# kwea123/nsff_pl

Hardware: AMD Instinct MI355X
Metric: ray-samples/sec (coarse+fine, static+dynamic) (higher is better)
Workload: dtype f16x3 (fp32 operands split into 2 halfs, 3 f16 MFMAs per product, fp32 accumulate; same 1e-4 parity as f32); 1 GPU; C2 (BASELINE.json configs[1]): static+dynamic NSFF, 1024 rays/GPU x (64 coarse + 64 importance -> 192 fine pts), train-mode fwd, fw/bw flow warp t+-1, perturb=1 noise_std=1, 8x256 MLPs, N_tau=48, all 47 outputs on device.  `value` is render_rays' throughput with autograd DISABLED (the train-mode FLAGS, inference launches: nothing kept for a backward pass); what a trainer's forward costs is aux.tra; rays_per_gpu=1024, N_samples=64, N_importance=64, parallelism=single GPU, field_launch=persistent (one workgroup per CU)

## Files before the change

include/nsff_render.h:

```cpp
#ifndef NSFF_RENDER_H
#define NSFF_RENDER_H

#include <stddef.h>
#include <stdint.h>

#ifdef __cplusplus
extern "C" {
#endif

#define NSFF_OK               0
#define NSFF_ERR_INVALID     -1
#define NSFF_ERR_NULL        -2
#define NSFF_ERR_ALIGN       -3
#define NSFF_ERR_HIP         -4

#define NSFF_ABI_VERSION      32
#define NSFF_RAW_STRIDE      16
#define NSFF_MAX_FREQS       24
#define NSFF_MAX_LAYERS       8


typedef struct NsffModelDesc {
    int32_t D;
    int32_t W;
    int32_t skip;
    int32_t in_xyz;
    int32_t in_dir;
    int32_t in_a;
    int32_t in_t;
    int32_t use_viewdir;
    int32_t has_transient;
    int32_t has_flow;
    float   flow_scale;
    int32_t skip_mask;
} NsffModelDesc;

static inline uint32_t nsff_skip_layers(const NsffModelDesc* d) {
    return d->skip_mask ? (uint32_t)d->skip_mask : (d->skip > 0 ? 1u << d->skip : 0u);
}

#define NSFF_PREC_F32        0
#define NSFF_PREC_F16X3      1

int nsff_packed_bytes(const NsffModelDesc* desc, int precision, size_t* bytes);

int nsff_param_count(const NsffModelDesc* desc);

int nsff_pack_weights(const NsffModelDesc* desc, int precision, const float* const* params,
                      void* packed, void* stream);

#define NSFF_PACK_SKIP_FOLD 1
int nsff_pack_weights_ex(const NsffModelDesc* desc, int precision, const float* const* params,
                         void* packed, int32_t flags, void* stream);
int nsff_fold_heads(const NsffModelDesc* desc, int precision, const float* const* params, void* packed, void* stream);

int nsff_posenc(const float* x, int64_t n_rows, const float* freqs_host, int n_freqs,
                float* out, void* stream);

int nsff_time_rows(const float* table, int64_t n_table, int32_t width, const int64_t* ts, int64_t n, int64_t max_t,
                   float* next, float* prev, void* stream);

int nsff_time_rows_backward(const float* g_cur, const float* g_next, const float* g_prev, const int64_t* ts, int64_t n,
                            int64_t max_t, int64_t n_table, int32_t width, float* d_table, void* stream);

typedef struct NsffFieldArgs {
    int64_t n_points;
    int32_t precision;
    int32_t tile_points;
    int32_t pts_per_ray;
    int32_t static_mode;
    int32_t transient_mode;
    int32_t flow_heads;
    const float* xyz;
    int32_t n_freqs;
    float   freqs[NSFF_MAX_FREQS];
    const float* dir_emb;
    const float* a_emb;
    const float* t_emb;
    const float* x_emb;
    int32_t ld_emb;
    int32_t off_xyz, off_dir, off_a, off_t;
    float*  raw;
    void*   save_acts;
    void*   save_xin;
    void*   save_masks;
    void*   save_side;
    const float* t_bias;
    int32_t t_bias_rows;
    int32_t reserved0;
    const float* s_bias;
    int32_t s_bias_rows;
    int32_t launch_form;
    int64_t save_lo_delta[3];
} NsffFieldArgs;

int nsff_field_query(const NsffModelDesc* desc, const void* packed,
                     const NsffFieldArgs* args, void* stream);

#define NSFF_MAX_TIME_BIAS_JOBS 4
typedef struct NsffTimeBiasJob {
    const NsffModelDesc* desc;
    const float* w[NSFF_MAX_LAYERS];
    const float* b[NSFF_MAX_LAYERS];
    const float* t_rows;
    float* out;
    const float* table;
    const int64_t* ts;
    int64_t n_table, max_t;
    int32_t delta, pad_;
    float* rows_out;
} NsffTimeBiasJob;
int nsff_time_bias_rows(const NsffModelDesc* desc);
int nsff_time_bias(const NsffTimeBiasJob* jobs, int32_t n_jobs, int64_t n_rays, void* stream);

#define NSFF_MAX_RNG_JOBS 12
typedef struct NsffRngJob {
    float*   out;
    int64_t  numel;
    uint64_t offset;
    int32_t  kind;
    uint32_t grid;
} NsffRngJob;
int nsff_rng_draws(const NsffRngJob* jobs, int32_t n_jobs, uint64_t seed, void* stream);
typedef struct NsffRngCoarse {
    const float* rays;
    const float* z_lin;
    float*       zs;
    float*       xyz;
    int32_t      n_samples;
    float        perturb;
    int32_t      job;
    int32_t      pad_;
} NsffRngCoarse;
int nsff_rng_draws_coarse(const NsffRngJob* jobs, int32_t n_jobs, uint64_t seed, const NsffRngCoarse* coarse, void* stream);

int nsff_side_bias(const NsffModelDesc* desc, const void* packed_f16x3, const float* w_dir, const float* dir_rows,
                   const float* a_rows, int64_t n_rays, float* out, void* stream);

int nsff_train_dims(const NsffModelDesc* desc, int32_t* xin_rows, int32_t* t_row0, int32_t* side_rows);
int nsff_bwd_packed_bytes(const NsffModelDesc* desc, size_t* bytes);
int nsff_pack_weights_bwd(const NsffModelDesc* desc, const float* const* params, void* packed, void* stream);
int nsff_pack_weights_bwd_ex(const NsffModelDesc* desc, const float* const* params, void* packed, const void* fwd_packed, void* stream);

typedef struct NsffFieldBwdArgs {
    int64_t n_points;
    int32_t static_mode;
    int32_t transient_mode;
    const float* d_raw;
    const float* raw;
    const float* gmax;
    const void*  masks;
    void*  dpre;
    void*  dhead;
    float* d_xin;
    float* d_side;
    int64_t dpre_lo_delta;
} NsffFieldBwdArgs;
int nsff_field_backward(const NsffModelDesc* desc, const void* packed_bwd, const NsffFieldBwdArgs* args, void* stream);
int nsff_last_bwd_kernel(void);
int nsff_last_bwd_grid(void);
int nsff_field_bwd_phase_program(const NsffModelDesc* desc, int32_t dynamic, int32_t want_xin, int64_t n_tiles, uint32_t* out,
                                 int32_t max_phases, uint32_t* seg_offsets, int32_t max_segs);

int nsff_field_input_backward(const float* d_xin, int32_t xin_rows, int32_t t_row0, const float* xyz, int64_t n_rays,
                              int32_t pts_per_ray, const float* freqs_host, int32_t n_freqs, int32_t in_t, float* d_xyz,
                              float* d_t, void* stream);

typedef struct NsffWgradJob {
    const void* a;  const void* b;
    int32_t a_rows, b_rows;
    int64_t out_off;
    int32_t trunk, pad_;
    int64_t a_lo_delta, b_lo_delta;
} NsffWgradJob;
int64_t nsff_weight_grad_scratch(const NsffWgradJob* jobs, int32_t n_jobs, int64_t n_tiles, int32_t n_splits);
int nsff_weight_grad(const NsffWgradJob* jobs, int32_t n_jobs, int64_t n_tiles, int32_t n_splits,
                     float* scratch, float* out, float* bias, const float* gmax, void* stream);

typedef struct NsffGradMapEntry {
    int32_t dst;
    int32_t e_a, e_b;
    int16_t job_a, job_b;
} NsffGradMapEntry;
int nsff_weight_grad_accumulate(const NsffWgradJob* jobs, int32_t n_jobs, int64_t n_tiles, int32_t n_splits, float* scratch,
                                const NsffGradMapEntry* map, int64_t n_map, float* grad_base, const float* gmax, void* stream);

int nsff_weight_grad_accumulate_aux(const NsffWgradJob* jobs, int32_t n_jobs, int64_t n_tiles, int32_t n_splits, float* scratch,
                                    const NsffGradMapEntry* map, int64_t n_map, float* grad_base, float* aux, const float* gmax,
                                    void* stream);

typedef struct NsffFoldGradArgs {
    int32_t n_rows, pad_;
    const float* g; const float* gb;
    const float* w_final; const float* b_final;
    const float* w_head[16];
    float* d_w_head[16]; float* d_b_head[16];
    float* d_w_final; float* d_b_final;
} NsffFoldGradArgs;
int nsff_fold_grads(const NsffFoldGradArgs* args, void* stream);

typedef struct NsffFoldDenseArgs {
    int32_t n_rows, accumulate;
    int32_t ld_head, ld_dhead;
    const float* g; const float* g2; const float* gb; const float* gb2;
    const float* w_head; const float* w_final; const float* b_final;
    float* d_w_head; float* d_b_head; float* d_w_final; float* d_b_final;
} NsffFoldDenseArgs;
int nsff_fold_grads_dense(const NsffFoldDenseArgs* args, void* stream);

int nsff_absmax(const float* x, int64_t n, float* out, void* stream);
int nsff_absmax_raw(const float* d_raw, int64_t n_points, float* out16, void* stream);

int nsff_adam_step(float* param, const float* grad, float* exp_avg, float* exp_avg_sq, int64_t n, float* state,
                   const float* lr, double beta1, double beta2, double eps, double weight_decay, void* stream);

int nsff_adam_step_segments(float* param, const float* grad, float* exp_avg, float* exp_avg_sq, int64_t n, float* state,
                            const float* lr, double beta1, double beta2, double eps, double weight_decay,
                            const int64_t* seg_start, int n_seg, int32_t* seg_used, void* stream);

typedef struct NsffLossArgs {
    int64_t n_rays; int32_t n_samples; int32_t n_keep;
    int32_t n_frames; int32_t max_t;
    double  topk;
    int32_t thickness; int32_t pad_;
    const float* rgb_fine; const float* rgb_coarse;
    const float* depth_fine; const float* depth_coarse;
    const float* t_weights; const float* s_weights;
    const float* xyz_fw; const float* xyz_bw;
    const float* rgb_fw; const float* rgb_bw;
    const float* disocc_fw; const float* disocc_bw;
    const float* disoccs_fw; const float* disoccs_bw;
    const float* xyzs_fw_bw; const float* xyzs_bw_fw;
    const float* xyzs_fine; const float* xyzs_fw; const float* xyzs_bw;
    const float* rgbs; const float* disps;
    const int64_t* ts; const int64_t* cam_ids;
    const float* uv_fw; const float* uv_bw;
    const float* Ks; const float* Ps;
    const float* hyper;
    float* stats;
    float* terms;
    const float* term_w;
    const float* weights;
    float* per_ray;
    float* coef;
    float* g_rgb_fine; float* g_rgb_coarse; float* g_depth_fine; float* g_depth_coarse;
    float* g_t_weights; float* g_s_weights; float* g_xyz_fw; float* g_xyz_bw; float* g_rgb_fw; float* g_rgb_bw;
    float* g_xyzs_fw_bw; float* g_xyzs_bw_fw; float* g_xyzs_fw; float* g_xyzs_bw;
} NsffLossArgs;
int nsff_nerfw_loss(const NsffLossArgs* args, int mode, void* stream);

int nsff_coarse_samples(const float* rays, int64_t n_rays, const float* z_lin, int32_t n_samples,
                        float perturb, const float* perturb_rand,
                        float* zs, float* xyz, void* stream);

int nsff_fine_samples(const float* rays, int64_t n_rays, const float* z_lin, const float* zs_coarse,
                      int32_t n_samples, int32_t n_importance,
                      const float* weights_static, const float* weights_transient,
                      const float* u_static, const float* u_transient, int32_t u_per_ray,
                      float* samples_static, float* samples_transient,
                      float* zs_fine, float* xyz_fine, void* stream);

int nsff_sample_pdf(const float* bins, const float* weights, int64_t n_rays, int32_t n_bins_minus1,
                    const float* u, int32_t n_importance, int32_t u_per_ray, float eps,
                    float* samples, void* stream);

int nsff_warp_points(const float* raw, const float* xyz, const float* zs, int64_t n_points,
                     float z_far, float* xyz_fw, float* xyz_bw, void* stream);

int nsff_frame_rays(const float* K4_host, const float* c2w_host, int32_t H, int32_t W, float near, float shift_near,
                    int64_t first_pixel, int64_t n_pixels, float* rays, void* stream);

typedef struct NsffFrustumArgs {
    const float*   w2c;
    const int64_t* ts;
    float   K4[4];
    int32_t n_cams, n_frames, H, W;
} NsffFrustumArgs;

typedef struct NsffCompositeArgs {
    int64_t n_rays;
    int32_t n_samples;
    int32_t has_transient;
    int32_t has_rgb;
    int32_t flow_mode;
    int32_t want_disocc;
    float   noise_std;
    float   z_far;
    const float* raw;
    const float* raw_fw;
    const float* raw_bw;
    const float* zs;
    const float* xyz;
    const float* xyz_fw;
    const float* xyz_bw;
    const float* noise_static;
    const float* noise_transient;
    const float* noise_fw;
    const float* noise_bw;
    const float* visibility;
    float* static_rgbs;  float* transient_rgbs;
    float* flows_fw;     float* flows_bw;
    float* static_sigmas; float* transient_sigmas;
    float* static_alphas; float* transient_alphas;
    float* static_weights; float* transient_weights; float* weights;
    float* xyzs_fw_bw;   float* xyzs_bw_fw;
    float* disoccs_fw;   float* disoccs_bw;
    float* depth;  float* rgb;  float* transient_alpha;  float* transient_rgb;
    float* static_only_rgb;  float* static_only_depth;
    float* xyz_exp;  float* flow_fw_exp;  float* flow_bw_exp;  float* xyz_fw_exp;  float* xyz_bw_exp;
    float* rgb_fw;   float* rgb_bw;
    float* disocc_fw;  float* disocc_bw;
    NsffFrustumArgs vis;
} NsffCompositeArgs;

int nsff_composite(const NsffCompositeArgs* args, void* stream);

int nsff_frustum_visibility(const NsffFrustumArgs* vis, const float* xyz, int64_t n_points, float* vis_count,
                            void* stream);

typedef struct NsffSplatArgs {
    int32_t H, W, n_planes;
    float   K4[4];
    float   P[12];
    float   scale;
    const float* xyz;
    const float* flow;
    const float* rgb;
    const float* alpha;
    float*       accum;
    void*        work;
    int64_t      work_bytes;
} NsffSplatArgs;
int64_t nsff_splat_work_bytes(int32_t H, int32_t W, int32_t n_planes);
int nsff_splat_planes(const NsffSplatArgs* args, void* stream);

typedef struct NsffMpiArgs {
    int32_t H, W, n_planes;
    float   dt;
    const float* accum_fw;
    const float* accum_bw;
    const float* static_rgb;
    const float* static_alpha;
    const float* zs;
    float* rgb;
    float* depth;
} NsffMpiArgs;
int nsff_mpi_composite(const NsffMpiArgs* args, void* stream);

typedef struct NsffCompositeBwdArgs {
    int64_t n_rays;
    int32_t n_samples, has_transient, flow_mode;
    float   noise_std;
    const float* raw;  const float* raw_fw;  const float* raw_bw;
    const float* zs;   const float* xyz;     const float* f_fw;  const float* f_bw;
    const float* noise_static;  const float* noise_transient;  const float* noise_fw;  const float* noise_bw;
    const float* g_static_sigmas;  const float* g_transient_sigmas;
    const float* g_static_weights; const float* g_transient_weights;  const float* g_weights;
    const float* g_depth;  const float* g_rgb;  const float* g_transient_alpha;  const float* g_transient_rgb;
    const float* g_so_rgb; const float* g_so_depth;
    const float* g_xyz_exp;  const float* g_flow_fw_exp;  const float* g_flow_bw_exp;
    const float* g_rgb_fw;   const float* g_rgb_bw;
    float* scratch;
    float* d_raw;  float* d_raw_fw;  float* d_raw_bw;  float* d_f_fw;  float* d_f_bw;
} NsffCompositeBwdArgs;
int nsff_composite_backward(const NsffCompositeBwdArgs* args, void* stream);

typedef struct {
    int64_t n_points;
    const float* zs;
    float z_far;
    int32_t accumulate;
    int32_t col_a, col_b;
    int32_t pad_;
    const float* g_a[4];
    const float* g_b[4];
    float* out;
} NsffFlowGradArgs;
int nsff_flow_grad(const NsffFlowGradArgs* args, void* stream);

#define NSFF_RAY_RECORD      16

typedef struct NsffSsimArgs {
    int32_t n_frames, H, W, window;
    const float* gt;  const float* pred;  const uint8_t* mask;
    float* map;  float* mean_map;  double* sums;
    void* scratch;  int64_t scratch_bytes;
} NsffSsimArgs;
int64_t nsff_ssim_scratch_bytes(int32_t n_frames, int32_t H, int32_t W);
int nsff_ssim(const NsffSsimArgs* args, void* stream);

int nsff_cdf(const float* weights, int64_t n_frames, int64_t n, double* cdf, void* stream);

typedef struct NsffRayDrawArgs {
    int64_t n_frames, n_pixels, frame, batch;
    const float* records;  const double* cdf;  const float* u;
    float* rays;  float* rgbs;  int64_t* ts;  int64_t* cam_ids;  float* disps;  float* rays_mask;  float* uv_fw;  float* uv_bw;
    int64_t* rand_idx;
} NsffRayDrawArgs;
int nsff_ray_draw(const NsffRayDrawArgs* args, void* stream);

int nsff_prof_enable(int on);
int nsff_prof_collect(int64_t* launches, double* total_ms, double* total_flops, double* executed_flops);
int nsff_prof_collect_clock(int64_t* launches, double* total_ms, double* total_flops, double* executed_flops,
                            double* shader_ticks, double* ticks_ms);

#define NSFF_KERNEL_F32       1
#define NSFF_KERNEL_H3_64     2
#define NSFF_KERNEL_H3_8WAVE  3
#define NSFF_KERNEL_H3A       4
#define NSFF_KERNEL_H3_SAVE   5
#define NSFF_KERNEL_H3A_TBIAS 7
#define NSFF_KERNEL_H3A_SAVE  9
#define NSFF_KERNEL_H3A_SIDE  8
int         nsff_last_field_kernel(void);
int         nsff_last_field_grid(void);
int         nsff_field_phase_program(const NsffModelDesc* desc, int static_mode, int transient_mode, int fold_t, uint32_t* steps,
                             int* n_steps, int* n_static_steps, uint32_t* phases_static, uint32_t* phases_dynamic, int* n_phases);

#define NSFF_RANGE_ACT     0x1u
#define NSFF_RANGE_SAVED   0x2u
#define NSFF_RANGE_PARAMS  0x4u
#define NSFF_RANGE_CODES   0x8u
int         nsff_range_flags(uint32_t* out, int32_t clear, void* stream);

int         nsff_abi_version(void);
const char* nsff_last_hip_error(void);

#ifdef __cplusplus
}
#endif
#endif
```

nsff_pl_amd/_lib.py:

```python
import ctypes as C
import os

import torch

_HERE = os.path.dirname(os.path.abspath(__file__))
LIB_PATH = os.environ.get("NSFF_LIB") or os.path.join(_HERE, "libnsff_hip.so")

RAW_STRIDE = 16
ABI_VERSION = 32
MAX_FREQS = 24

_ERR = {-1: "NSFF_ERR_INVALID (bad shape/flag/unsupported architecture)",
        -2: "NSFF_ERR_NULL (required pointer missing)",
        -3: "NSFF_ERR_ALIGN (pointer not 16-byte aligned)",
        -4: "NSFF_ERR_HIP"}

_fp = C.c_void_p


class ModelDesc(C.Structure):
    _fields_ = [("D", C.c_int32), ("W", C.c_int32), ("skip", C.c_int32),
                ("in_xyz", C.c_int32), ("in_dir", C.c_int32), ("in_a", C.c_int32),
                ("in_t", C.c_int32), ("use_viewdir", C.c_int32),
                ("has_transient", C.c_int32), ("has_flow", C.c_int32),
# ... 4 lines not shown
    _fields_ = [("n_points", C.c_int64), ("precision", C.c_int32), ("tile_points", C.c_int32),
                ("pts_per_ray", C.c_int32),
                ("static_mode", C.c_int32), ("transient_mode", C.c_int32),
                ("flow_heads", C.c_int32),
                ("xyz", _fp), ("n_freqs", C.c_int32), ("freqs", C.c_float * MAX_FREQS),
                ("dir_emb", _fp), ("a_emb", _fp), ("t_emb", _fp),
                ("x_emb", _fp), ("ld_emb", C.c_int32),
                ("off_xyz", C.c_int32), ("off_dir", C.c_int32), ("off_a", C.c_int32),
                ("off_t", C.c_int32), ("raw", _fp), ("save_acts", _fp), ("save_xin", _fp), ("save_masks", _fp),
                ("save_side", _fp), ("t_bias", _fp), ("t_bias_rows", C.c_int32), ("reserved0", C.c_int32),
                ("s_bias", _fp), ("s_bias_rows", C.c_int32), ("launch_form", C.c_int32), ("save_lo_delta", C.c_int64 * 3)]


class TimeBiasJob(C.Structure):
    _fields_ = [("desc", C.POINTER(ModelDesc)), ("w", _fp * 8), ("b", _fp * 8), ("t_rows", _fp), ("out", _fp),
                ("table", _fp), ("ts", _fp), ("n_table", C.c_int64), ("max_t", C.c_int64), ("delta", C.c_int32), ("pad_", C.c_int32),
                ("rows_out", _fp)]


MAX_TIME_BIAS_JOBS = 4


class RngJob(C.Structure):
    _fields_ = [("out", _fp), ("numel", C.c_int64), ("offset", C.c_uint64), ("kind", C.c_int32), ("grid", C.c_uint32)]


MAX_RNG_JOBS = 12


class RngCoarse(C.Structure):
    _fields_ = [("rays", _fp), ("z_lin", _fp), ("zs", _fp), ("xyz", _fp), ("n_samples", C.c_int32), ("perturb", C.c_float),
                ("job", C.c_int32), ("pad_", C.c_int32)]


_COMPOSITE_PTRS_IN = ["raw", "raw_fw", "raw_bw", "zs", "xyz", "xyz_fw", "xyz_bw",
                      "noise_static", "noise_transient", "noise_fw", "noise_bw", "visibility"]
_COMPOSITE_PTRS_OUT = ["static_rgbs", "transient_rgbs", "flows_fw", "flows_bw",
                       "static_sigmas", "transient_sigmas", "static_alphas", "transient_alphas",
                       "static_weights", "transient_weights", "weights",
                       "xyzs_fw_bw", "xyzs_bw_fw", "disoccs_fw", "disoccs_bw",
                       "depth", "rgb", "transient_alpha", "transient_rgb",
                       "static_only_rgb", "static_only_depth",
                       "xyz_exp", "flow_fw_exp", "flow_bw_exp", "xyz_fw_exp", "xyz_bw_exp",
                       "rgb_fw", "rgb_bw", "disocc_fw", "disocc_bw"]


class FrustumArgs(C.Structure):
    _fields_ = [("w2c", _fp), ("ts", _fp), ("K4", C.c_float * 4), ("n_cams", C.c_int32), ("n_frames", C.c_int32),
                ("H", C.c_int32), ("W", C.c_int32)]


class CompositeArgs(C.Structure):
    _fields_ = ([("n_rays", C.c_int64), ("n_samples", C.c_int32), ("has_transient", C.c_int32),
                 ("has_rgb", C.c_int32), ("flow_mode", C.c_int32), ("want_disocc", C.c_int32),
                 ("noise_std", C.c_float), ("z_far", C.c_float)]
                + [(n, _fp) for n in _COMPOSITE_PTRS_IN]
                + [(n, _fp) for n in _COMPOSITE_PTRS_OUT]
                + [("vis", FrustumArgs)])


_CBWD_IN = ["raw", "raw_fw", "raw_bw", "zs", "xyz", "f_fw", "f_bw", "noise_static", "noise_transient", "noise_fw", "noise_bw"]
_CBWD_G = ["g_static_sigmas", "g_transient_sigmas", "g_static_weights", "g_transient_weights", "g_weights", "g_depth",
           "g_rgb", "g_transient_alpha", "g_transient_rgb", "g_so_rgb", "g_so_depth", "g_xyz_exp", "g_flow_fw_exp",
           "g_flow_bw_exp", "g_rgb_fw", "g_rgb_bw"]
_CBWD_OUT = ["scratch", "d_raw", "d_raw_fw", "d_raw_bw", "d_f_fw", "d_f_bw"]


class CompositeBwdArgs(C.Structure):
    _fields_ = ([("n_rays", C.c_int64), ("n_samples", C.c_int32), ("has_transient", C.c_int32), ("flow_mode", C.c_int32),
                 ("noise_std", C.c_float)] + [(n, _fp) for n in _CBWD_IN + _CBWD_G + _CBWD_OUT])


class FieldBwdArgs(C.Structure):
    _fields_ = [("n_points", C.c_int64), ("static_mode", C.c_int32), ("transient_mode", C.c_int32),
                ("d_raw", _fp), ("raw", _fp), ("gmax", _fp), ("masks", _fp), ("dpre", _fp), ("dhead", _fp),
                ("d_xin", _fp), ("d_side", _fp), ("dpre_lo_delta", C.c_int64)]


class WgradJob(C.Structure):
    _fields_ = [("a", _fp), ("b", _fp), ("a_rows", C.c_int32), ("b_rows", C.c_int32), ("out_off", C.c_int64), ("trunk", C.c_int32),
                ("pad_", C.c_int32), ("a_lo_delta", C.c_int64), ("b_lo_delta", C.c_int64)]


class FoldGradArgs(C.Structure):
    _fields_ = [("n_rows", C.c_int32), ("pad_", C.c_int32), ("g", _fp), ("gb", _fp), ("w_final", _fp), ("b_final", _fp),
                ("w_head", _fp * 16), ("d_w_head", _fp * 16), ("d_b_head", _fp * 16), ("d_w_final", _fp), ("d_b_final", _fp)]


class FoldDenseArgs(C.Structure):
    _fields_ = [("n_rows", C.c_int32), ("accumulate", C.c_int32), ("ld_head", C.c_int32), ("ld_dhead", C.c_int32),
                ("g", _fp), ("g2", _fp), ("gb", _fp), ("gb2", _fp), ("w_head", _fp), ("w_final", _fp), ("b_final", _fp),
                ("d_w_head", _fp), ("d_b_head", _fp), ("d_w_final", _fp), ("d_b_final", _fp)]


class SplatArgs(C.Structure):
    _fields_ = [("H", C.c_int32), ("W", C.c_int32), ("n_planes", C.c_int32), ("K4", C.c_float * 4),
                ("P", C.c_float * 12), ("scale", C.c_float),
                ("xyz", _fp), ("flow", _fp), ("rgb", _fp), ("alpha", _fp), ("accum", _fp), ("work", _fp),
                ("work_bytes", C.c_int64)]


class MpiArgs(C.Structure):
    _fields_ = [("H", C.c_int32), ("W", C.c_int32), ("n_planes", C.c_int32), ("dt", C.c_float),
                ("accum_fw", _fp), ("accum_bw", _fp), ("static_rgb", _fp), ("static_alpha", _fp), ("zs", _fp),
                ("rgb", _fp), ("depth", _fp)]


_LOSS_IN = ["rgb_fine", "rgb_coarse", "depth_fine", "depth_coarse", "t_weights", "s_weights", "xyz_fw", "xyz_bw", "rgb_fw",
            "rgb_bw", "disocc_fw", "disocc_bw", "disoccs_fw", "disoccs_bw", "xyzs_fw_bw", "xyzs_bw_fw", "xyzs_fine",
            "xyzs_fw", "xyzs_bw", "rgbs", "disps", "ts", "cam_ids", "uv_fw", "uv_bw", "Ks", "Ps", "hyper", "stats", "terms",
            "term_w"]
LOSS_GRADS = ["g_rgb_fine", "g_rgb_coarse", "g_depth_fine", "g_depth_coarse", "g_t_weights", "g_s_weights", "g_xyz_fw",
              "g_xyz_bw", "g_rgb_fw", "g_rgb_bw", "g_xyzs_fw_bw", "g_xyzs_bw_fw", "g_xyzs_fw", "g_xyzs_bw"]


class LossArgs(C.Structure):
    _fields_ = ([("n_rays", C.c_int64), ("n_samples", C.c_int32), ("n_keep", C.c_int32), ("n_frames", C.c_int32),
                 ("max_t", C.c_int32), ("topk", C.c_double), ("thickness", C.c_int32), ("pad_", C.c_int32)]
                + [(n, _fp) for n in _LOSS_IN] + [("weights", _fp), ("per_ray", _fp), ("coef", _fp)]
                + [(n, _fp) for n in LOSS_GRADS])


class FlowGradArgs(C.Structure):
    _fields_ = [("n_points", C.c_int64), ("zs", _fp), ("z_far", C.c_float), ("accumulate", C.c_int32), ("col_a", C.c_int32),
                ("col_b", C.c_int32), ("pad_", C.c_int32), ("g_a", _fp * 4), ("g_b", _fp * 4), ("out", _fp)]


class SsimArgs(C.Structure):
    _fields_ = [("n_frames", C.c_int32), ("H", C.c_int32), ("W", C.c_int32), ("window", C.c_int32),
                ("gt", _fp), ("pred", _fp), ("mask", _fp), ("map", _fp), ("mean_map", _fp), ("sums", _fp),
                ("scratch", _fp), ("scratch_bytes", C.c_int64)]


RAY_RECORD = 16
_DRAW_OUT = ["rays", "rgbs", "ts", "cam_ids", "disps", "rays_mask", "uv_fw", "uv_bw", "rand_idx"]


class RayDrawArgs(C.Structure):
    _fields_ = ([("n_frames", C.c_int64), ("n_pixels", C.c_int64), ("frame", C.c_int64), ("batch", C.c_int64),
                 ("records", _fp), ("cdf", _fp), ("u", _fp)] + [(n, _fp) for n in _DRAW_OUT])


_SIGNATURES = {
    "nsff_abi_version": (C.c_int, []),
    "nsff_range_flags": (C.c_int, [_fp, C.c_int32, _fp]),
    "nsff_last_field_kernel": (C.c_int, []),
    "nsff_last_field_grid": (C.c_int, []),
    "nsff_field_phase_program": (C.c_int, [C.POINTER(ModelDesc), C.c_int, C.c_int, C.c_int, C.POINTER(C.c_uint32), C.POINTER(C.c_int),
                                   C.POINTER(C.c_int), C.POINTER(C.c_uint32), C.POINTER(C.c_uint32), C.POINTER(C.c_int)]),
    "nsff_time_bias_rows": (C.c_int, [C.POINTER(ModelDesc)]),
    "nsff_time_bias": (C.c_int, [C.POINTER(TimeBiasJob), C.c_int32, C.c_int64, C.c_void_p]),
    "nsff_rng_draws": (C.c_int, [C.POINTER(RngJob), C.c_int32, C.c_uint64, C.c_void_p]),
    "nsff_rng_draws_coarse": (C.c_int, [C.POINTER(RngJob), C.c_int32, C.c_uint64, C.POINTER(RngCoarse), C.c_void_p]),
    "nsff_side_bias": (C.c_int, [C.POINTER(ModelDesc), _fp, _fp, _fp, _fp, C.c_int64, _fp, C.c_void_p]),
    "nsff_last_hip_error": (C.c_char_p, []),
    "nsff_packed_bytes": (C.c_int, [C.POINTER(ModelDesc), C.c_int, C.POINTER(C.c_size_t)]),
    "nsff_param_count": (C.c_int, [C.POINTER(ModelDesc)]),
    "nsff_pack_weights": (C.c_int, [C.POINTER(ModelDesc), C.c_int, C.POINTER(_fp), _fp, _fp]),
    "nsff_pack_weights_ex": (C.c_int, [C.POINTER(ModelDesc), C.c_int, C.POINTER(_fp), _fp, C.c_int32, _fp]),
    "nsff_fold_heads": (C.c_int, [C.POINTER(ModelDesc), C.c_int, C.POINTER(_fp), _fp, _fp]),
    "nsff_posenc": (C.c_int, [_fp, C.c_int64, C.POINTER(C.c_float), C.c_int, _fp, _fp]),
    "nsff_time_rows": (C.c_int, [_fp, C.c_int64, C.c_int32, _fp, C.c_int64, C.c_int64, _fp, _fp, _fp]),
    "nsff_time_rows_backward": (C.c_int, [_fp, _fp, _fp, _fp, C.c_int64, C.c_int64, C.c_int64, C.c_int32, _fp, _fp]),
    "nsff_field_query": (C.c_int, [C.POINTER(ModelDesc), _fp, C.POINTER(FieldArgs), _fp]),
    "nsff_coarse_samples": (C.c_int, [_fp, C.c_int64, _fp, C.c_int32, C.c_float, _fp, _fp, _fp, _fp]),
    "nsff_fine_samples": (C.c_int, [_fp, C.c_int64, _fp, _fp, C.c_int32, C.c_int32, _fp, _fp, _fp, _fp,
                                    C.c_int32, _fp, _fp, _fp, _fp, _fp]),
    "nsff_sample_pdf": (C.c_int, [_fp, _fp, C.c_int64, C.c_int32, _fp, C.c_int32, C.c_int32,
                                  C.c_float, _fp, _fp]),
    "nsff_warp_points": (C.c_int, [_fp, _fp, _fp, C.c_int64, C.c_float, _fp, _fp, _fp]),
    "nsff_composite": (C.c_int, [C.POINTER(CompositeArgs), _fp]),
    "nsff_frustum_visibility": (C.c_int, [C.POINTER(FrustumArgs), _fp, C.c_int64, _fp, _fp]),
    "nsff_frame_rays": (C.c_int, [C.POINTER(C.c_float), C.POINTER(C.c_float), C.c_int32, C.c_int32, C.c_float,
                                  C.c_float, C.c_int64, C.c_int64, _fp, _fp]),
    "nsff_bwd_packed_bytes": (C.c_int, [C.POINTER(ModelDesc), C.POINTER(C.c_size_t)]),
    "nsff_pack_weights_bwd": (C.c_int, [C.POINTER(ModelDesc), C.POINTER(_fp), _fp, _fp]),
    "nsff_field_backward": (C.c_int, [C.POINTER(ModelDesc), _fp, C.POINTER(FieldBwdArgs), _fp]),
    "nsff_field_input_backward": (C.c_int, [_fp, C.c_int32, C.c_int32, _fp, C.c_int64, C.c_int32, C.POINTER(C.c_float), C.c_int32,
                                            C.c_int32, _fp, _fp, _fp]),
    "nsff_train_dims": (C.c_int, [C.POINTER(ModelDesc), C.POINTER(C.c_int32), C.POINTER(C.c_int32), C.POINTER(C.c_int32)]),
    "nsff_weight_grad_scratch": (C.c_int64, [C.POINTER(WgradJob), C.c_int32, C.c_int64, C.c_int32]),
    "nsff_weight_grad": (C.c_int, [C.POINTER(WgradJob), C.c_int32, C.c_int64, C.c_int32, _fp, _fp, _fp, _fp, _fp]),
    "nsff_weight_grad_accumulate": (C.c_int, [C.POINTER(WgradJob), C.c_int32, C.c_int64, C.c_int32, _fp, _fp, C.c_int64,
                                              _fp, _fp, _fp]),
    "nsff_weight_grad_accumulate_aux": (C.c_int, [C.POINTER(WgradJob), C.c_int32, C.c_int64, C.c_int32, _fp, _fp, C.c_int64,
                                                  _fp, _fp, _fp, _fp]),
    "nsff_absmax_raw": (C.c_int, [_fp, C.c_int64, _fp, _fp]),
    "nsff_last_bwd_kernel": (C.c_int, []),
    "nsff_last_bwd_grid": (C.c_int, []),
    "nsff_field_bwd_phase_program": (C.c_int, [C.POINTER(ModelDesc), C.c_int32, C.c_int32, C.c_int64, C.POINTER(C.c_uint32), C.c_int32,
                                                C.POINTER(C.c_uint32), C.c_int32]),
    "nsff_fold_grads": (C.c_int, [C.POINTER(FoldGradArgs), _fp]),
    "nsff_fold_grads_dense": (C.c_int, [C.POINTER(FoldDenseArgs), _fp]),
    "nsff_pack_weights_bwd_ex": (C.c_int, [C.POINTER(ModelDesc), C.POINTER(_fp), _fp, _fp, _fp]),
    "nsff_absmax": (C.c_int, [_fp, C.c_int64, _fp, _fp]),
    "nsff_adam_step": (C.c_int, [_fp, _fp, _fp, _fp, C.c_int64, _fp, _fp, C.c_double, C.c_double, C.c_double, C.c_double, _fp]),
    "nsff_adam_step_segments": (C.c_int, [_fp, _fp, _fp, _fp, C.c_int64, _fp, _fp, C.c_double, C.c_double, C.c_double, C.c_double,
                                          _fp, C.c_int, _fp, _fp]),
    "nsff_composite_backward": (C.c_int, [C.POINTER(CompositeBwdArgs), _fp]),
    "nsff_flow_grad": (C.c_int, [C.POINTER(FlowGradArgs), _fp]),
    "nsff_nerfw_loss": (C.c_int, [C.POINTER(LossArgs), C.c_int, _fp]),
    "nsff_splat_planes": (C.c_int, [C.POINTER(SplatArgs), _fp]),
    "nsff_splat_work_bytes": (C.c_int64, [C.c_int32, C.c_int32, C.c_int32]),
    "nsff_mpi_composite": (C.c_int, [C.POINTER(MpiArgs), _fp]),
    "nsff_ssim_scratch_bytes": (C.c_int64, [C.c_int32, C.c_int32, C.c_int32]),
    "nsff_ssim": (C.c_int, [C.POINTER(SsimArgs), _fp]),
    "nsff_cdf": (C.c_int, [_fp, C.c_int64, C.c_int64, _fp, _fp]),
    "nsff_ray_draw": (C.c_int, [C.POINTER(RayDrawArgs), _fp]),
    "nsff_prof_enable": (C.c_int, [C.c_int]),
    "nsff_prof_collect": (C.c_int, [C.POINTER(C.c_int64), C.POINTER(C.c_double), C.POINTER(C.c_double), C.POINTER(C.c_double)]),
    "nsff_prof_collect_clock": (C.c_int, [C.POINTER(C.c_int64)] + [C.POINTER(C.c_double)] * 5),
}
EXPORTED_SYMBOLS = tuple(_SIGNATURES)

_lib = None


def load():
    global _lib
    if _lib is None:
        if not os.path.exists(LIB_PATH):
            raise RuntimeError(
                f"{LIB_PATH} is missing: build it with `python -c 'import __graft_entry__ as g; g.build()'` "
                "(or `make -C nsff_pl_amd/csrc`).  There is no CPU fallback for the render path.")
        lib = C.CDLL(LIB_PATH)
        for name, (res, args) in _SIGNATURES.items():
            fn = getattr(lib, name)
            fn.restype, fn.argtypes = res, args
        if lib.nsff_abi_version() != ABI_VERSION:
            raise RuntimeError("libnsff_hip.so ABI version mismatch")
        _lib = lib
    return _lib


def _check(rc, what):
    if rc != 0:
        msg = _ERR.get(rc, f"error {rc}")
        if rc == -4:
            msg += ": " + load().nsff_last_hip_error().decode()
        raise RuntimeError(f"{what} failed: {msg}")


def require_gpu_tensor(t, what):
    if not isinstance(t, torch.Tensor) or not t.is_cuda:
        raise RuntimeError(f"{what} must be a GPU tensor: the NSFF render path runs only on the "
                           "HIP kernels of libnsff_hip.so (no CPU fallback)")


def _ptr(t):
    if t is None:
        return None
    assert t.is_cuda and t.dtype == torch.float32 and t.is_contiguous(), "need contiguous fp32 GPU tensor"
    return t.data_ptr()


def _stream():
    return torch.cuda.current_stream().cuda_stream


def model_desc(model):
    if model.W != 256:
        raise RuntimeError(f"unsupported NeRF architecture: W={model.W} (the gfx950 field kernels tile W=256 trunks "
                           "into 4 x 64-neuron wave blocks; other widths are not built)")
    skips = sorted(set(int(s) for s in model.skips))
    if not 2 <= model.D <= 8 or any(not 1 <= s < model.D for s in skips):
        raise RuntimeError(f"unsupported NeRF architecture: D={model.D}, skips={list(model.skips)} (need 2 <= D <= 8 "
                           "and every skip layer in 1..D-1; a skip at layer 0 would concatenate the input with itself)")
    mask = sum(1 << s for s in skips)
    return ModelDesc(D=model.D, W=model.W, skip=skips[0] if len(skips) == 1 else 0, skip_mask=mask if len(skips) != 1 else 0,
                     in_xyz=model.in_channels_xyz,
                     in_dir=model.in_channels_dir,
                     in_a=model.in_channels_a if model.use_viewdir else 0,
                     in_t=model.in_channels_t, use_viewdir=int(model.use_viewdir),
                     has_transient=int(model.encode_transient),
                     has_flow=int(getattr(model, "has_flow_heads", hasattr(model, "transient_flow_fw"))),
                     flow_scale=float(getattr(model, "flow_scale", 0.0)))


def param_list(model):
    def lin(m):
        layer = m[0] if isinstance(m, torch.nn.Sequential) else m
        return [layer.weight, layer.bias]
    out = []
    for i in range(model.D):
        out += lin(getattr(model, f"static_xyz_encoding_{i + 1}"))
    out += lin(model.static_xyz_encoding_final)
    if model.use_viewdir:
        out += lin(model.static_dir_encoding)
    out += lin(model.static_sigma) + lin(model.static_rgb)
    if model.encode_transient:
        for i in range(model.D):
            out += lin(getattr(model, f"transient_xyz_encoding_{i + 1}"))
        out += lin(model.transient_xyz_encoding_final)
        out += lin(model.transient_sigma) + lin(model.transient_rgb)
        if hasattr(model, "transient_flow_fw"):
            out += lin(model.transient_flow_fw) + lin(model.transient_flow_bw)
    return out


def packed_bytes(desc, precision=0):
    n = C.c_size_t(0)
    _check(load().nsff_packed_bytes(C.byref(desc), int(precision), C.byref(n)), "nsff_packed_bytes")
    return n.value


PACK_SKIP_FOLD = 1


def pack_weights(desc, params, packed, precision=0, fold=True):
    lib = load()
    if lib.nsff_param_count(C.byref(desc)) != len(params):
        raise RuntimeError("parameter list does not match the model description")
    keep = [p.detach().contiguous().float() for p in params]
    for p in keep:
        require_gpu_tensor(p, "model parameter")
    arr = (_fp * len(keep))(*[p.data_ptr() for p in keep])
    _check(lib.nsff_pack_weights_ex(C.byref(desc), int(precision), arr, _ptr(packed), 0 if fold else PACK_SKIP_FOLD,
                                    _stream()), "nsff_pack_weights_ex")
    return keep


def fold_heads(desc, params, packed, precision):
    keep = [p.detach().contiguous().float() for p in params]
    arr = (_fp * len(keep))(*[p.data_ptr() for p in keep])
    _check(load().nsff_fold_heads(C.byref(desc), int(precision), arr, _ptr(packed), _stream()), "nsff_fold_heads")
    return keep


def time_rows_backward(g_cur, g_next, g_prev, ts, max_t, n_table):
    gs = [None if g is None else g.contiguous() for g in (g_cur, g_next, g_prev)]
    width = next(g for g in gs if g is not None).shape[1]
    assert ts.dtype == torch.int64 and ts.is_cuda and ts.is_contiguous()
    d = torch.empty(int(n_table), width, device=ts.device)
    _check(load().nsff_time_rows_backward(_ptr(gs[0]), _ptr(gs[1]), _ptr(gs[2]), C.c_void_p(ts.data_ptr()), ts.shape[0],
                                          int(max_t), int(n_table), width, _ptr(d), _stream()), "nsff_time_rows_backward")
    return d


def time_rows(table, ts, max_t, want_next=True, want_prev=True):
    n, width = ts.shape[0], table.shape[1]
    if want_next and want_prev:
        both = torch.empty(2, n, width, device=table.device)
        nxt, prv = both[0], both[1]
    else:
        nxt = torch.empty(n, width, device=table.device) if want_next else None
        prv = torch.empty(n, width, device=table.device) if want_prev else None
    assert ts.dtype == torch.int64 and ts.is_cuda and ts.is_contiguous()
    _check(load().nsff_time_rows(_ptr(table), table.shape[0], width, C.c_void_p(ts.data_ptr()), n, int(max_t),
                                 _ptr(nxt), _ptr(prv), _stream()), "nsff_time_rows")
    return nxt, prv


def posenc(x, freqs, out):
    f = [float(v) for v in freqs]
    arr = (C.c_float * len(f))(*f)
    _check(load().nsff_posenc(_ptr(x), x.shape[0], arr, len(f), _ptr(out), _stream()), "nsff_posenc")


def field_query(model, raw, n_points, pts_per_ray, static_mode, transient_mode, flow_heads=0,
                xyz=None, freqs=None, dir_emb=None, a_emb=None, t_emb=None,
                x_emb=None, emb_offsets=(0, -1, -1, -1), save_acts=None, save_xin=None, save_masks=None, save_side=None,
                precision=None, t_bias=None, s_bias=None, save_lo=False):
    from . import config
    desc = model_desc(model)
    prec = config.precision_code(model) if precision is None else precision
    saves = not (save_acts is None and save_xin is None and save_masks is None and save_side is None)
    packed = model.packed(prec)
    a = FieldArgs()
    a.precision, a.tile_points = prec, config.get_tile_points()
    a.launch_form = 0 if config.get_persistent() else 1
    a.n_points, a.pts_per_ray = int(n_points), int(pts_per_ray)
    a.static_mode, a.transient_mode, a.flow_heads = int(static_mode), int(transient_mode), int(flow_heads)
    a.xyz = _ptr(xyz)
    if freqs is not None:
        f = [float(v) for v in freqs]
        if len(f) > MAX_FREQS:
            raise RuntimeError("too many embedding frequencies")
        a.n_freqs = len(f)
        for i, v in enumerate(f):
            a.freqs[i] = v
    a.dir_emb, a.a_emb, a.t_emb = _ptr(dir_emb), _ptr(a_emb), _ptr(t_emb)
    a.x_emb = _ptr(x_emb)
    a.ld_emb = int(x_emb.shape[1]) if x_emb is not None else 0
    a.off_xyz, a.off_dir, a.off_a, a.off_t = [int(v) for v in emb_offsets]
    a.raw = _ptr(raw)
    a.save_acts = None if save_acts is None else save_acts.data_ptr()
    a.save_xin = None if save_xin is None else save_xin.data_ptr()
    a.save_masks = None if save_masks is None else save_masks.data_ptr()
    a.save_side = None if save_side is None else save_side.data_ptr()
    if save_lo:
        for i, t in enumerate((save_acts, save_xin, save_side)):
            a.save_lo_delta[i] = 0 if t is None else lo_delta(t)
    if t_bias is not None:
        a.t_bias, a.t_bias_rows = _ptr(t_bias), int(t_bias.shape[1])
    if s_bias is not None:
        a.s_bias, a.s_bias_rows = _ptr(s_bias), int(s_bias.shape[1])
    _check(load().nsff_field_query(C.byref(desc), _ptr(packed), C.byref(a), _stream()), "nsff_field_query")


def lo_delta(t):
    n = t.numel()
    if t.untyped_storage().nbytes() < (t.storage_offset() + 2 * n) * t.element_size():
        raise RuntimeError("three-product backward: this buffer has no remainder plane behind it (field_grad.alloc_saves(..., x3=True))")
    return n


def side_bias(model, dir_rows, a_rows=None):
    from . import config
    desc = model_desc(model)
    n_rays = int(dir_rows.shape[0])
    assert dir_rows.shape == (n_rays, desc.in_dir) and (desc.in_a == 0 or (a_rows is not None and a_rows.shape == (n_rays, desc.in_a)))
    packed = model.packed(config.PRECISIONS["f16x3"])
    w = model.static_dir_encoding[0].weight.detach()
    out = torch.empty(n_rays, 1, 256, device=dir_rows.device, dtype=torch.float32)
    _check(load().nsff_side_bias(C.byref(desc), _ptr(packed), _ptr(w), _ptr(dir_rows), _ptr(a_rows) if desc.in_a > 0 else None,
                                 n_rays, _ptr(out), _stream()), "nsff_side_bias")
    return out


_DEVICE_RNG_GEOMETRY = {}


def fused_draws(plan, device, values=True, coarse=None):
    dev = torch.device(device)
    idx = dev.index if dev.index is not None else torch.cuda.current_device()
    if idx not in _DEVICE_RNG_GEOMETRY:
        p = torch.cuda.get_device_properties(idx)
        _DEVICE_RNG_GEOMETRY[idx] = p.multi_processor_count * (p.max_threads_per_multi_processor // 256)
    max_grid = _DEVICE_RNG_GEOMETRY[idx]
    gen = torch.cuda.default_generators[idx]
    seed, offset = gen.initial_seed(), gen.get_offset()
    wanted = values if isinstance(values, (list, tuple)) else [bool(values)] * len(plan)
    sizes = []
    for kind, shape in plan:
        n = 1
        for s in shape:
            n *= int(s)
        sizes.append(n)
    total = sum(n for n, w in zip(sizes, wanted) if w)
    buf = torch.empty(max(total, 1), device=dev, dtype=torch.float32)
    outs, jobs, at = [], [], 0
    for (kind, shape), numel, want in zip(plan, sizes, wanted):
        if numel == 0:
            outs.append(torch.empty(*shape, device=dev, dtype=torch.float32))
            continue
        grid = min(max_grid, (numel + 255) // 256)
        if coarse is not None and not outs and not want:
            jobs.append((None, numel, offset, 0, grid))
            outs.append(None)
        elif want:
            t = buf[at:at + numel].view(*shape)
            at += numel
            jobs.append((t, numel, offset, 1 if kind == "randn" else 0, grid))
            outs.append(t)
        else:
            outs.append(None)
        offset += ((numel - 1) // (1024 * grid) + 1) * 4
    hook = None
    if coarse is not None:
        rays, z_lin, perturb, zs, xyz = coarse
        assert plan and plan[0][0] == "rand" and tuple(plan[0][1]) == (rays.shape[0], z_lin.shape[0]) and perturb > 0
        if sizes[0]:
            hook = RngCoarse(_ptr(rays), _ptr(z_lin), _ptr(zs), _ptr(xyz), int(z_lin.shape[0]), float(perturb), 0, 0)
    for k in range(0, len(jobs), MAX_RNG_JOBS):
        part = jobs[k:k + MAX_RNG_JOBS]
        arr = (RngJob * len(part))()
        for j, (t, numel, off, kind, grid) in enumerate(part):
            arr[j].out, arr[j].numel, arr[j].offset, arr[j].kind, arr[j].grid = (None if t is None else t.data_ptr()), numel, off, kind, grid
        with torch.cuda.device(idx):
            _check(load().nsff_rng_draws_coarse(arr, len(part), seed, C.byref(hook) if (hook is not None and k == 0) else None, _stream()),
                   "nsff_rng_draws")
    gen.set_offset(offset)
    return outs


_FUSED_DRAWS_OK = {}


def fused_draws_match_torch(device):
    dev = torch.device(device)
    idx = dev.index if dev.index is not None else torch.cuda.current_device()
    if idx in _FUSED_DRAWS_OK:
        return _FUSED_DRAWS_OK[idx]
    if torch.cuda.is_current_stream_capturing():
        return False
    gen = torch.cuda.default_generators[idx]
    state = gen.get_state()
    ok = True
    try:
        plan = [("rand", (7, 64)), ("randn", (1031,)), ("rand", (3, 5, 2)), ("randn", (70000,)), ("rand", (300001,))]
        gen.manual_seed(0x5EED1234)
        gen.set_offset(8)
        mine = fused_draws(plan, torch.device("cuda", idx))
        end_mine = gen.get_offset()
        gen.manual_seed(0x5EED1234)
        gen.set_offset(8)
        with torch.cuda.device(idx):
            ref = [(torch.rand if k == "rand" else torch.randn)(*shape, device=torch.device("cuda", idx)) for k, shape in plan]
        end_ref = gen.get_offset()
        ok = end_mine == end_ref and all(torch.equal(a.view(torch.int32), b.view(torch.int32)) for a, b in zip(mine, ref))
    except Exception:
        ok = False
    finally:
        gen.set_state(state)
    if not ok:
        import warnings
        warnings.warn("nsff_pl_amd: the fused generator kernel (nsff_rng_draws) no longer reproduces torch.rand / torch.randn on "
                      f"cuda:{idx} (torch {torch.__version__}); render_rays draws with the torch calls instead (slower by ~1 %, same "
                      "numbers as the reference)")
    _FUSED_DRAWS_OK[idx] = ok
    return ok


def time_bias_rows(model):
    return load().nsff_time_bias_rows(C.byref(model_desc(model)))


def time_bias(jobs, index=None):
    assert 1 <= len(jobs) <= MAX_TIME_BIAS_JOBS
    arr = (TimeBiasJob * len(jobs))()
    keep, outs, per_model, pair = [], [], {}, None
    rows_of = {}
    if index is not None:
        table, ts, max_t = index
        assert ts.dtype == torch.int64 and ts.is_cuda and ts.is_contiguous() and ts.dim() == 1, "ts: one int64 frame index per ray"
        n_rays, width = int(ts.shape[0]), int(table.shape[1])
        deltas = sorted({int(d) for _, d in jobs})
        if 1 in deltas and -1 in deltas:
            both = torch.empty(2, n_rays, width, device=table.device, dtype=torch.float32)
            rows_of[1], rows_of[-1] = both[0], both[1]
        for d in deltas:
            if d not in rows_of:
                rows_of[d] = torch.empty(n_rays, width, device=table.device, dtype=torch.float32)
        written = set()
    else:
        n_rays = int(jobs[0][1].shape[0])
    for j, (model, t_rows) in enumerate(jobs):
        if id(model) not in per_model:
            desc = model_desc(model)
            lins = [getattr(model, f"transient_xyz_encoding_{l + 1}")[0] for l in [0] + sorted(set(int(v) for v in model.skips))]
            wb = [(m.weight.detach(), m.bias.detach()) for m in lins]
            for w, b in wb:
                _ptr(w), _ptr(b)
            per_model[id(model)] = (desc, C.pointer(desc), wb)
        desc, pdesc, wb = per_model[id(model)]
        if index is not None:
            delta, t_rows = int(t_rows), None
            assert width == desc.in_t
        else:
            assert t_rows.shape == (n_rays, desc.in_t)
        dev = wb[0][0].device
        if j + 1 < len(jobs) and jobs[j + 1][0] is model and pair is None:
            pair = torch.empty(2, n_rays, len(wb), 256, device=dev, dtype=torch.float32)
            out = pair[0]
        elif pair is not None:
            out, pair = pair[1], None
        else:
            out = torch.empty(n_rays, len(wb), 256, device=dev, dtype=torch.float32)
        arr[j].desc = pdesc
        for i, (w, b) in enumerate(wb):
            arr[j].w[i], arr[j].b[i] = w.data_ptr(), b.data_ptr()
        arr[j].t_rows, arr[j].out = _ptr(t_rows), _ptr(out)
        if index is not None:
            arr[j].table, arr[j].ts = _ptr(table), ts.data_ptr()
            arr[j].n_table, arr[j].max_t, arr[j].delta = int(table.shape[0]), int(max_t), delta
            if delta not in written:
                arr[j].rows_out = _ptr(rows_of[delta])
                written.add(delta)
        outs.append(out)
    keep.append(per_model)
    _check(load().nsff_time_bias(arr, len(jobs), n_rays, _stream()), "nsff_time_bias")
    return outs if index is None else (outs, rows_of)


def coarse_samples(rays, z_lin, perturb, perturb_rand, zs, xyz):
    _check(load().nsff_coarse_samples(_ptr(rays), rays.shape[0], _ptr(z_lin), z_lin.shape[0],
                                      float(perturb), _ptr(perturb_rand), _ptr(zs), _ptr(xyz), _stream()),
           "nsff_coarse_samples")


def fine_samples(rays, z_lin, zs_coarse, n_importance, w_static, w_transient, u_static, u_transient,
                 u_per_ray, samples_static, samples_transient, zs_fine, xyz_fine):
    _check(load().nsff_fine_samples(_ptr(rays), rays.shape[0], _ptr(z_lin), _ptr(zs_coarse),
                                    z_lin.shape[0], int(n_importance), _ptr(w_static), _ptr(w_transient),
                                    _ptr(u_static), _ptr(u_transient), int(u_per_ray),
                                    _ptr(samples_static), _ptr(samples_transient),
                                    _ptr(zs_fine), _ptr(xyz_fine), _stream()), "nsff_fine_samples")


def sample_pdf(bins, weights, u, u_per_ray, eps, samples):
    _check(load().nsff_sample_pdf(_ptr(bins), _ptr(weights), weights.shape[0], weights.shape[1],
                                  _ptr(u), samples.shape[1], int(u_per_ray), float(eps),
                                  _ptr(samples), _stream()), "nsff_sample_pdf")


def warp_points(raw, xyz, zs, z_far, xyz_fw, xyz_bw):
    _check(load().nsff_warp_points(_ptr(raw), _ptr(xyz), _ptr(zs), zs.numel(), float(z_far),
                                   _ptr(xyz_fw), _ptr(xyz_bw), _stream()), "nsff_warp_points")


def frustum_args(w2c, ts, K4, n_cams, n_frames, H, W):
    assert w2c.is_cuda and w2c.dtype == torch.float32 and w2c.is_contiguous() and w2c.shape == (n_cams * n_frames, 12)
    assert ts.is_cuda and ts.dtype == torch.int64 and ts.is_contiguous() and ts.numel() >= 1
    a = FrustumArgs(w2c=w2c.data_ptr(), ts=ts.data_ptr(), n_cams=int(n_cams), n_frames=int(n_frames), H=int(H), W=int(W))
    a.K4[:] = [float(v) for v in K4]
    a._keep = (w2c, ts)
    return a


def frustum_visibility(vis, xyz, out):
    _check(load().nsff_frustum_visibility(C.byref(vis), _ptr(xyz), xyz.shape[0], _ptr(out), _stream()),
           "nsff_frustum_visibility")


def composite(vis=None, **kw):
    a = CompositeArgs()
    for k, v in kw.items():
        if k in _COMPOSITE_PTRS_IN or k in _COMPOSITE_PTRS_OUT:
            setattr(a, k, _ptr(v))
        else:
            setattr(a, k, v)
    if vis is not None:
        a.vis = vis
    _check(load().nsff_composite(C.byref(a), _stream()), "nsff_composite")


def frame_rays(K4, c2w12, H, W, near, shift_near, first, count, rays):
    k = (C.c_float * 4)(*[float(v) for v in K4])
    m = (C.c_float * 12)(*[float(v) for v in c2w12])
    _check(load().nsff_frame_rays(k, m, int(H), int(W), float(near), float(shift_near), int(first), int(count),
                                  _ptr(rays), _stream()), "nsff_frame_rays")


BWD_PACK = 100


def bwd_packed_bytes(desc):
    n = C.c_size_t(0)
    _check(load().nsff_bwd_packed_bytes(C.byref(desc), C.byref(n)), "nsff_bwd_packed_bytes")
    return n.value


def pack_weights_bwd(desc, params, packed, fwd_packed=None):
    arr = (_fp * len(params))(*[p.data_ptr() for p in params])
    _check(load().nsff_pack_weights_bwd_ex(C.byref(desc), arr, _ptr(packed), _ptr(fwd_packed), _stream()), "nsff_pack_weights_bwd_ex")


def last_bwd_kernel():
    return {0: "c", 1: "h3b", 2: "c+h3b", 3: "x3"}[load().nsff_last_bwd_kernel()]


def last_bwd_grid():
    return load().nsff_last_bwd_grid()


def field_bwd_phase_program(model, dynamic, want_xin, n_tiles, max_phases=32):
    import numpy as np
    desc = model_desc(model)
    out = (C.c_uint32 * (8 * max_phases))()
    segs = (C.c_uint32 * 48)()
    n = load().nsff_field_bwd_phase_program(C.byref(desc), 1 if dynamic else 0, 1 if want_xin else 0, int(n_tiles), out, max_phases, segs, 48)
    if n < 0:
        raise RuntimeError(f"nsff_field_bwd_phase_program failed ({n})")
    offs = np.array(list(segs), np.uint32)
    return (np.array(list(out), np.uint32).reshape(max_phases, 8)[:n] if n > 0 else None), offs


def field_backward(model, n_points, static, transient, d_raw, raw, gmax, masks, dpre, dhead, d_xin, d_side=None, x3=False):
    desc = model_desc(model)
    a = FieldBwdArgs(n_points=int(n_points), static_mode=2 if static else 0, transient_mode=2 if transient else 0,
                     d_raw=_ptr(d_raw), raw=_ptr(raw), gmax=_ptr(gmax), masks=masks.data_ptr(), dpre=dpre.data_ptr(),
                     dhead=dhead.data_ptr(), d_xin=_ptr(d_xin), d_side=_ptr(d_side), dpre_lo_delta=lo_delta(dpre) if x3 else 0)
    _check(load().nsff_field_backward(C.byref(desc), _ptr(model.packed(BWD_PACK)), C.byref(a), _stream()),
           "nsff_field_backward")


def train_dims(model):
    desc = model_desc(model)
    xr, t0, sr = C.c_int32(0), C.c_int32(0), C.c_int32(0)
    _check(load().nsff_train_dims(C.byref(desc), C.byref(xr), C.byref(t0), C.byref(sr)), "nsff_train_dims")
    return xr.value, t0.value, sr.value


def field_input_backward(d_xin, t_row0, xyz, pts_per_ray, freqs, in_t, want_xyz, want_t):
    P, xin_rows = d_xin.shape
    n_rays = P // pts_per_ray
    d_xyz = torch.empty(P, 3, device=d_xin.device) if want_xyz else None
    d_t = torch.empty(n_rays, in_t, device=d_xin.device) if want_t else None
    f = [float(v) for v in freqs]
    arr = (C.c_float * max(len(f), 1))(*f)
    _check(load().nsff_field_input_backward(_ptr(d_xin), int(xin_rows), int(t_row0), _ptr(xyz), n_rays, int(pts_per_ray), arr,
                                            len(f), int(in_t), _ptr(d_xyz), _ptr(d_t), _stream()), "nsff_field_input_backward")
    return d_xyz, d_t


def _wgrad_jobs(jobs, with_off):
    return (WgradJob * len(jobs))(*[WgradJob(a=j[0], b=j[1], a_rows=j[2], b_rows=j[3], out_off=j[4] if with_off else 0, trunk=j[5],
                                             a_lo_delta=j[6] if len(j) > 6 else 0, b_lo_delta=j[7] if len(j) > 7 else 0) for j in jobs])


def weight_grad(jobs, n_tiles, n_splits, out, bias, gmax):
    arr = _wgrad_jobs(jobs, True)
    n = load().nsff_weight_grad_scratch(arr, len(jobs), int(n_tiles), int(n_splits))
    if n < 0:
        raise RuntimeError("nsff_weight_grad_scratch failed")
    scratch = torch.empty(n, device=out.device)
    _check(load().nsff_weight_grad(arr, len(jobs), int(n_tiles), int(n_splits), _ptr(scratch), _ptr(out), _ptr(bias),
                                   _ptr(gmax), _stream()), "nsff_weight_grad")


def weight_grad_accumulate(jobs, n_tiles, n_splits, grad_map, grad_base_ptr, gmax, aux=None):
    arr = _wgrad_jobs(jobs, False)
    n = load().nsff_weight_grad_scratch(arr, len(jobs), int(n_tiles), int(n_splits))
    if n < 0:
        raise RuntimeError("nsff_weight_grad_scratch failed")
    assert grad_map.dtype == torch.int32 and grad_map.is_contiguous() and grad_map.shape[1] == 4
    scratch = torch.empty(n, device=gmax.device)
    _check(load().nsff_weight_grad_accumulate_aux(arr, len(jobs), int(n_tiles), int(n_splits), _ptr(scratch),
                                                  C.c_void_p(grad_map.data_ptr()), grad_map.shape[0], C.c_void_p(grad_base_ptr),
                                                  _ptr(aux), _ptr(gmax), _stream()), "nsff_weight_grad_accumulate_aux")
    return scratch


def fold_grads(g, gb, w_final, b_final, head_rows, d_w_final, d_b_final):
    a = FoldGradArgs(n_rows=len(head_rows), g=_ptr(g), gb=_ptr(gb), w_final=_ptr(w_final), b_final=_ptr(b_final),
                     d_w_final=_ptr(d_w_final), d_b_final=_ptr(d_b_final))
    for r, (w, dw, db) in enumerate(head_rows):
        a.w_head[r], a.d_w_head[r], a.d_b_head[r] = w.data_ptr(), dw.data_ptr(), db.data_ptr()
    _check(load().nsff_fold_grads(C.byref(a), _stream()), "nsff_fold_grads")


def fold_grads_dense(g, gb, w_head, w_final, b_final, d_w_head, d_b_head, d_w_final, d_b_final, accumulate, g2=None, gb2=None):
    R = int(g.shape[0])
    for t in (g, g2, gb, gb2, w_final, b_final, d_w_final, d_b_final, d_b_head):
        assert t is None or (t.is_cuda and t.dtype == torch.float32 and t.is_contiguous())
    for t in (w_head, d_w_head):
        assert t.is_cuda and t.dtype == torch.float32 and t.shape[0] == R and t.shape[1] == 256 and t.stride(1) == 1
    a = FoldDenseArgs(n_rows=R, accumulate=1 if accumulate else 0, ld_head=int(w_head.stride(0)), ld_dhead=int(d_w_head.stride(0)),
                      g=g.data_ptr(), g2=None if g2 is None else g2.data_ptr(), gb=gb.data_ptr(), gb2=None if gb2 is None else gb2.data_ptr(),
                      w_head=w_head.data_ptr(), w_final=w_final.data_ptr(), b_final=b_final.data_ptr(), d_w_head=d_w_head.data_ptr(),
                      d_b_head=d_b_head.data_ptr(), d_w_final=d_w_final.data_ptr(), d_b_final=d_b_final.data_ptr())
    _check(load().nsff_fold_grads_dense(C.byref(a), _stream()), "nsff_fold_grads_dense")


def absmax(x):
    x = x.contiguous()
    if x.dim() == 2 and x.shape[1] == RAW_STRIDE:
        out = torch.empty(RAW_STRIDE, device=x.device, dtype=torch.float32)
        _check(load().nsff_absmax_raw(_ptr(x), x.shape[0], _ptr(out), _stream()), "nsff_absmax_raw")
        return out
    out = torch.empty((), device=x.device, dtype=torch.float32)
    _check(load().nsff_absmax(_ptr(x), x.numel(), _ptr(out), _stream()), "nsff_absmax")
    return out


def adam_step(param, grad, exp_avg, exp_avg_sq, state, lr, beta1, beta2, eps, weight_decay, seg_start=None, seg_used=None):
    if seg_start is None:
        _check(load().nsff_adam_step(_ptr(param), _ptr(grad), _ptr(exp_avg), _ptr(exp_avg_sq), param.numel(), _ptr(state), _ptr(lr),
                                     float(beta1), float(beta2), float(eps), float(weight_decay), _stream()), "nsff_adam_step")
        return
    _check(load().nsff_adam_step_segments(_ptr(param), _ptr(grad), _ptr(exp_avg), _ptr(exp_avg_sq), param.numel(), _ptr(state),
                                          _ptr(lr), float(beta1), float(beta2), float(eps), float(weight_decay),
                                          C.c_void_p(seg_start.data_ptr()), int(seg_used.numel()),
                                          C.c_void_p(seg_used.data_ptr()), _stream()),
           "nsff_adam_step_segments")


def composite_backward(n_rays, n_samples, has_transient, flow_mode, noise_std, **tensors):
    a = CompositeBwdArgs(n_rays=int(n_rays), n_samples=int(n_samples), has_transient=int(has_transient),
                         flow_mode=int(flow_mode), noise_std=float(noise_std))
    for k, v in tensors.items():
        setattr(a, k, _ptr(v))
    _check(load().nsff_composite_backward(C.byref(a), _stream()), "nsff_composite_backward")


def flow_grad(zs, z_far, out, accumulate, col_a=-1, g_a=(), col_b=-1, g_b=()):
    a = FlowGradArgs(n_points=int(out.shape[0]), zs=_ptr(zs), z_far=float(z_far), accumulate=int(bool(accumulate)),
# ... 152 lines not shown
```

nsff_pl_amd/csrc/field_h3.hip:

```cpp
#include <hip/hip_runtime.h>
#include <algorithm>
#include <cstdlib>
#include <vector>
#include "nsff_layout_h3.h"
#include "nsff_common.h"
#include "nsff_internal.h"

typedef float f32x16 __attribute__((ext_vector_type(16)));
typedef _Float16 h8 __attribute__((ext_vector_type(8)));
typedef _Float16 h4 __attribute__((ext_vector_type(4)));
typedef __fp16 h2 __attribute__((ext_vector_type(2)));
typedef _Float16 h2f __attribute__((ext_vector_type(2)));

#ifdef H3_TIMING
__device__ unsigned g_h3_timing[256 * 8 * 32 * 6 + 256 * 4 * 256];
#define H3A_TBASE (256 * 8 * 32 * 6)
__device__ unsigned long long g_h3_span[2] = {~0ull, 0ull};
#define H3_SPAN(k) do { if (lane == 0) { const unsigned long long t_ = __builtin_amdgcn_s_memtime(); \
    if (k) atomicMax(&g_h3_span[1], t_); else atomicMin(&g_h3_span[0], t_); } } while (0)
#define H3_STAMP(k) do { if (lane == 0 && blockIdx.x < 256 && i < 32) \
    g_h3_timing[((blockIdx.x * 8 + wave_id) * 32 + i) * 6 + (k)] = (unsigned)__builtin_amdgcn_s_memtime(); } while (0)
#define H3_HSTAMP(k) do { if (lane == 0 && blockIdx.x < 256) \
    g_h3_timing[((blockIdx.x * 8 + wave) * 32 + 30) * 6 + (k)] = (unsigned)__builtin_amdgcn_s_memtime(); } while (0)
#else
#define H3_STAMP(k) do {} while (0)
#define H3_SPAN(k) do {} while (0)
#define H3_HSTAMP(k) do {} while (0)
#endif

namespace {

#ifndef H3_SAVE_INTERLEAVE
#define H3_SAVE_INTERLEAVE 1
#endif
constexpr int LDH = 264;
__device__ __forceinline__ h8 lds_h8(const _Float16* p) { return *reinterpret_cast<const h8*>(p); }

struct H3Step {
    uint32_t w_off;
    uint32_t bias_off;
    uint16_t nks;
    uint8_t pre;
    uint8_t post;
    uint8_t head;
    uint8_t save;
    uint8_t pad[2];
};
enum { PRE_NONE = 0, PRE_INPUT = 1, PRE_INPUT_T = 2, PRE_SIDE = 3 };
enum { POST_NONE = 0, POST_RELU = 1, POST_LINEAR = 2 };
enum { HEAD_NONE = 0, HEAD_S_SIGMA = 1, HEAD_S_RGB = 2, HEAD_T = 3, HEAD_S_FOLD = 4, HEAD_T_FOLD = 5 };
constexpr int MAX_STEPS = 28;

struct H3KArgs {
    NsffLayoutH3 L;
    H3Step steps[MAX_STEPS];
    int n_steps;
    int n_static_steps;
    int split_trunks;
    long long grid_tiles;
    const uint32_t* packed;
    const float* xyz;
    const float* x_emb;
    const float* dir_emb;
    const float* a_emb;
    const float* t_emb;
    const float* t_bias;
    int tb_rows;
    const float* s_bias;
    int sb_rows;
    float* raw;
    long long lo_delta[3];
    _Float16* save_acts;
    _Float16* save_xin;
    unsigned long long* save_masks;
    _Float16* save_side;
    long long save_stride;
    int xin_rows, side_rows;
    long long n_tiles;
    long long n_points;
    int pts_per_ray;
    int static_mode, transient_mode;
    int D, skip;
    int in_xyz, in_dir, in_a, in_t;
    int use_viewdir;
    float flow_scale;
    int n_freqs;
    int octave_freqs;
    float freqs[NSFF_MAX_FREQS];
    int ld_emb, off_xyz, off_dir, off_a, off_t;
    unsigned long long* span;
    uint32_t* range;
};

struct SpanT { unsigned long long t, r; };
__device__ __forceinline__ SpanT span_begin(const unsigned long long* span) {
    SpanT s{0ull, 0ull};
#ifdef H3_TIMING
    s.t = __builtin_amdgcn_s_memtime();
#endif
    if (span != nullptr && (blockIdx.x & 15) == 0) { s.t = __builtin_amdgcn_s_memtime(); s.r = __builtin_amdgcn_s_memrealtime(); }
    return s;
}
__device__ __forceinline__ void span_end(unsigned long long* span, const SpanT& s0, unsigned tid) {
    if (span == nullptr || (blockIdx.x & 15) != 0 || tid != 0) return;
    const unsigned long long t = __builtin_amdgcn_s_memtime(), r = __builtin_amdgcn_s_memrealtime();
    atomicAdd(span, t - s0.t);
    atomicAdd(span + 1, r - s0.r);
}
__device__ __forceinline__ void span_end(unsigned long long* span, const SpanT& s0) { span_end(span, s0, threadIdx.x); }

#define MFMA_H(a, b, c) __builtin_amdgcn_mfma_f32_32x32x16_f16((a), (b), (c), 0, 0, 0)
#define H3_PIN() __builtin_amdgcn_sched_barrier(0)

__device__ __forceinline__ void split_store(_Float16* xh, _Float16* xl, int idx, float v, float& rm) {
    rm = nsff_absmax3(rm, v, v);
    const _Float16 hi = (_Float16)v;
    xh[idx] = hi;
    xl[idx] = (_Float16)(v - (float)hi);
}

template <int MTW> struct WFrag { h8 wh[MTW], wl[MTW]; };
template <int NT> struct XFrag { h8 xh[NT], xl[NT]; };
template <int MTW> struct WRing { WFrag<MTW> r[4]; };
template <int MTW> struct BiasRegs { float4 b[MTW][4]; };

template <int MTW>
__device__ __forceinline__ void load_w(WFrag<MTW>& f, const uint4* __restrict__& wp) {
    if constexpr (MTW == 2) {
        const uint4 a0 = wp[0], a1 = wp[64], a2 = wp[128], a3 = wp[192];
        wp += 256;
        f.wh[0] = __builtin_bit_cast(h8, a0); f.wl[0] = __builtin_bit_cast(h8, a1);
        f.wh[1] = __builtin_bit_cast(h8, a2); f.wl[1] = __builtin_bit_cast(h8, a3);
    } else {
        const uint4 a0 = wp[0], a1 = wp[64];
        wp += 256;
        f.wh[0] = __builtin_bit_cast(h8, a0); f.wl[0] = __builtin_bit_cast(h8, a1);
    }
}

template <int NT> struct BRows { const _Float16* h[NT]; const _Float16* l[NT]; };
template <int NT>
__device__ __forceinline__ BRows<NT> b_rows(const _Float16* bh, const _Float16* bl, int ld) {
    BRows<NT> b;
#pragma unroll
    for (int nt = 0; nt < NT; ++nt) { b.h[nt] = bh + nt * 32 * ld; b.l[nt] = bl + nt * 32 * ld; }
    return b;
}

template <int NT>
__device__ __forceinline__ void load_x(XFrag<NT>& f, const BRows<NT>& b, int ks) {
#pragma unroll
    for (int nt = 0; nt < NT; ++nt) {
        f.xh[nt] = lds_h8(b.h[nt] + ks * 16);
        f.xl[nt] = lds_h8(b.l[nt] + ks * 16);
    }
}

template <int MTW>
__device__ __forceinline__ const uint4* prefetch_w(WRing<MTW>& ring, const uint4* __restrict__ w) {
// ... 1513 lines not shown
                       hipStream_t st) {
    const NsffModelDesc& d = *desc;
    FoldArgs fs, ft, fd;
    const int pi = fold_args(d, params, fs, ft, fd);
    for (int i = 0; i < pi; ++i) if (!params[i]) return NSFF_ERR_NULL;
    if (!d.use_viewdir) {
        fs.out_w = s_w; fs.out_b = s_b;
        hipLaunchKernelGGL(nsff_fold_kernel_h3, dim3(4), dim3(256), 0, st, fs);
    }
    if (d.has_transient) {
        ft.out_w = t_w; ft.out_b = t_b;
        hipLaunchKernelGGL(nsff_fold_kernel_h3, dim3(d.has_flow ? 10 : 4), dim3(256), 0, st, ft);
    }
    return nsff_launch_status();
}

int nsff_h3_fold_heads(const NsffModelDesc* desc, const float* const* params, void* packed, hipStream_t st) {
    NsffLayoutH3 L;
    const int rc = nsff_make_layout_h3(*desc, L);
    if (rc) return rc;
    const NsffModelDesc& d = *desc;
    FoldArgs fs, ft, fd;
    const int pi = fold_args(d, params, fs, ft, fd);
    for (int i = 0; i < pi; ++i) if (!params[i]) return NSFF_ERR_NULL;
    uint32_t* pw = reinterpret_cast<uint32_t*>(packed);
    PackArgsH3 pf{};
    pf.dst = pw;
    pf.range = nsff_range_word(st);
    int nf = 0;
    auto fold = [&](FoldArgs& f, uint32_t scratch, uint32_t tile, uint32_t bias) {
        f.out_w = reinterpret_cast<float*>(pw + scratch); f.out_b = reinterpret_cast<float*>(pw + bias);
        hipLaunchKernelGGL(nsff_fold_kernel_h3, dim3(32), dim3(256), 0, st, f);
        pf.seg[nf++] = PackSegH3{f.out_w, tile, 2, NSFF_W, NSFF_W, 0, 0, 0, 0, 0, 0, 32};
    };
    if (!d.use_viewdir) fold(fs, L.fold_f32, L.s_fold_w, L.s_fold_b);
    if (d.has_transient) fold(ft, L.fold_f32 + 32 * NSFF_W, L.t_fold_w, L.t_fold_b);
    int max_threads = 8 * NSFF_W;
    if (d.use_viewdir) {
        fd.out_w = reinterpret_cast<float*>(pw + L.dir_fold_f32); fd.out_b = reinterpret_cast<float*>(pw + L.dir_b_fold);
        hipLaunchKernelGGL(nsff_fold_kernel_h3, dim3(NSFF_W), dim3(256), 0, st, fd);
        pf.seg[nf++] = PackSegH3{fd.out_w, L.dir_h_fold, 1, NSFF_W, NSFF_W, NSFF_W, 0, 0, 0, 0, 0, 0};
        max_threads = 64 * NSFF_W;
    }
    if (nf > 0) hipLaunchKernelGGL(nsff_pack_kernel_h3, dim3((max_threads + 255) / 256, nf), dim3(256), 0, st, pf);
    return nsff_launch_status();
}

static int h3_step_program(const NsffModelDesc& d, int static_mode, int transient_mode, bool fold, H3KArgs& k, bool side_fold = false) {
    int n = 0;
    auto push = [&](uint32_t w, uint32_t b, uint32_t kcols, int pre, int post, int head, int slot = -1) {
        H3Step& s = k.steps[n++];
        s.w_off = w; s.bias_off = b; s.nks = (uint16_t)(kcols / 16);
        s.pre = (uint8_t)pre; s.post = (uint8_t)post; s.head = (uint8_t)head;
        s.save = (uint8_t)(slot + 1);
    };
    auto trunk = [&](const NsffTrunkLayoutH3& T, int pre_kind, int last_head, int slot0) {
        for (int l = 0; l < d.D; ++l) {
            const int head = (l == d.D - 1) ? last_head : HEAD_NONE;
            if (l == 0) {
                push(T.seg_x[0], T.bias[0], T.k0, pre_kind, POST_RELU, HEAD_NONE, slot0);
            } else if ((nsff_skip_layers(&d) >> l) & 1u) {
                push(T.seg_h[l], T.bias[l], NSFF_W, PRE_NONE, POST_NONE, HEAD_NONE);
                push(T.seg_x[l], NSFF_NONE, T.k0, pre_kind, POST_RELU, head, slot0 + l);
            } else {
                push(T.seg_h[l], T.bias[l], NSFF_W, PRE_NONE, POST_RELU, head, slot0 + l);
            }
        }
    };
    if (static_mode == 2 && fold && !d.use_viewdir) {
        trunk(k.L.st, PRE_INPUT, HEAD_S_FOLD, 0);
    } else if (static_mode == 2 && fold && side_fold) {
        trunk(k.L.st, PRE_INPUT, HEAD_S_SIGMA, 0);
        push(k.L.dir_h_fold, k.L.dir_b_fold, NSFF_W, PRE_NONE, POST_RELU, HEAD_S_RGB, d.D);
    } else if (static_mode == 2 && fold) {
        trunk(k.L.st, PRE_INPUT, HEAD_S_SIGMA, 0);
        push(k.L.dir_h_fold, k.L.dir_b_fold, NSFF_W, PRE_NONE, POST_NONE, HEAD_NONE);
        push(k.L.dir_x, NSFF_NONE, k.L.side_k, PRE_SIDE, POST_RELU, HEAD_S_RGB, d.D);
    } else if (static_mode) {
        trunk(k.L.st, PRE_INPUT, HEAD_S_SIGMA, 0);
        if (static_mode == 2) {
            push(k.L.st.final_w, k.L.st.final_b, NSFF_W, PRE_NONE, POST_LINEAR, d.use_viewdir ? HEAD_NONE : HEAD_S_RGB, d.D);
            if (d.use_viewdir) {
                push(k.L.dir_h, k.L.dir_b, NSFF_W, PRE_NONE, POST_NONE, HEAD_NONE);
                push(k.L.dir_x, NSFF_NONE, k.L.side_k, PRE_SIDE, POST_RELU, HEAD_S_RGB, d.D);
            }
        }
    }
    k.n_static_steps = n;
    if (transient_mode && fold) {
        trunk(k.L.tr, PRE_INPUT_T, HEAD_T_FOLD, d.D + 1);
    } else if (transient_mode) {
        trunk(k.L.tr, PRE_INPUT_T, HEAD_NONE, d.D + 1);
        push(k.L.tr.final_w, k.L.tr.final_b, NSFF_W, PRE_NONE, POST_LINEAR, HEAD_T, 2 * d.D + 1);
    }
    if (n > MAX_STEPS) return NSFF_ERR_INVALID;
    k.n_steps = n;
    return NSFF_OK;
}

static bool h3a_make_persistent(H3APhase* ph) {
    int at = -1;
    for (int i = 1; i < H3A_MAX_PHASES && !(i > 1 && ph[i].d[0] == H3A_BODY_END); ++i)
        if (ph[i].d[0] == H3A_BODY_B16L) { if (at >= 0) return false; at = i; }
    if (at < 0) return false;
    ph[at].d[0] = H3A_BODY_B16LP;
    for (int j = 3; j < 8; ++j) ph[at].d[j] = ph[0].d[j];
    return true;
}

extern "C" int nsff_field_phase_program(const NsffModelDesc* desc, int static_mode, int transient_mode, int fold_t, uint32_t* steps,
                                int* n_steps, int* n_static_steps, uint32_t* phases_static, uint32_t* phases_dynamic, int* n_phases) {
    if (!desc || !steps || !n_steps || !n_static_steps || !phases_static || !phases_dynamic || !n_phases) return NSFF_ERR_NULL;
    H3KArgs k{};
    int rc = nsff_make_layout_h3(*desc, k.L);
    if (rc) return rc;
    const bool side_fold = (fold_t & 2) != 0 && static_mode == 2 && desc->use_viewdir;
    const bool persist = (fold_t & 4) != 0;
    fold_t &= 1;
    rc = h3_step_program(*desc, static_mode, transient_mode, true, k, side_fold);
    if (rc) return rc;
    for (int i = 0; i < k.n_steps; ++i) {
        const H3Step& st = k.steps[i];
        steps[4 * i + 0] = st.w_off; steps[4 * i + 1] = st.bias_off;
        steps[4 * i + 2] = (uint32_t)st.nks | ((uint32_t)st.pre << 8) | ((uint32_t)st.post << 16) | ((uint32_t)st.head << 24);
        steps[4 * i + 3] = 0;
    }
    *n_steps = k.n_steps; *n_static_steps = k.n_static_steps;
    n_phases[0] = n_phases[1] = 0;
    H3APhase ph[H3A_MAX_PHASES];
    uint32_t boff[H3A_MAX_BIAS];
    int nb = 0, head = 0;
    if (k.n_static_steps > 0 && (side_fold || !(static_mode == 2 && desc->use_viewdir))) {
        for (auto& p : ph) for (auto& x : p.d) x = 0;
        int np = 0;
        k.sb_rows = side_fold ? 1 : 0;
        if (h3a_build_program(k, 0, k.n_static_steps, false, false, ph, boff, nb, head, &np, side_fold) && (!persist || h3a_make_persistent(ph))) {
            n_phases[0] = np;
            for (int i = 0; i < n_phases[0]; ++i) for (int j = 0; j < 8; ++j) phases_static[8 * i + j] = ph[i].d[j];
        }
    }
    if (k.n_steps > k.n_static_steps) {
        for (auto& p : ph) for (auto& x : p.d) x = 0;
        int np = 0;
        k.tb_rows = fold_t ? nsff_time_bias_rows(desc) : 0;
        if (h3a_build_program(k, k.n_static_steps, k.n_steps, true, fold_t != 0, ph, boff, nb, head, &np) && (!persist || h3a_make_persistent(ph))) {
            n_phases[1] = np;
            for (int i = 0; i < n_phases[1]; ++i) for (int j = 0; j < 8; ++j) phases_dynamic[8 * i + j] = ph[i].d[j];
        }
    }
    return NSFF_OK;
}

namespace {
struct TimeBiasJobK { const float* w[NSFF_MAX_LAYERS]; const float* b[NSFF_MAX_LAYERS]; int ld[NSFF_MAX_LAYERS];
                      const float* t_rows; float* out; int rows, in_xyz, in_t;
                      const float* table; const long long* ts; long long n_table, max_t; int delta; float* rows_out; };
struct TimeBiasArgs { TimeBiasJobK job[NSFF_MAX_TIME_BIAS_JOBS]; long long n_rays; };
constexpr int TB_RAYS = 16;
__global__ __launch_bounds__(256) void nsff_time_bias_kernel(const TimeBiasArgs a) {
    const TimeBiasJobK& j = a.job[blockIdx.z];
    const int i = blockIdx.y, n = threadIdx.x;
    if (i >= j.rows) return;
    const long long r0 = (long long)blockIdx.x * TB_RAYS;
    __shared__ __attribute__((aligned(16))) float st[TB_RAYS][64];
    __shared__ float sw[16][NSFF_W + 1];
    const float* __restrict__ wl = j.w[i] + j.in_xyz;
    const int ld = j.ld[i], in_t = j.in_t;
    float tv[TB_RAYS / 4], wv[4][16];
#pragma unroll
    for (int k = 0; k < TB_RAYS / 4; ++k) {
        const int e = threadIdx.x + 256 * k, r = e >> 6, c = e & 63;
        const long long ray = r0 + r < a.n_rays ? r0 + r : a.n_rays - 1;
        const float* row = j.t_rows != nullptr ? j.t_rows + ray * in_t : nullptr;
        if (row == nullptr) {
            long long t = j.ts[ray] + j.delta;
            if (j.delta > 0) t = t < j.max_t ? t : j.max_t;
            if (j.delta < 0) t = t > 0 ? t : 0;
            t = t < 0 ? 0 : (t > j.n_table - 1 ? j.n_table - 1 : t);
            row = j.table + t * in_t;
        }
        tv[k] = c < in_t ? row[c] : 0.f;
        if (j.rows_out != nullptr && i == 0 && c < in_t && r0 + r < a.n_rays) j.rows_out[(r0 + r) * in_t + c] = tv[k];
    }
    const float b = j.b[i][n];
#pragma unroll
    for (int q = 0; q < 4; ++q)
#pragma unroll
        for (int k = 0; k < 16; ++k) {
            const int e = threadIdx.x + 256 * k, row = e >> 4, c = 16 * q + (e & 15);
            wv[q][k] = c < in_t ? wl[row * ld + c] : 0.f;
        }
#pragma unroll
    for (int k = 0; k < TB_RAYS / 4; ++k) { const int e = threadIdx.x + 256 * k; st[e >> 6][e & 63] = tv[k]; }
    float acc[TB_RAYS];
#pragma unroll
    for (int r = 0; r < TB_RAYS; ++r) acc[r] = b;
#pragma unroll
    for (int q = 0; q < 4; ++q) {
        if (16 * q >= in_t) break;
        __syncthreads();
#pragma unroll
        for (int k = 0; k < 16; ++k) { const int e = threadIdx.x + 256 * k; sw[e & 15][e >> 4] = wv[q][k]; }
        __syncthreads();
#pragma unroll
        for (int u = 0; u < 16; u += 4) {
            const float w0 = sw[u][n], w1 = sw[u + 1][n], w2 = sw[u + 2][n], w3 = sw[u + 3][n];
#pragma unroll
            for (int r = 0; r < TB_RAYS; ++r) {
                const float4 t4 = *reinterpret_cast<const float4*>(&st[r][16 * q + u]);
                acc[r] = fmaf(w3, t4.w, fmaf(w2, t4.z, fmaf(w1, t4.y, fmaf(w0, t4.x, acc[r]))));
            }
        }
    }
#pragma unroll
    for (int r = 0; r < TB_RAYS; ++r)
        if (r0 + r < a.n_rays) j.out[((r0 + r) * j.rows + i) * NSFF_W + n] = acc[r];
}
}

extern "C" int nsff_time_bias_rows(const NsffModelDesc* desc) {
    if (!desc || !desc->has_transient || desc->in_t < 1) return 0;
    return 1 + __builtin_popcount(nsff_skip_layers(desc));
}

extern "C" int nsff_time_bias(const NsffTimeBiasJob* jobs, int32_t n_jobs, int64_t n_rays, void* stream) {
    if (!jobs) return NSFF_ERR_NULL;
    if (n_jobs < 1 || n_jobs > NSFF_MAX_TIME_BIAS_JOBS || n_rays < 0) return NSFF_ERR_INVALID;
    if (n_rays == 0) return NSFF_OK;
    TimeBiasArgs a{};
    a.n_rays = n_rays;
    int max_rows = 0;
    for (int q = 0; q < n_jobs; ++q) {
        const NsffTimeBiasJob& jb = jobs[q];
        if (!jb.desc || !jb.out) return NSFF_ERR_NULL;
        if (!jb.t_rows && (!jb.table || !jb.ts || jb.n_table < 1 || jb.delta < -1 || jb.delta > 1)) return NSFF_ERR_NULL;
        const NsffModelDesc& d = *jb.desc;
        NsffLayoutH3 L;
        const int rc = nsff_make_layout_h3(d, L);
        if (rc) return rc;
        TimeBiasJobK& k = a.job[q];
        k.rows = nsff_time_bias_rows(&d);
        if (k.rows < 1) return NSFF_ERR_INVALID;
        if (d.in_t > 64 || (d.in_t & 3) != 0) return NSFF_ERR_INVALID;
        k.in_xyz = d.in_xyz; k.in_t = d.in_t; k.t_rows = jb.t_rows; k.out = jb.out;
        k.table = jb.table; k.ts = reinterpret_cast<const long long*>(jb.ts); k.n_table = jb.n_table; k.max_t = jb.max_t;
        k.delta = jb.delta; k.rows_out = jb.t_rows ? nullptr : jb.rows_out;
        const uint32_t skips = nsff_skip_layers(&d);
        int i = 0;
        for (int l = 0; l < d.D; ++l) {
            if (l != 0 && !((skips >> l) & 1u)) continue;
            k.w[i] = jb.w[i]; k.b[i] = jb.b[i];
            if (!k.w[i] || !k.b[i]) return NSFF_ERR_NULL;
            k.ld[i] = d.in_xyz + d.in_t + (l ? NSFF_W : 0);
            ++i;
        }
        max_rows = std::max(max_rows, k.rows);
    }
    const long long gx = (n_rays + TB_RAYS - 1) / TB_RAYS;
    if (gx > 0x7fffffffLL) return NSFF_ERR_INVALID;
    hipLaunchKernelGGL(nsff_time_bias_kernel, dim3((unsigned)gx, (unsigned)max_rows, (unsigned)n_jobs), dim3(256), 0,
                       reinterpret_cast<hipStream_t>(stream), a);
    return nsff_launch_status();
}

namespace {
struct SideBiasArgs { const float* w; const float* b; const float* dir_rows; const float* a_rows; float* out;
                      int in_dir, in_a, ld; long long n_rays; };
__global__ __launch_bounds__(256) void nsff_side_bias_kernel(const SideBiasArgs a) {
    const int n = threadIdx.x;
    const long long r0 = (long long)blockIdx.x * TB_RAYS;
    const int in = a.in_dir + a.in_a;
    __shared__ __attribute__((aligned(16))) float st[TB_RAYS][NSFF_W];
    __shared__ float sw[16][NSFF_W + 1];
    for (int e = threadIdx.x; e < TB_RAYS * NSFF_W; e += 256) {
        const int r = e >> 8, c = e & 255;
        const long long ray = r0 + r < a.n_rays ? r0 + r : a.n_rays - 1;
        float v = 0.f;
        if (c < a.in_dir) v = a.dir_rows[ray * a.in_dir + c];
        else if (c < in) v = a.a_rows[ray * a.in_a + (c - a.in_dir)];
        st[r][c] = v;
    }
    float acc[TB_RAYS];
    const float b = a.b[n];
#pragma unroll
    for (int r = 0; r < TB_RAYS; ++r) acc[r] = b;
    const float* __restrict__ wl = a.w + NSFF_W;
    for (int c0 = 0; c0 < in; c0 += 16) {
        __syncthreads();
#pragma unroll
        for (int k = 0; k < 16; ++k) {
            const int e = threadIdx.x + 256 * k, row = e >> 4, c = c0 + (e & 15);
            sw[e & 15][row] = c < in ? wl[(long long)row * a.ld + c] : 0.f;
        }
        __syncthreads();
#pragma unroll
        for (int u = 0; u < 16; u += 4) {
            const float w0 = sw[u][n], w1 = sw[u + 1][n], w2 = sw[u + 2][n], w3 = sw[u + 3][n];
#pragma unroll
            for (int r = 0; r < TB_RAYS; ++r) {
                const float4 t4 = *reinterpret_cast<const float4*>(&st[r][c0 + u]);
                acc[r] = fmaf(w3, t4.w, fmaf(w2, t4.z, fmaf(w1, t4.y, fmaf(w0, t4.x, acc[r]))));
            }
        }
    }
#pragma unroll
    for (int r = 0; r < TB_RAYS; ++r)
        if (r0 + r < a.n_rays) a.out[(r0 + r) * NSFF_W + n] = acc[r];
}
}

extern "C" int nsff_side_bias(const NsffModelDesc* desc, const void* packed_f16x3, const float* w_dir, const float* dir_rows,
                              const float* a_rows, int64_t n_rays, float* out, void* stream) {
    if (!desc || !packed_f16x3 || !w_dir || !dir_rows || !out) return NSFF_ERR_NULL;
    const NsffModelDesc& d = *desc;
    NsffLayoutH3 L;
    const int rc = nsff_make_layout_h3(d, L);
    if (rc) return rc;
    if (!d.use_viewdir || d.in_dir < 1 || n_rays < 0) return NSFF_ERR_INVALID;
    if (d.in_a > 0 && !a_rows) return NSFF_ERR_NULL;
    if (n_rays == 0) return NSFF_OK;
    SideBiasArgs a{};
    a.w = w_dir; a.b = reinterpret_cast<const float*>(packed_f16x3) + L.dir_b_fold;
    a.dir_rows = dir_rows; a.a_rows = a_rows; a.out = out;
    a.in_dir = d.in_dir; a.in_a = d.in_a; a.ld = NSFF_W + d.in_dir + d.in_a; a.n_rays = n_rays;
    const long long gx = (n_rays + TB_RAYS - 1) / TB_RAYS;
    if (gx > 0x7fffffffLL) return NSFF_ERR_INVALID;
    hipLaunchKernelGGL(nsff_side_bias_kernel, dim3((unsigned)gx), dim3(256), 0, reinterpret_cast<hipStream_t>(stream), a);
    return nsff_launch_status();
}

int g_nsff_last_h3_kernel = 0;
static int h3a_device_cus() {
    static int cus[64];
    int dev = 0;
    if (hipGetDevice(&dev) != hipSuccess || dev < 0 || dev >= 64) return 0;
    if (cus[dev] == 0) {
        int n = 0;
        cus[dev] = (hipDeviceGetAttribute(&n, hipDeviceAttributeMultiprocessorCount, dev) == hipSuccess && n > 0) ? n : -1;
    }
    return cus[dev] > 0 ? cus[dev] : 0;
}

int g_nsff_last_h3_grid = 0;

namespace {
struct SideTileArgs { const float* dir_emb; const float* a_emb; _Float16* out; long long n_points; int pts_per_ray, in_dir, in_a, side_rows;
                     uint32_t* range; };
__global__ __launch_bounds__(256) void nsff_side_tile_kernel(const SideTileArgs a) {
    const long long tile = blockIdx.x, p0 = tile * 64;
    const int lane = threadIdx.x & 63, rblocks = a.side_rows >> 5;
    _Float16* dst = a.out + tile * (64LL * a.side_rows);
    float rm = 0.f;
    for (int blk = threadIdx.x >> 6; blk < 4 * rblocks; blk += 4) {
        const int ks = blk / rblocks, rb = blk % rblocks;
        const int row = 32 * rb + (lane & 31), pt0 = 16 * ks + 8 * (lane >> 5);
        h8 out;
#pragma unroll
        for (int t = 0; t < 8; ++t) {
            const long long p = p0 + pt0 + t;
            float v = 0.f;
            if (p < a.n_points) {
                const long long ray = p / a.pts_per_ray;
                if (row < a.in_dir) v = a.dir_emb[ray * a.in_dir + row];
                else if (row < a.in_dir + a.in_a) v = a.a_emb[ray * a.in_a + (row - a.in_dir)];
            }
            rm = nsff_absmax3(rm, v, v);
            out[t] = (_Float16)v;
        }
        *reinterpret_cast<h8*>(dst + (((long long)ks * rblocks + rb) * 64 + lane) * 8) = out;
    }
    nsff_range_flag(a.range, rm, NSFF_RANGE_CODES, (unsigned)lane);
}
}

int nsff_h3_field_query(const NsffModelDesc* desc, const void* packed, const NsffFieldArgs* args,
                        int points_per_block, hipStream_t st, unsigned long long* span) {
    const NsffModelDesc& d = *desc;
    const NsffFieldArgs& g = *args;
    g_nsff_last_h3_grid = 0;
    H3KArgs k{};
    const int rc = nsff_make_layout_h3(d, k.L);
    if (rc) return rc;
    if (g.xyz && 3 + 6 * g.n_freqs != d.in_xyz) return NSFF_ERR_INVALID;
    k.packed = reinterpret_cast<const uint32_t*>(packed);
    k.span = span;
    k.range = nsff_range_word(st);
    k.xyz = g.xyz; k.x_emb = g.x_emb; k.dir_emb = g.dir_emb; k.a_emb = g.a_emb; k.t_emb = g.t_emb;
    k.raw = g.raw; k.n_points = g.n_points; k.pts_per_ray = g.pts_per_ray;
    k.save_acts = reinterpret_cast<_Float16*>(g.save_acts);
    k.save_xin = reinterpret_cast<_Float16*>(g.save_xin);
    k.save_masks = reinterpret_cast<unsigned long long*>(g.save_masks);
    k.save_side = reinterpret_cast<_Float16*>(g.save_side);
    k.n_tiles = (g.n_points + 63) / 64;
    k.save_stride = k.n_tiles * 64 * NSFF_W;
    if ((g.save_acts || g.save_xin || g.save_masks || g.save_side) && !g.xyz) return NSFF_ERR_INVALID;
    const void* const lo_of[3] = {g.save_acts, g.save_xin, g.save_side};
    bool save_lo = false;
    for (int i = 0; i < 3; ++i) {
        if (g.save_lo_delta[i] < 0 || (g.save_lo_delta[i] & 7) || (g.save_lo_delta[i] != 0 && !lo_of[i])) return NSFF_ERR_INVALID;
        k.lo_delta[i] = g.save_lo_delta[i];
        save_lo = save_lo || g.save_lo_delta[i] != 0;
    }
    k.xin_rows = (k.L.k0s + k.L.kt) <= 128 ? 128 : 256;
    k.side_rows = k.L.side_k <= 128 ? 128 : 256;
    k.static_mode = g.static_mode; k.transient_mode = g.transient_mode;
    k.D = d.D; k.skip = d.skip;
    k.in_xyz = d.in_xyz; k.in_dir = d.in_dir; k.in_a = d.in_a; k.in_t = d.in_t;
    k.use_viewdir = d.use_viewdir; k.flow_scale = d.flow_scale;
    k.n_freqs = g.n_freqs;
    for (int i = 0; i < NSFF_MAX_FREQS; ++i) k.freqs[i] = g.freqs[i];
    k.octave_freqs = (g.xyz != nullptr && g.n_freqs >= 1 && g.n_freqs <= 10 && k.L.k0s == 64) ? 1 : 0;
    for (int i = 0; i + 1 < g.n_freqs; ++i)
        if (g.freqs[i + 1] != 2.0f * g.freqs[i]) k.octave_freqs = 0;
    k.ld_emb = g.ld_emb; k.off_xyz = g.off_xyz; k.off_dir = g.off_dir; k.off_a = g.off_a; k.off_t = g.off_t;
// ... 175 lines not shown
```

nsff_pl_amd/csrc/rays.hip:

```cpp
#include <hip/hip_runtime.h>
#include <cstdlib>
#include "nsff_common.h"

namespace {

constexpr int WAVES_PER_BLOCK = 4;
constexpr int RS = NSFF_RAW_STRIDE;

__device__ __forceinline__ float wave_sum(float v) {
#pragma unroll
    for (int off = 32; off > 0; off >>= 1) v += __shfl_xor(v, off);
    return v;
}

__device__ __forceinline__ float wave_scan_mul(float v, int lane) {
#pragma unroll
    for (int off = 1; off < 64; off <<= 1) {
        const float u = __shfl_up(v, off);
        if (lane >= off) v *= u;
    }
    return v;
}
__device__ __forceinline__ float wave_scan_add(float v, int lane) {
#pragma unroll
    for (int off = 1; off < 64; off <<= 1) {
        const float u = __shfl_up(v, off);
        if (lane >= off) v += u;
    }
    return v;
}

__device__ __forceinline__ float softplus(float x) { return x > 20.f ? x : log1pf(expf(x)); }

__global__ void coarse_samples_kernel(const float* __restrict__ rays, long long n_rays,
                                      const float* __restrict__ z_lin, int S, float perturb,
                                      const float* __restrict__ rnd, float* __restrict__ zs,
                                      float* __restrict__ xyz) {
    const long long idx = (long long)blockIdx.x * blockDim.x + threadIdx.x;
    if (idx >= n_rays * S) return;
    const long long n = idx / S;
    const int i = (int)(idx - n * S);
    float z = z_lin[i];
    if (perturb > 0.f) {
        const float lower = i > 0 ? 0.5f * (z_lin[i - 1] + z_lin[i]) : z_lin[0];
        const float upper = i < S - 1 ? 0.5f * (z_lin[i] + z_lin[i + 1]) : z_lin[S - 1];
        z = lower + (upper - lower) * (perturb * rnd[idx]);
    }
    zs[idx] = z;
    const float* r = rays + n * 6;
#pragma unroll
    for (int c = 0; c < 3; ++c) xyz[idx * 3 + c] = r[c] + r[3 + c] * z;
}

__device__ __forceinline__ void sample_pdf_ray(const float* w, const float* bins, int M, float eps,
                                               const float* u, int n_imp, float* cdf,
                                               float* out_a, float* out_b, int lane, bool active) {
    float part = 0.f;
    for (int j = lane; j < M; j += 64) part += (active ? w[j] : 0.f) + eps;
    const float total = wave_sum(part);
    float carry = 0.f;
    if (lane == 0) cdf[0] = 0.f;
    for (int base = 0; base < M; base += 64) {
        const int j = base + lane;
        const float pdf = j < M ? ((active ? w[j] : 0.f) + eps) / total : 0.f;
        const float inc = wave_scan_add(pdf, lane) + carry;
        if (j < M) cdf[j + 1] = inc;
        carry = __shfl(inc, 63);
    }
    __syncthreads();
    for (int k = lane; k < n_imp; k += 64) {
        const float uk = active ? u[k] : 0.f;
        int lo = 0, hi = M + 1;
        while (lo < hi) {
            const int mid = (lo + hi) >> 1;
            if (cdf[mid] <= uk) lo = mid + 1; else hi = mid;
        }
        const int below = max(lo - 1, 0), above = min(lo, M);
        const float cb = cdf[below], ca = cdf[above];
        const float bb = bins[below], ba = bins[above];
        float denom = ca - cb;
        if (denom < eps) denom = 1.f;
        const float s = bb + (uk - cb) / denom * (ba - bb);
        if (active) {
            if (out_a) out_a[k] = s;
            if (out_b) out_b[k] = s;
        }
    }
    __syncthreads();
}

struct FineArgs {
    const float* rays; long long n_rays; const float* z_lin; const float* zs_coarse;
    int S, n_imp;
    const float* w_static; const float* w_transient;
    const float* u_static; const float* u_transient; int u_per_ray;
    float* samples_static; float* samples_transient;
    float* zs_fine; float* xyz_fine;
};

__global__ __launch_bounds__(64 * WAVES_PER_BLOCK) void fine_samples_kernel(const FineArgs a) {
    extern __shared__ __attribute__((aligned(16))) float smem[];
    const int lane = threadIdx.x & 63, wave = threadIdx.x >> 6, tid = threadIdx.x;
    constexpr int T = 64 * WAVES_PER_BLOCK;
    const long long ray = blockIdx.x;
    const int S = a.S, n_imp = a.n_imp;
    const int k_sets = a.w_transient ? 2 : 1;
    const int Sf = S + k_sets * n_imp;
    float* cdf = smem + wave * S;
    float* bins = smem + WAVES_PER_BLOCK * S;
    float* merged = bins + ((S + 3) & ~3);
    for (int j = tid; j < S - 1; j += T) bins[j] = 0.5f * (a.z_lin[j] + a.z_lin[j + 1]);
    for (int j = tid; j < S; j += T) merged[j] = a.zs_coarse[ray * S + j];
    __syncthreads();
    {
        const bool mine = wave < k_sets;
        const int set = mine ? wave : 0;
        const float* w = (set == 0 ? a.w_static : a.w_transient) + ray * S + 1;
        const float* ub = set == 0 ? a.u_static : a.u_transient;
        const float* u = a.u_per_ray ? ub + ray * n_imp : ub;
        float* keep = set == 0 ? a.samples_static : a.samples_transient;
        sample_pdf_ray(w, bins, S - 2, 1e-5f, u, n_imp, cdf, merged + S + set * n_imp,
                       keep ? keep + ray * n_imp : nullptr, lane, mine);
    }
    const float* r = a.rays + ray * 6;
    const float o0 = r[0], o1 = r[1], o2 = r[2], d0 = r[3], d1 = r[4], d2 = r[5];
    for (int i = tid; i < Sf; i += T) {
        const float v = merged[i];
        int rank = 0;
        int j = 0;
        for (; j + 4 <= Sf; j += 4) {
            const float4 o = *reinterpret_cast<const float4*>(merged + j);
            rank += (o.x < v || (o.x == v && j < i)) ? 1 : 0;
            rank += (o.y < v || (o.y == v && j + 1 < i)) ? 1 : 0;
            rank += (o.z < v || (o.z == v && j + 2 < i)) ? 1 : 0;
            rank += (o.w < v || (o.w == v && j + 3 < i)) ? 1 : 0;
        }
        for (; j < Sf; ++j) {
            const float o = merged[j];
            rank += (o < v || (o == v && j < i)) ? 1 : 0;
        }
        const long long dst = ray * Sf + rank;
        a.zs_fine[dst] = v;
        a.xyz_fine[dst * 3 + 0] = o0 + d0 * v;
        a.xyz_fine[dst * 3 + 1] = o1 + d1 * v;
        a.xyz_fine[dst * 3 + 2] = o2 + d2 * v;
    }
}

struct PdfArgs {
    const float* bins; const float* weights; long long n_rays; int M;
    const float* u; int n_imp; int u_per_ray; float eps; float* samples;
};

__global__ __launch_bounds__(64 * WAVES_PER_BLOCK) void sample_pdf_kernel(const PdfArgs a) {
    extern __shared__ __attribute__((aligned(16))) float smem[];
    const int lane = threadIdx.x & 63, wave = threadIdx.x >> 6;
    const long long ray_raw = (long long)blockIdx.x * WAVES_PER_BLOCK + wave;
    const bool active = ray_raw < a.n_rays;
    const long long ray = active ? ray_raw : a.n_rays - 1;
    float* cdf = smem + wave * (a.M + 1);
    const float* u = a.u_per_ray ? a.u + ray * a.n_imp : a.u;
    sample_pdf_ray(a.weights + ray * a.M, a.bins + ray * (a.M + 1), a.M, a.eps, u, a.n_imp, cdf,
                   active ? a.samples + ray * a.n_imp : nullptr, nullptr, lane, true);
}

struct FrameRayArgs {
    float fx, fy, cx, cy;
    float c2w[12];
    int W;
    float near, shift_near;
    long long first, count;
    float* rays;
};

__global__ void frame_rays_kernel(const FrameRayArgs a) {
    const long long idx = (long long)blockIdx.x * blockDim.x + threadIdx.x;
    if (idx >= a.count) return;
    const long long pix = a.first + idx;
    const float i = (float)(pix % a.W), j = (float)(pix / a.W);
    const float dc[3] = {(i - a.cx) / a.fx, -(j - a.cy) / a.fy, -1.0f};
    float d[3];
#pragma unroll
    for (int r = 0; r < 3; ++r) d[r] = dc[0] * a.c2w[4 * r + 0] + dc[1] * a.c2w[4 * r + 1] + dc[2] * a.c2w[4 * r + 2];
    const float nrm = sqrtf(d[0] * d[0] + d[1] * d[1] + d[2] * d[2]);
#pragma unroll
    for (int r = 0; r < 3; ++r) d[r] /= nrm;
    float o[3] = {a.c2w[3], a.c2w[7], a.c2w[11]};
    const float t = -(a.shift_near + o[2]) / d[2];
#pragma unroll
    for (int r = 0; r < 3; ++r) o[r] = o[r] + t * d[r];
    const float ox_oz = o[0] / o[2], oy_oz = o[1] / o[2];
    const float sx = -1.0f / (a.cx / a.fx), sy = -1.0f / (a.cy / a.fy);
    const float o2 = 1.0f + 2.0f * a.near / o[2];
    float* r = a.rays + idx * 6;
    r[0] = sx * ox_oz;
    r[1] = sy * oy_oz;
    r[2] = o2;
    r[3] = sx * (d[0] / d[2] - ox_oz);
    r[4] = sy * (d[1] / d[2] - oy_oz);
    r[5] = 1.0f - o2;
}

__global__ void warp_points_kernel(const float* __restrict__ raw, const float* __restrict__ xyz,
                                   const float* __restrict__ zs, long long n_points, float z_far,
                                   float* __restrict__ xyz_fw, float* __restrict__ xyz_bw) {
    const long long idx = (long long)blockIdx.x * blockDim.x + threadIdx.x;
    if (idx >= n_points * 3) return;
    const long long p = idx / 3;
    const int c = (int)(idx - p * 3);
    const bool far = zs[p] > z_far;
    const float x = xyz[idx];
    xyz_fw[idx] = x + (far ? 0.f : raw[p * RS + 8 + c]);
    xyz_bw[idx] = x + (far ? 0.f : raw[p * RS + 11 + c]);
}

__device__ __forceinline__ float frustum_count(const NsffFrustumArgs& v, float x, float y, float z) {
    const float fx = v.K4[0], fy = v.K4[1], cx = v.K4[2], cy = v.K4[3];
    const float rz = 2.0f / (z - 1.0f - 1e-6f);
    const float rx = -rz * x * cx / fx;
    const float ry = -rz * y * cy / fy;
    const long long frame = v.ts[0];
    float count = 0.f;
    if (frame < 0 || frame >= v.n_frames) return count;
    for (int c = 0; c < v.n_cams; ++c) {
        const float* m = v.w2c + ((long long)c * v.n_frames + frame) * 12;
        const float cam0 = fmaf(m[2], rz, fmaf(m[1], ry, m[0] * rx)) + m[3];
        const float cam1 = fmaf(m[6], rz, fmaf(m[5], ry, m[4] * rx)) + m[7];
        const float cam2 = fmaf(m[10], rz, fmaf(m[9], ry, m[8] * rx)) + m[11];
        if (!(cam2 < 0.f)) continue;
        const float c1 = -cam1, c2 = -cam2;
        const float u = fmaf(cx, c2, fx * cam0) / c2, w = fmaf(cy, c2, fy * c1) / c2;
        if (u >= 0.f && u < (float)v.W && w >= 0.f && w < (float)v.H) count += 1.f;
    }
    return count;
}

__global__ __launch_bounds__(256) void frustum_visibility_kernel(const NsffFrustumArgs v, const float* __restrict__ xyz,
                                                                 long long n_points, float* __restrict__ out) {
    const long long p = (long long)blockIdx.x * 256 + threadIdx.x;
    if (p < n_points) out[p] = frustum_count(v, xyz[3 * p], xyz[3 * p + 1], xyz[3 * p + 2]);
}

__global__ __launch_bounds__(64 * WAVES_PER_BLOCK) void composite_kernel(const NsffCompositeArgs a) {
    const int lane = threadIdx.x & 63;
    const long long ray = (long long)blockIdx.x * WAVES_PER_BLOCK + (threadIdx.x >> 6);
    if (ray >= a.n_rays) return;
    const int S = a.n_samples;
    const bool tr = a.has_transient != 0;
    const bool flows = tr && a.flow_mode >= 1;
    const bool warps = tr && a.flow_mode >= 2;

    float cT = 1.f, cTs = 1.f, cTfw = 1.f, cTbw = 1.f;
    float s_depth = 0.f, s_rgb[3] = {0, 0, 0}, s_talpha = 0.f, s_trgb[3] = {0, 0, 0};
    float s_sorgb[3] = {0, 0, 0}, s_sodepth = 0.f;
    float s_xyz[3] = {0, 0, 0}, s_ffw[3] = {0, 0, 0}, s_fbw[3] = {0, 0, 0};
    float s_rgbfw[3] = {0, 0, 0}, s_rgbbw[3] = {0, 0, 0}, s_occfw = 0.f, s_occbw = 0.f;

    for (int base = 0; base < S; base += 64) {
        const int i = base + lane;
        const bool on = i < S;
        const long long idx = ray * S + (on ? i : S - 1);
        const float z = a.zs[idx];
        const bool last = i >= S - 1;
        const float dz = last ? 0.f : a.zs[idx + 1] - z;
        const float d_s = last ? 100.f : dz;
        const float d_t = last ? 1e-3f : dz;
        const float* rec = a.raw + idx * RS;

        float sig_s = rec[3];
        if (a.noise_static) sig_s += a.noise_static[idx] * a.noise_std;
        sig_s = softplus(sig_s);
        const float al_s = 1.f - expf(-d_s * sig_s);
        float rgb_s[3] = {0, 0, 0};
        if (a.has_rgb) { rgb_s[0] = rec[0]; rgb_s[1] = rec[1]; rgb_s[2] = rec[2]; }

        float sig_t = 0.f, al_t = 0.f, alpha = al_s;
        float rgb_t[3] = {0, 0, 0};
        if (tr) {
            sig_t = rec[7];
            if (a.visibility && a.visibility[idx] == 0.f) sig_t = -10.f;
            if (a.vis.w2c && frustum_count(a.vis, a.xyz[idx * 3], a.xyz[idx * 3 + 1], a.xyz[idx * 3 + 2]) == 0.f) sig_t = -10.f;
            if (a.noise_transient) sig_t += a.noise_transient[idx] * a.noise_std;
            sig_t = softplus(sig_t);
            al_t = 1.f - expf(-d_t * sig_t);
            alpha = 1.f - (1.f - al_s) * (1.f - al_t);
            if (a.has_rgb) { rgb_t[0] = rec[4]; rgb_t[1] = rec[5]; rgb_t[2] = rec[6]; }
        }
        const float om = on ? 1.f - alpha : 1.f;
        const float inc = wave_scan_mul(om, lane);
        float exc = __shfl_up(inc, 1);
        if (lane == 0) exc = 1.f;
        const float T = cT * exc;
        cT *= __shfl(inc, 63);
        const float w = alpha * T, w_s = al_s * T, w_t = al_t * T;

        if (on) {
            if (a.static_sigmas) a.static_sigmas[idx] = sig_s;
            if (a.has_rgb && a.static_rgbs) {
                a.static_rgbs[idx * 3 + 0] = rgb_s[0]; a.static_rgbs[idx * 3 + 1] = rgb_s[1];
                a.static_rgbs[idx * 3 + 2] = rgb_s[2];
            }
            if (tr) {
                if (a.transient_sigmas) a.transient_sigmas[idx] = sig_t;
                if (a.has_rgb && a.transient_rgbs) {
                    a.transient_rgbs[idx * 3 + 0] = rgb_t[0]; a.transient_rgbs[idx * 3 + 1] = rgb_t[1];
                    a.transient_rgbs[idx * 3 + 2] = rgb_t[2];
                }
                if (a.static_alphas) a.static_alphas[idx] = al_s;
                if (a.transient_alphas) a.transient_alphas[idx] = al_t;
                if (a.static_weights) a.static_weights[idx] = w_s;
                if (a.transient_weights) a.transient_weights[idx] = w_t;
                if (a.weights) a.weights[idx] = w;
            } else {
                if (a.static_weights) a.static_weights[idx] = w;
                if (a.weights) a.weights[idx] = w;
            }
        }
        if (!a.has_rgb) continue;

        if (on) {
            s_depth += w * z;
            if (tr) {
#pragma unroll
                for (int c = 0; c < 3; ++c) { s_rgb[c] += w_s * rgb_s[c]; s_trgb[c] += w_t * rgb_t[c]; }
                s_talpha += w_t;
            } else {
#pragma unroll
                for (int c = 0; c < 3; ++c) s_rgb[c] += w * rgb_s[c];
            }
        }
        if (!tr) continue;

        {
            const float oms = on ? 1.f - al_s : 1.f;
            const float incs = wave_scan_mul(oms, lane);
            float excs = __shfl_up(incs, 1);
            if (lane == 0) excs = 1.f;
            const float Ts = cTs * excs;
            cTs *= __shfl(incs, 63);
            const float wso = al_s * Ts;
            if (on) {
#pragma unroll
                for (int c = 0; c < 3; ++c) s_sorgb[c] += wso * rgb_s[c];
                s_sodepth += wso * z;
            }
        }
        if (!flows) continue;

        const bool far = z > a.z_far;
        float ffw[3], fbw[3], x[3];
#pragma unroll
        for (int c = 0; c < 3; ++c) {
            ffw[c] = far ? 0.f : rec[8 + c];
            fbw[c] = far ? 0.f : rec[11 + c];
            x[c] = a.xyz[idx * 3 + c];
        }
        if (on) {
#pragma unroll
            for (int c = 0; c < 3; ++c) {
                if (a.flows_fw) a.flows_fw[idx * 3 + c] = ffw[c];
                if (a.flows_bw) a.flows_bw[idx * 3 + c] = fbw[c];
                s_xyz[c] += w * x[c]; s_ffw[c] += w * ffw[c]; s_fbw[c] += w * fbw[c];
            }
        }
        if (!warps) continue;

#pragma unroll
        for (int dir = 0; dir < 2; ++dir) {
            const float* recw = (dir == 0 ? a.raw_fw : a.raw_bw) + idx * RS;
            const float* nz = dir == 0 ? a.noise_fw : a.noise_bw;
            float sg = recw[7];
            if (nz) sg += nz[idx] * a.noise_std;
            const float al_tw = 1.f - expf(-d_t * softplus(sg));
            const float al_w = 1.f - (1.f - al_s) * (1.f - al_tw);
            const float omw = on ? 1.f - al_w : 1.f;
            const float incw = wave_scan_mul(omw, lane);
            float excw = __shfl_up(incw, 1);
            if (lane == 0) excw = 1.f;
            float& cw = dir == 0 ? cTfw : cTbw;
            const float Tw = cw * excw;
            cw *= __shfl(incw, 63);
            const float ws_w = al_s * Tw, wt_w = al_tw * Tw;
            if (on) {
                float* srgb = dir == 0 ? s_rgbfw : s_rgbbw;
#pragma unroll
                for (int c = 0; c < 3; ++c) srgb[c] += ws_w * rgb_s[c] + wt_w * recw[4 + c];
                const float* xw = (dir == 0 ? a.xyz_fw : a.xyz_bw) + idx * 3;
                float* cyc = dir == 0 ? a.xyzs_fw_bw : a.xyzs_bw_fw;
                const int head = dir == 0 ? 11 : 8;
                if (cyc) {
#pragma unroll
                    for (int c = 0; c < 3; ++c) cyc[idx * 3 + c] = xw[c] + (far ? 0.f : recw[head + c]);
                }
                const float occ = wt_w - w_t;
                if (dir == 0) { s_occfw += occ; if (a.disoccs_fw) a.disoccs_fw[idx] = 1.f - fabsf(occ); }
                else          { s_occbw += occ; if (a.disoccs_bw) a.disoccs_bw[idx] = 1.f - fabsf(occ); }
            }
        }
    }
    if (!a.has_rgb) return;

    s_depth = wave_sum(s_depth);
#pragma unroll
    for (int c = 0; c < 3; ++c) s_rgb[c] = wave_sum(s_rgb[c]);
    if (tr) {
        s_talpha = wave_sum(s_talpha); s_sodepth = wave_sum(s_sodepth);
#pragma unroll
        for (int c = 0; c < 3; ++c) { s_trgb[c] = wave_sum(s_trgb[c]); s_sorgb[c] = wave_sum(s_sorgb[c]); }
    }
    if (flows) {
#pragma unroll
        for (int c = 0; c < 3; ++c) { s_xyz[c] = wave_sum(s_xyz[c]); s_ffw[c] = wave_sum(s_ffw[c]); s_fbw[c] = wave_sum(s_fbw[c]); }
    }
    if (warps) {
        s_occfw = wave_sum(s_occfw); s_occbw = wave_sum(s_occbw);
#pragma unroll
        for (int c = 0; c < 3; ++c) { s_rgbfw[c] = wave_sum(s_rgbfw[c]); s_rgbbw[c] = wave_sum(s_rgbbw[c]); }
    }
    if (lane != 0) return;
    if (a.depth) a.depth[ray] = s_depth;
    if (!tr) {
        if (a.rgb) for (int c = 0; c < 3; ++c) a.rgb[ray * 3 + c] = s_rgb[c];
        return;
    }
    for (int c = 0; c < 3; ++c) {
        if (a.rgb) a.rgb[ray * 3 + c] = s_rgb[c] + s_trgb[c];
        if (a.transient_rgb) a.transient_rgb[ray * 3 + c] = s_trgb[c] + 0.8f * (1.f - s_talpha);
        if (a.static_only_rgb) a.static_only_rgb[ray * 3 + c] = s_sorgb[c];
    }
    if (a.transient_alpha) a.transient_alpha[ray] = s_talpha;
    if (a.static_only_depth) a.static_only_depth[ray] = s_sodepth;
    if (flows) {
        for (int c = 0; c < 3; ++c) {
            if (a.xyz_exp) a.xyz_exp[ray * 3 + c] = s_xyz[c];
            if (a.flow_fw_exp) a.flow_fw_exp[ray * 3 + c] = s_ffw[c];
            if (a.flow_bw_exp) a.flow_bw_exp[ray * 3 + c] = s_fbw[c];
            if (a.xyz_fw_exp) a.xyz_fw_exp[ray * 3 + c] = s_xyz[c] + s_ffw[c];
            if (a.xyz_bw_exp) a.xyz_bw_exp[ray * 3 + c] = s_xyz[c] + s_fbw[c];
        }
    }
    if (warps) {
        for (int c = 0; c < 3; ++c) {
            if (a.rgb_fw) a.rgb_fw[ray * 3 + c] = s_rgbfw[c];
            if (a.rgb_bw) a.rgb_bw[ray * 3 + c] = s_rgbbw[c];
        }
        if (a.disocc_fw) a.disocc_fw[ray] = 1.f - fabsf(s_occfw);
        if (a.disocc_bw) a.disocc_bw[ray] = 1.f - fabsf(s_occbw);
    }
}

template <int NCH>
__global__ __launch_bounds__(64 * NCH) void composite_kernel_chunks(const NsffCompositeArgs a) {
    __shared__ float tot[NCH][4];
    __shared__ float part[NCH][32];
    const int lane = threadIdx.x & 63, c = threadIdx.x >> 6;
    const long long ray = blockIdx.x;
    const int S = a.n_samples;
    const bool tr = a.has_transient != 0;
    const bool flows = tr && a.flow_mode >= 1;
    const bool warps = tr && a.flow_mode >= 2;

    const int i = 64 * c + lane;
    const bool on = i < S;
    const long long idx = ray * S + (on ? i : S - 1);
    const float z = a.zs[idx];
    const bool last = i >= S - 1;
    const float dz = last ? 0.f : a.zs[idx + 1] - z;
    const float d_s = last ? 100.f : dz;
    const float d_t = last ? 1e-3f : dz;
    const float* rec = a.raw + idx * RS;

    float sig_s = rec[3];
    if (a.noise_static) sig_s += a.noise_static[idx] * a.noise_std;
    sig_s = softplus(sig_s);
    const float al_s = 1.f - expf(-d_s * sig_s);
    float rgb_s[3] = {0, 0, 0};
    if (a.has_rgb) { rgb_s[0] = rec[0]; rgb_s[1] = rec[1]; rgb_s[2] = rec[2]; }

    float sig_t = 0.f, al_t = 0.f, alpha = al_s;
    float rgb_t[3] = {0, 0, 0};
    if (tr) {
        sig_t = rec[7];
        if (a.visibility && a.visibility[idx] == 0.f) sig_t = -10.f;
        if (a.vis.w2c && frustum_count(a.vis, a.xyz[idx * 3], a.xyz[idx * 3 + 1], a.xyz[idx * 3 + 2]) == 0.f) sig_t = -10.f;
        if (a.noise_transient) sig_t += a.noise_transient[idx] * a.noise_std;
        sig_t = softplus(sig_t);
        al_t = 1.f - expf(-d_t * sig_t);
        alpha = 1.f - (1.f - al_s) * (1.f - al_t);
        if (a.has_rgb) { rgb_t[0] = rec[4]; rgb_t[1] = rec[5]; rgb_t[2] = rec[6]; }
    }
    const float inc = wave_scan_mul(on ? 1.f - alpha : 1.f, lane);
    float incs = 1.f, incw[2] = {1.f, 1.f}, al_tw[2] = {0.f, 0.f};
    if (a.has_rgb && tr) incs = wave_scan_mul(on ? 1.f - al_s : 1.f, lane);
    if (a.has_rgb && warps) {
#pragma unroll
        for (int dir = 0; dir < 2; ++dir) {
            const float* recw = (dir == 0 ? a.raw_fw : a.raw_bw) + idx * RS;
            const float* nz = dir == 0 ? a.noise_fw : a.noise_bw;
            float sg = recw[7];
            if (nz) sg += nz[idx] * a.noise_std;
            al_tw[dir] = 1.f - expf(-d_t * softplus(sg));
            const float al_w = 1.f - (1.f - al_s) * (1.f - al_tw[dir]);
            incw[dir] = wave_scan_mul(on ? 1.f - al_w : 1.f, lane);
        }
    }
    if (lane == 63) { tot[c][0] = inc; tot[c][1] = incs; tot[c][2] = incw[0]; tot[c][3] = incw[1]; }
    __syncthreads();
    float cT = 1.f, cTs = 1.f, cTw[2] = {1.f, 1.f};
    for (int cc = 0; cc < c; ++cc) { cT *= tot[cc][0]; cTs *= tot[cc][1]; cTw[0] *= tot[cc][2]; cTw[1] *= tot[cc][3]; }

    float exc = __shfl_up(inc, 1);
    if (lane == 0) exc = 1.f;
    const float T = cT * exc;
    const float w = alpha * T, w_s = al_s * T, w_t = al_t * T;
    if (on) {
        if (a.static_sigmas) a.static_sigmas[idx] = sig_s;
        if (a.has_rgb && a.static_rgbs) {
            a.static_rgbs[idx * 3 + 0] = rgb_s[0]; a.static_rgbs[idx * 3 + 1] = rgb_s[1];
            a.static_rgbs[idx * 3 + 2] = rgb_s[2];
        }
        if (tr) {
            if (a.transient_sigmas) a.transient_sigmas[idx] = sig_t;
            if (a.has_rgb && a.transient_rgbs) {
                a.transient_rgbs[idx * 3 + 0] = rgb_t[0]; a.transient_rgbs[idx * 3 + 1] = rgb_t[1];
                a.transient_rgbs[idx * 3 + 2] = rgb_t[2];
            }
            if (a.static_alphas) a.static_alphas[idx] = al_s;
            if (a.transient_alphas) a.transient_alphas[idx] = al_t;
            if (a.static_weights) a.static_weights[idx] = w_s;
            if (a.transient_weights) a.transient_weights[idx] = w_t;
            if (a.weights) a.weights[idx] = w;
        } else {
            if (a.static_weights) a.static_weights[idx] = w;
            if (a.weights) a.weights[idx] = w;
        }
    }
    if (!a.has_rgb) return;

    enum { P_DEPTH, P_RGB, P_TRGB = P_RGB + 3, P_TALPHA = P_TRGB + 3, P_SORGB, P_SODEPTH = P_SORGB + 3, P_XYZ, P_FFW = P_XYZ + 3,
           P_FBW = P_FFW + 3, P_RGBFW = P_FBW + 3, P_RGBBW = P_RGBFW + 3, P_OCCFW = P_RGBBW + 3, P_OCCBW, P_N };
    static_assert(P_N <= 32, "part[] columns");
    float p[P_N];
#pragma unroll
    for (int k = 0; k < P_N; ++k) p[k] = 0.f;
    if (on) {
        p[P_DEPTH] = w * z;
        if (tr) {
#pragma unroll
            for (int k = 0; k < 3; ++k) { p[P_RGB + k] = w_s * rgb_s[k]; p[P_TRGB + k] = w_t * rgb_t[k]; }
            p[P_TALPHA] = w_t;
        } else {
#pragma unroll
            for (int k = 0; k < 3; ++k) p[P_RGB + k] = w * rgb_s[k];
        }
    }
    if (tr) {
        float excs = __shfl_up(incs, 1);
        if (lane == 0) excs = 1.f;
        const float wso = al_s * (cTs * excs);
        if (on) {
#pragma unroll
            for (int k = 0; k < 3; ++k) p[P_SORGB + k] = wso * rgb_s[k];
            p[P_SODEPTH] = wso * z;
        }
    }
    if (flows) {
        const bool far = z > a.z_far;
        float ffw[3], fbw[3], x[3];
#pragma unroll
        for (int k = 0; k < 3; ++k) {
            ffw[k] = far ? 0.f : rec[8 + k];
            fbw[k] = far ? 0.f : rec[11 + k];
            x[k] = a.xyz[idx * 3 + k];
        }
        if (on) {
#pragma unroll
            for (int k = 0; k < 3; ++k) {
                if (a.flows_fw) a.flows_fw[idx * 3 + k] = ffw[k];
                if (a.flows_bw) a.flows_bw[idx * 3 + k] = fbw[k];
                p[P_XYZ + k] = w * x[k]; p[P_FFW + k] = w * ffw[k]; p[P_FBW + k] = w * fbw[k];
            }
        }
        if (warps) {
#pragma unroll
            for (int dir = 0; dir < 2; ++dir) {
                const float* recw = (dir == 0 ? a.raw_fw : a.raw_bw) + idx * RS;
                float excw = __shfl_up(incw[dir], 1);
                if (lane == 0) excw = 1.f;
                const float Tw = cTw[dir] * excw;
                const float ws_w = al_s * Tw, wt_w = al_tw[dir] * Tw;
                if (on) {
#pragma unroll
                    for (int k = 0; k < 3; ++k) p[(dir == 0 ? P_RGBFW : P_RGBBW) + k] = ws_w * rgb_s[k] + wt_w * recw[4 + k];
                    const float* xw = (dir == 0 ? a.xyz_fw : a.xyz_bw) + idx * 3;
                    float* cyc = dir == 0 ? a.xyzs_fw_bw : a.xyzs_bw_fw;
                    const int head = dir == 0 ? 11 : 8;
                    if (cyc) {
#pragma unroll
                        for (int k = 0; k < 3; ++k) cyc[idx * 3 + k] = xw[k] + (far ? 0.f : recw[head + k]);
                    }
                    const float occ = wt_w - w_t;
                    if (dir == 0) { p[P_OCCFW] = occ; if (a.disoccs_fw) a.disoccs_fw[idx] = 1.f - fabsf(occ); }
                    else          { p[P_OCCBW] = occ; if (a.disoccs_bw) a.disoccs_bw[idx] = 1.f - fabsf(occ); }
                }
            }
        }
    }
    const int n_used = warps ? (int)P_N : (flows ? (int)P_RGBFW : (tr ? (int)P_XYZ : (int)P_TRGB));
#pragma unroll
    for (int k = 0; k < P_N; ++k) {
        if (k < n_used) {
            const float v = wave_sum(p[k]);
            if (lane == 0) part[c][k] = v;
        }
    }
    __syncthreads();
    if (threadIdx.x != 0) return;
    float s[P_N];
#pragma unroll
    for (int k = 0; k < P_N; ++k) {
        s[k] = 0.f;
        if (k < n_used) for (int cc = 0; cc < NCH; ++cc) s[k] += part[cc][k];
    }
    if (a.depth) a.depth[ray] = s[P_DEPTH];
    if (!tr) {
        if (a.rgb) for (int k = 0; k < 3; ++k) a.rgb[ray * 3 + k] = s[P_RGB + k];
        return;
    }
    for (int k = 0; k < 3; ++k) {
        if (a.rgb) a.rgb[ray * 3 + k] = s[P_RGB + k] + s[P_TRGB + k];
        if (a.transient_rgb) a.transient_rgb[ray * 3 + k] = s[P_TRGB + k] + 0.8f * (1.f - s[P_TALPHA]);
        if (a.static_only_rgb) a.static_only_rgb[ray * 3 + k] = s[P_SORGB + k];
    }
    if (a.transient_alpha) a.transient_alpha[ray] = s[P_TALPHA];
    if (a.static_only_depth) a.static_only_depth[ray] = s[P_SODEPTH];
    if (flows) {
        for (int k = 0; k < 3; ++k) {
            if (a.xyz_exp) a.xyz_exp[ray * 3 + k] = s[P_XYZ + k];
            if (a.flow_fw_exp) a.flow_fw_exp[ray * 3 + k] = s[P_FFW + k];
            if (a.flow_bw_exp) a.flow_bw_exp[ray * 3 + k] = s[P_FBW + k];
            if (a.xyz_fw_exp) a.xyz_fw_exp[ray * 3 + k] = s[P_XYZ + k] + s[P_FFW + k];
            if (a.xyz_bw_exp) a.xyz_bw_exp[ray * 3 + k] = s[P_XYZ + k] + s[P_FBW + k];
        }
    }
    if (warps) {
        for (int k = 0; k < 3; ++k) {
            if (a.rgb_fw) a.rgb_fw[ray * 3 + k] = s[P_RGBFW + k];
            if (a.rgb_bw) a.rgb_bw[ray * 3 + k] = s[P_RGBBW + k];
        }
        if (a.disocc_fw) a.disocc_fw[ray] = 1.f - fabsf(s[P_OCCFW]);
        if (a.disocc_bw) a.disocc_bw[ray] = 1.f - fabsf(s[P_OCCBW]);
    }
}

__global__ __launch_bounds__(256) void time_rows_kernel(const float* __restrict__ table, long long n_table, int width,
                                                         const long long* __restrict__ ts, long long n, long long max_t,
                                                         float* __restrict__ next, float* __restrict__ prev, int vec) {
    const int per_row = vec ? width / 4 : width;
    const long long i = (long long)blockIdx.x * 256 + threadIdx.x;
    if (i >= n * per_row) return;
    const long long r = i / per_row;
    const int c = (int)(i - r * per_row);
    const long long t = ts[r];
    long long tn = t + 1 < max_t ? t + 1 : max_t, tp = t - 1 > 0 ? t - 1 : 0;
    tn = tn < 0 ? 0 : (tn > n_table - 1 ? n_table - 1 : tn);
    tp = tp > n_table - 1 ? n_table - 1 : tp;
    if (vec) {
        if (next) reinterpret_cast<float4*>(next)[i] = reinterpret_cast<const float4*>(table + tn * width)[c];
        if (prev) reinterpret_cast<float4*>(prev)[i] = reinterpret_cast<const float4*>(table + tp * width)[c];
    } else {
        if (next) next[i] = table[tn * width + c];
        if (prev) prev[i] = table[tp * width + c];
    }
}

constexpr int TRB_CHUNK = 2048;
constexpr int TRB_COLS = 4;
__global__ __launch_bounds__(256) void time_rows_bwd_kernel(const float* __restrict__ g_cur, const float* __restrict__ g_next,
                                                             const float* __restrict__ g_prev, const long long* __restrict__ ts,
                                                             long long n, long long max_t, long long n_table, int width,
                                                             float* __restrict__ d_table) {
    __shared__ int sList[3][TRB_CHUNK];
    __shared__ int sTs[TRB_CHUNK];
    __shared__ int sCnt[3];
    __shared__ float sPart[4][64];
    const long long r = blockIdx.x;
    const int lane = threadIdx.x & 63, part = threadIdx.x >> 6;
    const float* gs[3] = {g_cur, g_next, g_prev};
    for (int cg = 0; cg < width; cg += 64 * TRB_COLS) {
        float acc[TRB_COLS];
#pragma unroll
        for (int j = 0; j < TRB_COLS; ++j) acc[j] = 0.f;
        for (long long base = 0; base < n; base += TRB_CHUNK) {
            const long long end = base + TRB_CHUNK < n ? base + TRB_CHUNK : n;
            for (long long i = base + threadIdx.x; i < end; i += 256) {
                const long long t = ts[i];
                sTs[i - base] = (int)(t < -2 ? -2 : (t > 0x7ffffff0LL ? 0x7ffffff0LL : t));
            }
            __syncthreads();
            if (part == 0) {
                int cnt[3] = {0, 0, 0};
                for (long long i0 = base; i0 < end; i0 += 64) {
                    const long long i = i0 + lane;
                    bool hit[3] = {false, false, false};
                    if (i < end) {
                        const long long t = sTs[i - base];
                        long long tn = t + 1 < max_t ? t + 1 : max_t, tp = t - 1 > 0 ? t - 1 : 0;
                        tn = tn < 0 ? 0 : (tn > n_table - 1 ? n_table - 1 : tn);
                        tp = tp > n_table - 1 ? n_table - 1 : tp;
                        hit[0] = t == r; hit[1] = tn == r; hit[2] = tp == r;
                    }
#pragma unroll
                    for (int l = 0; l < 3; ++l) {
                        const unsigned long long m = __ballot(hit[l] && gs[l] != nullptr);
                        if (hit[l] && gs[l] != nullptr) sList[l][cnt[l] + __popcll(m & ((1ull << lane) - 1ull))] = (int)(i - base);
                        cnt[l] += __popcll(m);
                    }
                }
                if (lane == 0) { sCnt[0] = cnt[0]; sCnt[1] = cnt[1]; sCnt[2] = cnt[2]; }
            }
            __syncthreads();
#pragma unroll
            for (int l = 0; l < 3; ++l) {
                const float* __restrict__ g = gs[l];
                const int cnt = sCnt[l];
                for (int k0 = part; k0 < cnt; k0 += 16) {
                    float v[4][TRB_COLS];
#pragma unroll
                    for (int u = 0; u < 4; ++u) {
                        const int k = k0 + 4 * u;
                        const float* row = g + (base + sList[l][k < cnt ? k : k0]) * width + cg + lane;
#pragma unroll
                        for (int j = 0; j < TRB_COLS; ++j)
                            v[u][j] = (k < cnt && cg + 64 * j + lane < width) ? row[64 * j] : 0.f;
                    }
#pragma unroll
                    for (int u = 0; u < 4; ++u)
#pragma unroll
                        for (int j = 0; j < TRB_COLS; ++j) acc[j] += v[u][j];
                }
            }
            __syncthreads();
        }
#pragma unroll
        for (int j = 0; j < TRB_COLS; ++j) {
            const int c = cg + 64 * j + lane;
            if (cg + 64 * j >= width) break;
            sPart[part][lane] = acc[j];
            __syncthreads();
            if (part == 0 && c < width) d_table[r * width + c] = (sPart[0][lane] + sPart[1][lane]) + (sPart[2][lane] + sPart[3][lane]);
            __syncthreads();
        }
    }
}

}

extern "C" {

int nsff_time_rows_backward(const float* g_cur, const float* g_next, const float* g_prev, const int64_t* ts, int64_t n,
                            int64_t max_t, int64_t n_table, int32_t width, float* d_table, void* stream) {
    if (n < 0 || n_table < 1 || n_table > 0x7fffffffLL || width < 1) return NSFF_ERR_INVALID;
    if (!d_table || (n > 0 && !ts)) return NSFF_ERR_NULL;
    hipLaunchKernelGGL(time_rows_bwd_kernel, dim3((unsigned)n_table), dim3(256), 0, (hipStream_t)stream, g_cur, g_next, g_prev,
                       reinterpret_cast<const long long*>(ts), (long long)n, (long long)max_t, (long long)n_table, (int)width,
                       d_table);
    return nsff_launch_status();
}

int nsff_time_rows(const float* table, int64_t n_table, int32_t width, const int64_t* ts, int64_t n, int64_t max_t,
                   float* next, float* prev, void* stream) {
    if (n < 0 || n_table < 1 || width < 1) return NSFF_ERR_INVALID;
    if (n == 0 || (!next && !prev)) return NSFF_OK;
    if (!table || !ts) return NSFF_ERR_NULL;
    const int vec = (width % 4 == 0) && !(((uintptr_t)table | (uintptr_t)next | (uintptr_t)prev) & 15);
    const long long total = n * (vec ? width / 4 : width);
    hipLaunchKernelGGL(time_rows_kernel, dim3((unsigned)((total + 255) / 256)), dim3(256), 0, (hipStream_t)stream, table,
                       (long long)n_table, (int)width, reinterpret_cast<const long long*>(ts), (long long)n, (long long)max_t,
                       next, prev, vec);
    return nsff_launch_status();
}


int nsff_coarse_samples(const float* rays, int64_t n_rays, const float* z_lin, int32_t n_samples,
                        float perturb, const float* perturb_rand, float* zs, float* xyz, void* stream) {
    if (n_rays < 0 || n_samples < 1) return NSFF_ERR_INVALID;
    if (n_rays == 0) return NSFF_OK;
    if (!rays || !z_lin || !zs || !xyz) return NSFF_ERR_NULL;
    if (perturb > 0.f && !perturb_rand) return NSFF_ERR_NULL;
    const long long total = (long long)n_rays * n_samples;
    hipLaunchKernelGGL(coarse_samples_kernel, dim3((unsigned)((total + 255) / 256)), dim3(256), 0,
                       (hipStream_t)stream, rays, (long long)n_rays, z_lin, n_samples, perturb,
                       perturb_rand, zs, xyz);
    return nsff_launch_status();
}

int nsff_fine_samples(const float* rays, int64_t n_rays, const float* z_lin, const float* zs_coarse,
                      int32_t n_samples, int32_t n_importance,
                      const float* weights_static, const float* weights_transient,
                      const float* u_static, const float* u_transient, int32_t u_per_ray,
                      float* samples_static, float* samples_transient,
                      float* zs_fine, float* xyz_fine, void* stream) {
    if (n_rays < 0 || n_samples < 3 || n_importance < 1) return NSFF_ERR_INVALID;
    if (n_rays == 0) return NSFF_OK;
    if (!rays || !z_lin || !zs_coarse || !weights_static || !u_static || !zs_fine || !xyz_fine) return NSFF_ERR_NULL;
    if (weights_transient && !u_transient) return NSFF_ERR_NULL;
    FineArgs a{rays, (long long)n_rays, z_lin, zs_coarse, n_samples, n_importance,
               weights_static, weights_transient, u_static, u_transient, u_per_ray,
               samples_static, samples_transient, zs_fine, xyz_fine};
    const int Sf = n_samples + (weights_transient ? 2 : 1) * n_importance;
    const size_t lds = (size_t)(WAVES_PER_BLOCK * n_samples + ((n_samples + 3) & ~3) + Sf) * sizeof(float);
    if (lds > 64 * 1024 || n_rays > 0x7fffffffLL) return NSFF_ERR_INVALID;
    const unsigned blocks = (unsigned)n_rays;
    hipLaunchKernelGGL(fine_samples_kernel, dim3(blocks), dim3(64 * WAVES_PER_BLOCK), lds,
                       (hipStream_t)stream, a);
    return nsff_launch_status();
}

int nsff_sample_pdf(const float* bins, const float* weights, int64_t n_rays, int32_t n_bins_minus1,
                    const float* u, int32_t n_importance, int32_t u_per_ray, float eps,
                    float* samples, void* stream) {
    if (n_rays < 0 || n_bins_minus1 < 1 || n_importance < 1) return NSFF_ERR_INVALID;
    if (n_rays == 0) return NSFF_OK;
    if (!bins || !weights || !u || !samples) return NSFF_ERR_NULL;
    PdfArgs a{bins, weights, (long long)n_rays, n_bins_minus1, u, n_importance, u_per_ray, eps, samples};
    const size_t lds = (size_t)WAVES_PER_BLOCK * (n_bins_minus1 + 1) * sizeof(float);
    if (lds > 64 * 1024) return NSFF_ERR_INVALID;
    const unsigned blocks = (unsigned)((n_rays + WAVES_PER_BLOCK - 1) / WAVES_PER_BLOCK);
    hipLaunchKernelGGL(sample_pdf_kernel, dim3(blocks), dim3(64 * WAVES_PER_BLOCK), lds,
                       (hipStream_t)stream, a);
    return nsff_launch_status();
}

int nsff_warp_points(const float* raw, const float* xyz, const float* zs, int64_t n_points,
                     float z_far, float* xyz_fw, float* xyz_bw, void* stream) {
    if (n_points < 0) return NSFF_ERR_INVALID;
    if (n_points == 0) return NSFF_OK;
    if (!raw || !xyz || !zs || !xyz_fw || !xyz_bw) return NSFF_ERR_NULL;
    const long long total = (long long)n_points * 3;
    hipLaunchKernelGGL(warp_points_kernel, dim3((unsigned)((total + 255) / 256)), dim3(256), 0,
                       (hipStream_t)stream, raw, xyz, zs, (long long)n_points, z_far, xyz_fw, xyz_bw);
    return nsff_launch_status();
}

int nsff_frame_rays(const float* K4_host, const float* c2w_host, int32_t H, int32_t W, float near, float shift_near,
                    int64_t first_pixel, int64_t n_pixels, float* rays, void* stream) {
    if (!K4_host || !c2w_host) return NSFF_ERR_NULL;
    if (H < 1 || W < 1 || first_pixel < 0 || n_pixels < 0 || first_pixel + n_pixels > (int64_t)H * W) return NSFF_ERR_INVALID;
    if (n_pixels == 0) return NSFF_OK;
    if (!rays) return NSFF_ERR_NULL;
    FrameRayArgs a{};
    a.fx = K4_host[0]; a.fy = K4_host[1]; a.cx = K4_host[2]; a.cy = K4_host[3];
    for (int i = 0; i < 12; ++i) a.c2w[i] = c2w_host[i];
    a.W = W; a.near = near; a.shift_near = shift_near; a.first = first_pixel; a.count = n_pixels; a.rays = rays;
    hipLaunchKernelGGL(frame_rays_kernel, dim3((unsigned)((n_pixels + 255) / 256)), dim3(256), 0, (hipStream_t)stream, a);
    return nsff_launch_status();
}

int nsff_composite(const NsffCompositeArgs* args, void* stream) {
    if (!args) return NSFF_ERR_NULL;
    const NsffCompositeArgs& a = *args;
    if (a.n_rays < 0 || a.n_samples < 1 || a.flow_mode < 0 || a.flow_mode > 2) return NSFF_ERR_INVALID;
    if (a.n_rays == 0) return NSFF_OK;
    if (!a.raw || !a.zs) return NSFF_ERR_NULL;
    if (a.flow_mode && (!a.has_transient || !a.has_rgb)) return NSFF_ERR_INVALID;
    if (a.flow_mode >= 1 && !a.xyz) return NSFF_ERR_NULL;
    if (a.flow_mode == 2 && (!a.raw_fw || !a.raw_bw || !a.xyz_fw || !a.xyz_bw)) return NSFF_ERR_NULL;
    if (a.vis.w2c && (!a.vis.ts || !a.xyz)) return NSFF_ERR_NULL;
    if (a.vis.w2c && (a.vis.n_cams < 1 || a.vis.n_frames < 1)) return NSFF_ERR_INVALID;
    const int nch = (a.n_samples + 63) / 64;
    if (nch >= 2 && nch <= 4 && a.n_rays <= 0x7fffffffLL && getenv("NSFF_SERIAL_COMPOSITE") == nullptr) {
        const dim3 grid((unsigned)a.n_rays);
        if (nch == 2) hipLaunchKernelGGL(composite_kernel_chunks<2>, grid, dim3(128), 0, (hipStream_t)stream, a);
        else if (nch == 3) hipLaunchKernelGGL(composite_kernel_chunks<3>, grid, dim3(192), 0, (hipStream_t)stream, a);
        else hipLaunchKernelGGL(composite_kernel_chunks<4>, grid, dim3(256), 0, (hipStream_t)stream, a);
        return nsff_launch_status();
    }
    const unsigned blocks = (unsigned)((a.n_rays + WAVES_PER_BLOCK - 1) / WAVES_PER_BLOCK);
    hipLaunchKernelGGL(composite_kernel, dim3(blocks), dim3(64 * WAVES_PER_BLOCK), 0,
                       (hipStream_t)stream, a);
    return nsff_launch_status();
}

int nsff_frustum_visibility(const NsffFrustumArgs* vis, const float* xyz, int64_t n_points, float* vis_count,
                            void* stream) {
    if (!vis || !vis->w2c || !vis->ts) return NSFF_ERR_NULL;
    if (n_points < 0 || vis->n_cams < 1 || vis->n_frames < 1) return NSFF_ERR_INVALID;
    if (n_points == 0) return NSFF_OK;
    if (!xyz || !vis_count) return NSFF_ERR_NULL;
    const long long blocks = (n_points + 255) / 256;
    if (blocks > 0x7fffffffLL) return NSFF_ERR_INVALID;
    hipLaunchKernelGGL(frustum_visibility_kernel, dim3((unsigned)blocks), dim3(256), 0, (hipStream_t)stream, *vis, xyz,
                       (long long)n_points, vis_count);
    return nsff_launch_status();
}

}
```

nsff_pl_amd/csrc/rng.hip:

```cpp
#include <hip/hip_runtime.h>
#include <hiprand/hiprand_kernel.h>
#include <cstdint>

#include "../../include/nsff_render.h"
#include "nsff_common.h"

namespace {

struct RngArgs {
    NsffRngJob job[NSFF_MAX_RNG_JOBS];
    unsigned first_block[NSFF_MAX_RNG_JOBS + 1];
    int n;
    unsigned long long seed;
    NsffRngCoarse coarse;
};

__device__ __forceinline__ void coarse_from_draw(const NsffRngCoarse& c, long long idx, float rnd) {
#pragma clang fp contract(off)
    const int S = c.n_samples;
    const long long n = idx / S;
    const int i = (int)(idx - n * S);
    const float* __restrict__ z_lin = c.z_lin;
    const float lower = i > 0 ? 0.5f * (z_lin[i - 1] + z_lin[i]) : z_lin[0];
    const float upper = i < S - 1 ? 0.5f * (z_lin[i] + z_lin[i + 1]) : z_lin[S - 1];
    const float t = c.perturb * rnd;
    const float span = upper - lower;
    const float z = lower + span * t;
    c.zs[idx] = z;
    const float* r = c.rays + n * 6;
#pragma unroll
    for (int k = 0; k < 3; ++k) { const float dz = r[3 + k] * z; c.xyz[idx * 3 + k] = r[k] + dz; }
}

__global__ __launch_bounds__(256) void nsff_rng_kernel(const RngArgs a) {
    int j = 0;
    while (j + 1 < a.n && blockIdx.x >= a.first_block[j + 1]) ++j;
    const NsffRngJob& J = a.job[j];
    const long long idx = (long long)(blockIdx.x - a.first_block[j]) * 256 + threadIdx.x;
    hiprandStatePhilox4_32_10_t state;
    hiprand_init(a.seed, (unsigned long long)idx, J.offset, &state);
    const long long stride = 256LL * J.grid, numel = J.numel;
    const long long rounded = ((numel - 1) / (stride * 4) + 1) * (stride * 4);
    for (long long li = idx; li < rounded; li += stride * 4) {
        const float4 r = J.kind ? hiprand_normal4(&state) : hiprand_uniform4(&state);
        const float v[4] = {r.x, r.y, r.z, r.w};
#pragma unroll
        for (int ii = 0; ii < 4; ++ii) {
            const long long l = li + stride * ii;
            if (l < numel) {
                const float x = v[ii] * 1.0f + 0.0f;
                const float y = J.kind ? x : (x == 1.0f ? 0.0f : x);
                if (J.out) J.out[l] = y;
                if (j == a.coarse.job) coarse_from_draw(a.coarse, l, y);
            }
        }
    }
}

}

extern "C" int nsff_rng_draws(const NsffRngJob* jobs, int32_t n_jobs, uint64_t seed, void* stream) {
    return nsff_rng_draws_coarse(jobs, n_jobs, seed, nullptr, stream);
}

extern "C" int nsff_rng_draws_coarse(const NsffRngJob* jobs, int32_t n_jobs, uint64_t seed, const NsffRngCoarse* coarse, void* stream) {
    if (n_jobs == 0) return coarse ? NSFF_ERR_INVALID : NSFF_OK;
    if (!jobs) return NSFF_ERR_NULL;
    if (n_jobs < 0 || n_jobs > NSFF_MAX_RNG_JOBS) return NSFF_ERR_INVALID;
    RngArgs a{};
    a.coarse.job = -1;
    if (coarse) {
        const NsffRngCoarse& c = *coarse;
        if (c.job < 0 || c.job >= n_jobs || c.n_samples < 1 || !(c.perturb > 0.f)) return NSFF_ERR_INVALID;
        if (!c.rays || !c.z_lin || !c.zs || !c.xyz) return NSFF_ERR_NULL;
        if (jobs[c.job].kind != 0 || jobs[c.job].numel % c.n_samples != 0) return NSFF_ERR_INVALID;
        a.coarse = c;
    }
    unsigned total = 0;
    for (int j = 0; j < n_jobs; ++j) {
        const NsffRngJob& J = jobs[j];
        if (!J.out && j != a.coarse.job) return NSFF_ERR_NULL;
        if (J.numel <= 0 || J.grid == 0 || (J.kind != 0 && J.kind != 1) || (J.offset & 3ull)) return NSFF_ERR_INVALID;
        if ((long long)J.grid > (J.numel + 255) / 256 || total + J.grid < total) return NSFF_ERR_INVALID;
        a.job[j] = J;
        a.first_block[j] = total;
        total += J.grid;
    }
    a.first_block[n_jobs] = total;
    a.n = n_jobs;
    a.seed = seed;
    hipLaunchKernelGGL(nsff_rng_kernel, dim3(total), dim3(256), 0, (hipStream_t)stream, a);
    const hipError_t e = hipGetLastError();
    return e == hipSuccess ? NSFF_OK : nsff_hip_fail(e);
}
```

nsff_pl_amd/rendering.py:

```python
import os

import torch

from . import _lib
from . import autograd
from . import config
from . import range_check
from . import field_grad
from . import ray_geometry

Z_FAR = 0.95

def _new(ref, *shape):
    return torch.empty(*shape, device=ref.device, dtype=torch.float32)


def sample_pdf(bins, weights, N_importance, det=False, eps=1e-5):
    _lib.require_gpu_tensor(bins, "sample_pdf bins")
    bins = bins.contiguous().float()
    weights = weights.contiguous().float()
    n_rays = weights.shape[0]
    if det:
        u = torch.linspace(0, 1, N_importance, device=bins.device)
    else:
        u = torch.rand(n_rays, N_importance, device=bins.device)
    out = _new(bins, n_rays, N_importance)
    if n_rays:
        _lib.sample_pdf(bins, weights, u.contiguous(), 0 if det else 1, eps, out)
    return out


_TORCH_RAND, _TORCH_RANDN = torch.rand, torch.randn


class _Draws:

    def __init__(self, device, n_rays, N_samples, N_importance, perturb, noise_std, test_time, models, kwargs, coarse=None):
        self.device = device
        self.coarse_done = False
        self.fused = (device.type == "cuda" and torch.rand is _TORCH_RAND and torch.randn is _TORCH_RANDN
                      and not os.environ.get("NSFF_TORCH_RNG") and not torch.cuda.is_current_stream_capturing()
                      and _lib.fused_draws_match_torch(device))
        self.at = 0
        if not self.fused:
            return
        first = models["coarse"] if N_importance > 0 else models["fine"]
        transient = bool(kwargs.get("output_transient", True) and first.encode_transient)
        flows = kwargs.get("output_transient_flow", []) if transient else []
        noisy = float(noise_std) != 0
        plan, need = [], []

        def add(kind, need_values, *shape):
            plan.append((kind, shape))
            need.append(bool(need_values))
        hook = None
        if perturb > 0:
            add("rand", coarse is None, n_rays, N_samples)
            if coarse is not None and n_rays:
                hook = (coarse[0], coarse[1], float(perturb), coarse[2], coarse[3])
        S = N_samples
        if N_importance > 0:
            add("randn", noisy, n_rays, S)
            if transient:
                add("randn", noisy, n_rays, S)
            if perturb != 0:
                add("rand", True, n_rays, N_importance)
                if transient:
                    add("rand", True, n_rays, N_importance)
            S = N_samples + (2 if transient else 1) * N_importance
        add("randn", noisy, n_rays, S)
        if transient:
            add("randn", noisy, n_rays, S)
            if flows and not test_time:
                add("randn", noisy, n_rays, S)
                add("randn", noisy, n_rays, S)
        self.plan = plan
        self.values = _lib.fused_draws(plan, device, need, coarse=hook)
        self.coarse_done = hook is not None

    def take(self, kind, *shape):
        if not self.fused:
            return (torch.rand if kind == "rand" else torch.randn)(*shape, device=self.device)
        if self.at >= len(self.plan) or self.plan[self.at] != (kind, shape):
            raise RuntimeError(f"draw {self.at}: {kind}{shape} is not the planned {self.plan[self.at:self.at + 1]}")
        self.at += 1
        return self.values[self.at - 1]


class _Pass:
    __slots__ = ("embeddings", "rays", "ts", "max_t", "noise_std", "test_time", "kwargs",
                 "freqs_xyz", "dir_embedded", "n_rays", "rec", "tbias", "neighbour_rows", "draws")


def _embed_rows(embeddings, key, idx):
    return embeddings[key](idx).detach().contiguous().float()


_LINSPACE = {}


def _unit_linspace(n, device):
    key = (int(n), str(device))
    if key not in _LINSPACE:
        if len(_LINSPACE) > 64:
            _LINSPACE.clear()
        _LINSPACE[key] = torch.linspace(0, 1, n, device=device)
    return _LINSPACE[key]


def _neighbour_time_rows(embeddings, ts, max_t):
    m = embeddings['t']
    if (isinstance(m, torch.nn.Embedding) and m.padding_idx is None and m.max_norm is None and m.weight.is_cuda
            and m.weight.dtype == torch.float32 and m.weight.is_contiguous() and ts.is_cuda and ts.dtype == torch.int64):
        return _lib.time_rows(m.weight.detach(), ts.contiguous(), max_t)
    return (_embed_rows(embeddings, 't', torch.clamp(ts + 1, max=max_t)),
            _embed_rows(embeddings, 't', torch.clamp(ts - 1, min=0)))


def _time_codes(ctx, models, kwargs, N_samples, N_importance, output_transient, flows):
    ctx.tbias, ctx.neighbour_rows = {}, None
    if not output_transient:
        return None
    n_rays, ts, m = ctx.n_rays, ctx.ts, ctx.embeddings.get('t')
    override = kwargs.get('t_embedded') if 't_embedded' in kwargs else None
    plan = []
    if not (ctx.rec is not None or n_rays == 0 or config.get_precision() != "f16x3" or config.get_tile_points() not in (0, 130)):
        passes = [('coarse', N_samples), ('fine', N_samples + 2 * N_importance)] if N_importance > 0 else [('fine', N_samples)]
        for typ, S in passes:
            model = models[typ]
            if not model.encode_transient or S % 64 or (n_rays * S < 32768 and config.get_tile_points() == 0):
                continue
            if model.in_channels_t > 64 or model.in_channels_t % 4:
                continue
            if typ == 'fine' and flows and not ctx.test_time and hasattr(model, "transient_flow_fw"):
                plan += [(typ, 'fw', model, 1), (typ, 'bw', model, -1)]
            plan.append((typ, 't', model, 0))
    plain = (override is None and isinstance(m, torch.nn.Embedding) and m.padding_idx is None and m.max_norm is None
             and m.weight.is_cuda and m.weight.dtype == torch.float32 and m.weight.is_contiguous()
             and torch.is_tensor(ts) and ts.is_cuda and ts.dtype == torch.int64
             and ts.dim() == 1 and ts.shape[0] == n_rays)
    if (plan and plain and all(mod.in_channels_t == m.weight.shape[1] for _, _, mod, _ in plan)
            and not os.environ.get('NSFF_NO_TIME_INDEX')):
        outs, rows = _lib.time_bias([(mod, d) for _, _, mod, d in plan], index=(m.weight.detach(), ts.contiguous(), ctx.max_t))
        for (typ, which, _, _), out in zip(plan, outs):
            ctx.tbias[(typ, which)] = out
        if 1 in rows:
            ctx.neighbour_rows = (rows[1], rows[-1])
        return rows[0]
    t_embedded = override if override is not None else ctx.embeddings['t'](ts)
    t_embedded = t_embedded.detach().contiguous().float()
    plan = [p for p in plan if t_embedded.shape == (n_rays, p[2].in_channels_t)]
    if plan:
        if any(w == 'fw' for _, w, _, _ in plan):
            ctx.neighbour_rows = _neighbour_time_rows(ctx.embeddings, ts, ctx.max_t)
        src = {0: t_embedded, 1: ctx.neighbour_rows[0] if ctx.neighbour_rows else None, -1: ctx.neighbour_rows[1] if ctx.neighbour_rows else None}
        for (typ, which, _, _), out in zip(plan, _lib.time_bias([(mod, src[d]) for _, _, mod, d in plan])):
            ctx.tbias[(typ, which)] = out
    return t_embedded


def _inference(results, ctx, model, xyz, zs, output_transient, output_transient_flow,
               t_embedded, a_embedded):
    typ = model.typ
    n_rays, S = zs.shape
    test_time = ctx.test_time
    results[f'zs_{typ}'] = zs
    results[f'xyzs_{typ}'] = xyz
    P = n_rays * S
    sigma_only = typ == 'coarse' and test_time
    want_flow = bool(output_transient_flow) and output_transient and not sigma_only
    warps = want_flow and not test_time
    disocc = warps and 'disocc' in output_transient_flow
    if want_flow and not hasattr(model, "transient_flow_fw"):
        raise AttributeError(f"{typ} model has no flow heads")

    raw = _new(zs, P, _lib.RAW_STRIDE)
    side = dict(dir_emb=ctx.dir_embedded if model.use_viewdir and not sigma_only else None,
                a_emb=a_embedded if (model.use_viewdir and model.in_channels_a > 0 and not sigma_only) else None)
    big_enough = ctx.rec is not None or config.get_tile_points() == 130 or (config.get_tile_points() == 0 and P >= 32768)
    if (side["dir_emb"] is not None and P and S % 64 == 0 and config.get_precision() == "f16x3" and config.get_tile_points() in (0, 130)
            and big_enough and not os.environ.get('NSFF_NO_SIDE_BIAS')):
        side["s_bias"] = _lib.side_bias(model, side["dir_emb"], side["a_emb"])

    def query(tag, raw_out, pts, static_mode, transient_mode, flow_heads, t_rows, which='t', **extra):
        saves = {}
        if ctx.rec is not None and field_grad.forward_can_save(model, static_mode, transient_mode):
            x3 = config.grad_x3()
            acts, xin, masks, side_rows = field_grad.alloc_saves(model, P, zs.device, bool(transient_mode), bool(static_mode), x3)
            saves = dict(save_acts=acts, save_xin=xin, save_masks=masks, save_side=side_rows, save_lo=x3)
            ctx.rec.setdefault("saved", {})[tag] = (raw_out, acts, xin, masks, pts.view(-1, 3), side_rows, x3)
        t_bias = ctx.tbias.get((typ, which)) if (transient_mode and not saves) else None
        _lib.field_query(model, raw_out, P, S, static_mode=static_mode, transient_mode=transient_mode,
                         flow_heads=flow_heads, xyz=pts, freqs=ctx.freqs_xyz, t_emb=t_rows, t_bias=t_bias, **saves, **extra)
    if P:
        query(typ, raw, xyz, 1 if sigma_only else 2, 0 if not output_transient else (1 if sigma_only else 2),
              2 if want_flow else 0, t_embedded if output_transient else None, **side)

    vis = None
    if test_time and output_transient and 'dataset' in ctx.kwargs and P:
        vis = ray_geometry.frustum_args(ctx.kwargs['dataset'], ctx.ts, zs.device)

    nstd = float(ctx.noise_std)
    noise_s = ctx.draws.take("randn", n_rays, S)
    noise_t = ctx.draws.take("randn", n_rays, S) if output_transient else None
    if ctx.rec is not None and nstd != 0:
        ctx.rec[f"{typ}_static"], ctx.rec[f"{typ}_transient"] = noise_s, noise_t

    args = dict(n_rays=n_rays, n_samples=S, has_transient=int(output_transient),
                has_rgb=int(not sigma_only), flow_mode=0, want_disocc=int(disocc),
                noise_std=nstd, z_far=Z_FAR, raw=raw, zs=zs, xyz=xyz, vis=vis,
                noise_static=noise_s if nstd != 0 else None,
                noise_transient=noise_t if (nstd != 0 and output_transient) else None)

    def out(key, *shape):
        t = _new(zs, *shape)
        results[key] = t
        return t

    if not sigma_only:
        args['static_rgbs'] = out(f'static_rgbs_{typ}', n_rays, S, 3)
        if output_transient:
            args['transient_rgbs'] = out(f'transient_rgbs_{typ}', n_rays, S, 3)
            if want_flow:
                args['flows_fw'] = out('transient_flows_fw', n_rays, S, 3)
                args['flows_bw'] = out('transient_flows_bw', n_rays, S, 3)
    args['static_sigmas'] = out(f'static_sigmas_{typ}', n_rays, S)
    if output_transient:
        args['transient_sigmas'] = out(f'transient_sigmas_{typ}', n_rays, S)

    if warps:
        ts = ctx.ts
        xyz_w = _new(zs, 2, n_rays, S, 3)
        xyz_fw, xyz_bw = xyz_w[0], xyz_w[1]
        results['xyzs_fw'] = xyz_fw
        raw_w = _new(zs, 2 * P, _lib.RAW_STRIDE)
        raw_fw, raw_bw = raw_w[:P], raw_w[P:]
        tp1, tm1 = ctx.neighbour_rows if ctx.neighbour_rows is not None else _neighbour_time_rows(ctx.embeddings, ts, ctx.max_t)
        tb_fw, tb_bw = ctx.tbias.get((typ, 'fw')), ctx.tbias.get((typ, 'bw'))
        def halves(a, b):
            return (a.untyped_storage().data_ptr() == b.untyped_storage().data_ptr()
                    and a.data_ptr() + a.numel() * 4 == b.data_ptr())
        merged = (ctx.rec is None and P > 0 and not os.environ.get('NSFF_NO_MERGED_REQUERY') and halves(tp1, tm1)
                  and (tb_fw is None) == (tb_bw is None) and (tb_fw is None or halves(tb_fw, tb_bw)))
        if P:
            _lib.warp_points(raw, xyz, zs, Z_FAR, xyz_fw, xyz_bw)
            if merged:
                ctx.tbias[(typ, 'fwbw')] = None if tb_fw is None else torch.as_strided(tb_fw, (2 * n_rays,) + tuple(tb_fw.shape[1:]),
                                                                                         tb_fw.stride())
                _lib.field_query(model, raw_w, 2 * P, S, static_mode=0, transient_mode=2, flow_heads=1, xyz=xyz_w,
                                 freqs=ctx.freqs_xyz, t_emb=torch.as_strided(tp1, (2 * n_rays, tp1.shape[1]), tp1.stride()),
                                 t_bias=ctx.tbias[(typ, 'fwbw')])
            else:
                query(f"{typ}_warp_fw", raw_fw, xyz_fw, 0, 2, 1, tp1, which='fw')
        noise_fw = ctx.draws.take("randn", n_rays, S)
        out('rgb_fw', n_rays, 3)
        results['xyzs_bw'] = xyz_bw
        if P and not merged:
            query(f"{typ}_warp_bw", raw_bw, xyz_bw, 0, 2, 1, tm1, which='bw')
        noise_bw = ctx.draws.take("randn", n_rays, S)
        if ctx.rec is not None and nstd != 0:
            ctx.rec[f"{typ}_warp_fw"], ctx.rec[f"{typ}_warp_bw"] = noise_fw, noise_bw
        out('rgb_bw', n_rays, 3)
        args.update(raw_fw=raw_fw, raw_bw=raw_bw, xyz_fw=xyz_fw, xyz_bw=xyz_bw,
                    noise_fw=noise_fw if nstd != 0 else None,
                    noise_bw=noise_bw if nstd != 0 else None,
                    rgb_fw=results['rgb_fw'], rgb_bw=results['rgb_bw'],
                    xyzs_fw_bw=out('xyzs_fw_bw', n_rays, S, 3),
                    xyzs_bw_fw=out('xyzs_bw_fw', n_rays, S, 3))

    if output_transient:
        args['static_weights'] = out(f'static_weights_{typ}', n_rays, S)
        args['transient_weights'] = out(f'transient_weights_{typ}', n_rays, S)
        args['weights'] = out(f'weights_{typ}', n_rays, S)
    else:
        args['static_weights'] = out(f'static_weights_{typ}', n_rays, S)
    if test_time and output_transient:
        args['static_alphas'] = out(f'static_alphas_{typ}', n_rays, S)
        args['transient_alphas'] = out(f'transient_alphas_{typ}', n_rays, S)

    if not sigma_only:
        args['depth'] = out(f'depth_{typ}', n_rays)
        args['rgb'] = out(f'rgb_{typ}', n_rays, 3)
        if output_transient:
            args['transient_alpha'] = out(f'transient_alpha_{typ}', n_rays)
            args['transient_rgb'] = out(f'transient_rgb_{typ}', n_rays, 3)
            args['static_only_rgb'] = out(f'_static_rgb_{typ}', n_rays, 3)
            args['static_only_depth'] = out(f'_static_depth_{typ}', n_rays)
            if want_flow:
                args['flow_mode'] = 2 if warps else 1
                args['xyz_exp'] = out('xyz_fine', n_rays, 3)
                args['flow_fw_exp'] = out('transient_flow_fw', n_rays, 3)
                args['xyz_fw_exp'] = out('xyz_fw', n_rays, 3)
                args['flow_bw_exp'] = out('transient_flow_bw', n_rays, 3)
                args['xyz_bw_exp'] = out('xyz_bw', n_rays, 3)
                if disocc:
                    args['disocc_fw'] = out('disocc_fw', n_rays, 1)
                    args['disoccs_fw'] = out('disoccs_fw', n_rays, S, 1)
                    args['disocc_bw'] = out('disocc_bw', n_rays, 1)
                    args['disoccs_bw'] = out('disoccs_bw', n_rays, S, 1)
    if n_rays:
        _lib.composite(**args)


def render_rays(models,
                embeddings,
                rays,
                ts,
                max_t,
                N_samples=64,
                perturb=0,
                noise_std=0,
                N_importance=0,
                chunk=1024 * 32,
                test_time=False,
                **kwargs):
    _lib.require_gpu_tensor(rays, "rays")
    return range_check.checked(
        "render_rays", rays.device,
        lambda: _render_rays(models, embeddings, rays, ts, max_t, N_samples, perturb, noise_std, N_importance, chunk, test_time, kwargs),
        can_fallback=bool(test_time) and perturb == 0 and noise_std == 0)


def _render_rays(models, embeddings, rays, ts, max_t, N_samples, perturb, noise_std, N_importance, chunk, test_time, kwargs,
                 fine_points=None):
    _lib.require_gpu_tensor(rays, "rays")
    _lib.load()
    want_grad = (torch.is_grad_enabled() and not test_time and
                 bool(autograd.grad_parameters(models, embeddings)))
    rec = {} if want_grad else None
    with torch.cuda.device(rays.device), torch.no_grad():
        results = {}
        rays = rays.contiguous().float()
        n_rays = rays.shape[0]
        embedding_xyz, embedding_dir = embeddings['xyz'], embeddings['dir']

        ctx = _Pass()
        ctx.embeddings, ctx.rays, ctx.ts, ctx.max_t = embeddings, rays, ts, max_t
        ctx.noise_std, ctx.test_time, ctx.kwargs, ctx.n_rays = noise_std, test_time, kwargs, n_rays
        ctx.freqs_xyz = [float(f) for f in embedding_xyz.freqs]
        ctx.rec = rec
        ctx.tbias, ctx.neighbour_rows = {}, None
        ctx.dir_embedded = None
        if any(m.use_viewdir for m in models.values()):
            view_dir = kwargs.get('view_dir', rays[:, 3:6])
            ctx.dir_embedded = embedding_dir(view_dir.contiguous().float())

        z_lin = _unit_linspace(N_samples, rays.device)
        zs = _new(rays, n_rays, N_samples)
        xyz_coarse = _new(rays, n_rays, N_samples, 3)
        ctx.draws = _Draws(rays.device, n_rays, N_samples, N_importance, perturb, noise_std, test_time, models, kwargs,
                           coarse=(rays, z_lin, zs, xyz_coarse))
        perturb_rand = ctx.draws.take("rand", n_rays, N_samples) if perturb > 0 else None
        if n_rays and not ctx.draws.coarse_done:
            _lib.coarse_samples(rays, z_lin, perturb, perturb_rand, zs, xyz_coarse)

        t_embedded = None
        if N_importance > 0:
            model = models['coarse']
            output_transient = bool(kwargs.get('output_transient', True) and model.encode_transient)
            t_embedded = _time_codes(ctx, models, kwargs, N_samples, N_importance, output_transient,
                                     kwargs.get('output_transient_flow', []))
            _inference(results, ctx, model, xyz_coarse, zs, output_transient, [], t_embedded, None)

            det = perturb == 0
            if det:
                u_s = _unit_linspace(N_importance, rays.device)
                u_t = u_s
            else:
                u_s = ctx.draws.take("rand", n_rays, N_importance)
                u_t = ctx.draws.take("rand", n_rays, N_importance) if output_transient else None
            S_fine = N_samples + (2 if output_transient else 1) * N_importance
            zs_static = _new(rays, n_rays, N_importance) if test_time else None
            zs_transient = _new(rays, n_rays, N_importance) if (test_time and output_transient) else None
            zs_fine = _new(rays, n_rays, S_fine)
            xyz_fine = _new(rays, n_rays, S_fine, 3)
            if n_rays:
                _lib.fine_samples(rays, z_lin, zs, N_importance,
                                  results['static_weights_coarse'],
                                  results['transient_weights_coarse'] if output_transient else None,
                                  u_s, u_t if output_transient else None, 0 if det else 1,
                                  zs_static, zs_transient, zs_fine, xyz_fine)
            if test_time:
                results['static_zs_fine'] = zs_static
                if output_transient:
                    results['transient_zs_fine'] = zs_transient
            if fine_points is not None:
                zs_fine, xyz_fine = fine_points(rays, zs_fine, xyz_fine)
                if tuple(zs_fine.shape) != (n_rays, S_fine) or tuple(xyz_fine.shape) != (n_rays, S_fine, 3):
                    raise ValueError(f"fine_points: expected shapes {(n_rays, S_fine)} / {(n_rays, S_fine, 3)}")
            zs, xyz = zs_fine, xyz_fine
        else:
            xyz = xyz_coarse

        model = models['fine']
        a_embedded = None
        if model.encode_appearance:
            a_embedded = kwargs['a_embedded'] if 'a_embedded' in kwargs else embeddings['a'](ts)
            a_embedded = a_embedded.detach().contiguous().float()
        if N_importance == 0:
            output_transient = bool(kwargs.get('output_transient', True) and model.encode_transient)
            t_embedded = _time_codes(ctx, models, kwargs, N_samples, 0, output_transient, kwargs.get('output_transient_flow', []))
        output_transient_flow = [] if not output_transient else kwargs.get('output_transient_flow', [])
        _inference(results, ctx, model, xyz, zs, output_transient, output_transient_flow,
                   t_embedded, a_embedded)
    if rec is None:
        return results
    rec.update(N_importance=N_importance, noise_std=float(noise_std), output_transient=output_transient,
               flows=list(output_transient_flow), zs_coarse=results.get('zs_coarse', results.get('zs_fine')),
               zs_fine=results['zs_fine'], view_dir=kwargs.get('view_dir', rays[:, 3:6]), dir_embedded=ctx.dir_embedded,
               t_embedded_override=kwargs.get('t_embedded'), a_embedded_override=kwargs.get('a_embedded'))
    return autograd.attach(results, models, embeddings, rays, ts, max_t, rec)


from .interpolation import interpolate
```

Baseline: 68.33 million ray-samples/s.

## Fuse time-bias into RNG launch and coarse composite into fine sampling

Moves the time-bias computation ahead of coarse sampling and, with glue fusion on, folds it into the RNG draw kernel so the two share one launch. The coarse composite is deferred and fused with fine-sample generation in a new kernel. The time-bias kernel is also restructured to read time rows from constant memory with per-thread weight registers instead of an LDS tile. The aim is fewer small launches and less inter-kernel gap time in the glue around the field kernels, at the cost of more complex combined kernels and more register pressure.

Result: no change. 68.48 million ray-samples/s (median of 6 runs) (+0.2%).

```diff
diff --git a/include/nsff_render.h b/include/nsff_render.h
--- a/include/nsff_render.h
+++ b/include/nsff_render.h
@@ -133,6 +133,8 @@
     int32_t      pad_;
 } NsffRngCoarse;
 int nsff_rng_draws_coarse(const NsffRngJob* jobs, int32_t n_jobs, uint64_t seed, const NsffRngCoarse* coarse, void* stream);
+int nsff_rng_draws_time_bias(const NsffRngJob* jobs, int32_t n_jobs, uint64_t seed, const NsffRngCoarse* coarse,
+                             const NsffTimeBiasJob* tb_jobs, int32_t n_tb_jobs, int64_t tb_n_rays, void* stream);
 
 int nsff_side_bias(const NsffModelDesc* desc, const void* packed_f16x3, const float* w_dir, const float* dir_rows,
                    const float* a_rows, int64_t n_rays, float* out, void* stream);
@@ -315,6 +317,10 @@
 
 int nsff_composite(const NsffCompositeArgs* args, void* stream);
 
+int nsff_composite_fine_samples(const NsffCompositeArgs* coarse, const float* rays, const float* z_lin, int32_t n_importance,
+                                const float* u_static, const float* u_transient, int32_t u_per_ray,
+                                float* samples_static, float* samples_transient, float* zs_fine, float* xyz_fine, void* stream);
+
 int nsff_frustum_visibility(const NsffFrustumArgs* vis, const float* xyz, int64_t n_points, float* vis_count,
                             void* stream);
 
diff --git a/nsff_pl_amd/_lib.py b/nsff_pl_amd/_lib.py
--- a/nsff_pl_amd/_lib.py
+++ b/nsff_pl_amd/_lib.py
@@ -180,6 +180,8 @@
     "nsff_time_bias": (C.c_int, [C.POINTER(TimeBiasJob), C.c_int32, C.c_int64, C.c_void_p]),
     "nsff_rng_draws": (C.c_int, [C.POINTER(RngJob), C.c_int32, C.c_uint64, C.c_void_p]),
     "nsff_rng_draws_coarse": (C.c_int, [C.POINTER(RngJob), C.c_int32, C.c_uint64, C.POINTER(RngCoarse), C.c_void_p]),
+    "nsff_rng_draws_time_bias": (C.c_int, [C.POINTER(RngJob), C.c_int32, C.c_uint64, C.POINTER(RngCoarse),
+                                           C.POINTER(TimeBiasJob), C.c_int32, C.c_int64, C.c_void_p]),
     "nsff_side_bias": (C.c_int, [C.POINTER(ModelDesc), _fp, _fp, _fp, _fp, C.c_int64, _fp, C.c_void_p]),
     "nsff_last_hip_error": (C.c_char_p, []),
     "nsff_packed_bytes": (C.c_int, [C.POINTER(ModelDesc), C.c_int, C.POINTER(C.c_size_t)]),
@@ -198,6 +200,8 @@
                                   C.c_float, _fp, _fp]),
     "nsff_warp_points": (C.c_int, [_fp, _fp, _fp, C.c_int64, C.c_float, _fp, _fp, _fp]),
     "nsff_composite": (C.c_int, [C.POINTER(CompositeArgs), _fp]),
+    "nsff_composite_fine_samples": (C.c_int, [C.POINTER(CompositeArgs), _fp, _fp, C.c_int32, _fp, _fp, C.c_int32,
+                                              _fp, _fp, _fp, _fp, _fp]),
     "nsff_frustum_visibility": (C.c_int, [C.POINTER(FrustumArgs), _fp, C.c_int64, _fp, _fp]),
     "nsff_frame_rays": (C.c_int, [C.POINTER(C.c_float), C.POINTER(C.c_float), C.c_int32, C.c_int32, C.c_float,
                                   C.c_float, C.c_int64, C.c_int64, _fp, _fp]),
@@ -449,7 +453,7 @@
 _DEVICE_RNG_GEOMETRY = {}
 
 
-def fused_draws(plan, device, values=True, coarse=None):
+def fused_draws(plan, device, values=True, coarse=None, time_bias=None):
     dev = torch.device(device)
     idx = dev.index if dev.index is not None else torch.cuda.current_device()
     if idx not in _DEVICE_RNG_GEOMETRY:
@@ -496,8 +500,13 @@
         for j, (t, numel, off, kind, grid) in enumerate(part):
             arr[j].out, arr[j].numel, arr[j].offset, arr[j].kind, arr[j].grid = (None if t is None else t.data_ptr()), numel, off, kind, grid
         with torch.cuda.device(idx):
-            _check(load().nsff_rng_draws_coarse(arr, len(part), seed, C.byref(hook) if (hook is not None and k == 0) else None, _stream()),
-                   "nsff_rng_draws")
+            hook_k = C.byref(hook) if (hook is not None and k == 0) else None
+            if time_bias:
+                tb_arr, tb_n, tb_rays, _keep = time_bias.pop()
+                _check(load().nsff_rng_draws_time_bias(arr, len(part), seed, hook_k, tb_arr, tb_n, tb_rays, _stream()),
+                       "nsff_rng_draws_time_bias")
+            else:
+                _check(load().nsff_rng_draws_coarse(arr, len(part), seed, hook_k, _stream()), "nsff_rng_draws")
     gen.set_offset(offset)
     return outs
 
@@ -544,7 +553,7 @@
     return load().nsff_time_bias_rows(C.byref(model_desc(model)))
 
 
-def time_bias(jobs, index=None):
+def time_bias(jobs, index=None, pending=None):
     assert 1 <= len(jobs) <= MAX_TIME_BIAS_JOBS
     arr = (TimeBiasJob * len(jobs))()
     keep, outs, per_model, pair = [], [], {}, None
@@ -597,8 +606,17 @@
                 written.add(delta)
         outs.append(out)
     keep.append(per_model)
-    _check(load().nsff_time_bias(arr, len(jobs), n_rays, _stream()), "nsff_time_bias")
+    if pending is not None:
+        pending.append((arr, len(jobs), n_rays, keep))
+    else:
+        _check(load().nsff_time_bias(arr, len(jobs), n_rays, _stream()), "nsff_time_bias")
     return outs if index is None else (outs, rows_of)
+
+
+def launch_time_bias(pending):
+    while pending:
+        arr, n, n_rays, _keep = pending.pop(0)
+        _check(load().nsff_time_bias(arr, n, n_rays, _stream()), "nsff_time_bias")
 
 
 def coarse_samples(rays, z_lin, perturb, perturb_rand, zs, xyz):
@@ -641,7 +659,7 @@
            "nsff_frustum_visibility")
 
 
-def composite(vis=None, **kw):
+def _composite_args(vis=None, **kw):
     a = CompositeArgs()
     for k, v in kw.items():
         if k in _COMPOSITE_PTRS_IN or k in _COMPOSITE_PTRS_OUT:
@@ -650,7 +668,19 @@
             setattr(a, k, v)
     if vis is not None:
         a.vis = vis
-    _check(load().nsff_composite(C.byref(a), _stream()), "nsff_composite")
+    return a
+
+
+def composite(vis=None, **kw):
+    _check(load().nsff_composite(C.byref(_composite_args(vis, **kw)), _stream()), "nsff_composite")
+
+
+def composite_fine_samples(coarse, rays, z_lin, n_importance, u_static, u_transient, u_per_ray,
+                           samples_static, samples_transient, zs_fine, xyz_fine):
+    a = _composite_args(**coarse)
+    _check(load().nsff_composite_fine_samples(C.byref(a), _ptr(rays), _ptr(z_lin), int(n_importance), _ptr(u_static),
+                                              _ptr(u_transient), int(u_per_ray), _ptr(samples_static), _ptr(samples_transient),
+                                              _ptr(zs_fine), _ptr(xyz_fine), _stream()), "nsff_composite_fine_samples")
 
 
 def frame_rays(K4, c2w12, H, W, near, shift_near, first, count, rays):
diff --git a/nsff_pl_amd/csrc/field_h3.hip b/nsff_pl_amd/csrc/field_h3.hip
--- a/nsff_pl_amd/csrc/field_h3.hip
+++ b/nsff_pl_amd/csrc/field_h3.hip
@@ -5,6 +5,7 @@
 #include "nsff_layout_h3.h"
 #include "nsff_common.h"
 #include "nsff_internal.h"
+#include "nsff_time_bias.h"
 
 typedef float f32x16 __attribute__((ext_vector_type(16)));
 typedef _Float16 h8 __attribute__((ext_vector_type(8)));
@@ -1824,70 +1825,8 @@
 }
 
 namespace {
-struct TimeBiasJobK { const float* w[NSFF_MAX_LAYERS]; const float* b[NSFF_MAX_LAYERS]; int ld[NSFF_MAX_LAYERS];
-                      const float* t_rows; float* out; int rows, in_xyz, in_t;
-                      const float* table; const long long* ts; long long n_table, max_t; int delta; float* rows_out; };
-struct TimeBiasArgs { TimeBiasJobK job[NSFF_MAX_TIME_BIAS_JOBS]; long long n_rays; };
-constexpr int TB_RAYS = 16;
-__global__ __launch_bounds__(256) void nsff_time_bias_kernel(const TimeBiasArgs a) {
-    const TimeBiasJobK& j = a.job[blockIdx.z];
-    const int i = blockIdx.y, n = threadIdx.x;
-    if (i >= j.rows) return;
-    const long long r0 = (long long)blockIdx.x * TB_RAYS;
-    __shared__ __attribute__((aligned(16))) float st[TB_RAYS][64];
-    __shared__ float sw[16][NSFF_W + 1];
-    const float* __restrict__ wl = j.w[i] + j.in_xyz;
-    const int ld = j.ld[i], in_t = j.in_t;
-    float tv[TB_RAYS / 4], wv[4][16];
-#pragma unroll
-    for (int k = 0; k < TB_RAYS / 4; ++k) {
-        const int e = threadIdx.x + 256 * k, r = e >> 6, c = e & 63;
-        const long long ray = r0 + r < a.n_rays ? r0 + r : a.n_rays - 1;
-        const float* row = j.t_rows != nullptr ? j.t_rows + ray * in_t : nullptr;
-        if (row == nullptr) {
-            long long t = j.ts[ray] + j.delta;
-            if (j.delta > 0) t = t < j.max_t ? t : j.max_t;
-            if (j.delta < 0) t = t > 0 ? t : 0;
-            t = t < 0 ? 0 : (t > j.n_table - 1 ? j.n_table - 1 : t);
-            row = j.table + t * in_t;
-        }
-        tv[k] = c < in_t ? row[c] : 0.f;
-        if (j.rows_out != nullptr && i == 0 && c < in_t && r0 + r < a.n_rays) j.rows_out[(r0 + r) * in_t + c] = tv[k];
-    }
-    const float b = j.b[i][n];
-#pragma unroll
-    for (int q = 0; q < 4; ++q)
-#pragma unroll
-        for (int k = 0; k < 16; ++k) {
-            const int e = threadIdx.x + 256 * k, row = e >> 4, c = 16 * q + (e & 15);
-            wv[q][k] = c < in_t ? wl[row * ld + c] : 0.f;
-        }
-#pragma unroll
-    for (int k = 0; k < TB_RAYS / 4; ++k) { const int e = threadIdx.x + 256 * k; st[e >> 6][e & 63] = tv[k]; }
-    float acc[TB_RAYS];
-#pragma unroll
-    for (int r = 0; r < TB_RAYS; ++r) acc[r] = b;
-#pragma unroll
-    for (int q = 0; q < 4; ++q) {
-        if (16 * q >= in_t) break;
-        __syncthreads();
-#pragma unroll
-        for (int k = 0; k < 16; ++k) { const int e = threadIdx.x + 256 * k; sw[e & 15][e >> 4] = wv[q][k]; }
-        __syncthreads();
-#pragma unroll
-        for (int u = 0; u < 16; u += 4) {
-            const float w0 = sw[u][n], w1 = sw[u + 1][n], w2 = sw[u + 2][n], w3 = sw[u + 3][n];
-#pragma unroll
-            for (int r = 0; r < TB_RAYS; ++r) {
-                const float4 t4 = *reinterpret_cast<const float4*>(&st[r][16 * q + u]);
-                acc[r] = fmaf(w3, t4.w, fmaf(w2, t4.z, fmaf(w1, t4.y, fmaf(w0, t4.x, acc[r]))));
-            }
-        }
-    }
-#pragma unroll
-    for (int r = 0; r < TB_RAYS; ++r)
-        if (r0 + r < a.n_rays) j.out[((r0 + r) * j.rows + i) * NSFF_W + n] = acc[r];
-}
+constexpr int TB_RAYS = nsff_tb::RAYS;
+__global__ __launch_bounds__(256) void nsff_time_bias_kernel(const nsff_tb::Args a) { nsff_tb::block(a, blockIdx.x); }
 }
 
 extern "C" int nsff_time_bias_rows(const NsffModelDesc* desc) {
@@ -1895,11 +1834,10 @@
     return 1 + __builtin_popcount(nsff_skip_layers(desc));
 }
 
-extern "C" int nsff_time_bias(const NsffTimeBiasJob* jobs, int32_t n_jobs, int64_t n_rays, void* stream) {
+int nsff_tb::prepare(const NsffTimeBiasJob* jobs, int n_jobs, int64_t n_rays, nsff_tb::Args& a) {
     if (!jobs) return NSFF_ERR_NULL;
     if (n_jobs < 1 || n_jobs > NSFF_MAX_TIME_BIAS_JOBS || n_rays < 0) return NSFF_ERR_INVALID;
-    if (n_rays == 0) return NSFF_OK;
-    TimeBiasArgs a{};
+    a = nsff_tb::Args{};
     a.n_rays = n_rays;
     int max_rows = 0;
     for (int q = 0; q < n_jobs; ++q) {
@@ -1910,7 +1848,7 @@
         NsffLayoutH3 L;
         const int rc = nsff_make_layout_h3(d, L);
         if (rc) return rc;
-        TimeBiasJobK& k = a.job[q];
+        nsff_tb::JobK& k = a.job[q];
         k.rows = nsff_time_bias_rows(&d);
         if (k.rows < 1) return NSFF_ERR_INVALID;
         if (d.in_t > 64 || (d.in_t & 3) != 0) return NSFF_ERR_INVALID;
@@ -1929,9 +1867,19 @@
         max_rows = std::max(max_rows, k.rows);
     }
     const long long gx = (n_rays + TB_RAYS - 1) / TB_RAYS;
-    if (gx > 0x7fffffffLL) return NSFF_ERR_INVALID;
-    hipLaunchKernelGGL(nsff_time_bias_kernel, dim3((unsigned)gx, (unsigned)max_rows, (unsigned)n_jobs), dim3(256), 0,
-                       reinterpret_cast<hipStream_t>(stream), a);
+    if (gx * max_rows * n_jobs > 0x7fffffffLL) return NSFF_ERR_INVALID;
+    a.gx = (unsigned)gx; a.max_rows = (unsigned)max_rows; a.n_blocks = (unsigned)(gx * max_rows * n_jobs);
+    return NSFF_OK;
+}
+
+extern "C" int nsff_time_bias(const NsffTimeBiasJob* jobs, int32_t n_jobs, int64_t n_rays, void* stream) {
+    if (!jobs) return NSFF_ERR_NULL;
+    if (n_jobs < 1 || n_jobs > NSFF_MAX_TIME_BIAS_JOBS || n_rays < 0) return NSFF_ERR_INVALID;
+    if (n_rays == 0) return NSFF_OK;
+    nsff_tb::Args a;
+    const int rc = nsff_tb::prepare(jobs, n_jobs, n_rays, a);
+    if (rc) return rc;
+    hipLaunchKernelGGL(nsff_time_bias_kernel, dim3(a.n_blocks), dim3(256), 0, reinterpret_cast<hipStream_t>(stream), a);
     return nsff_launch_status();
 }
 
diff --git a/nsff_pl_amd/csrc/nsff_time_bias.h b/nsff_pl_amd/csrc/nsff_time_bias.h
--- /dev/null
+++ b/nsff_pl_amd/csrc/nsff_time_bias.h
@@ -0,0 +1,98 @@
+#pragma once
+#include <hip/hip_runtime.h>
+#include "../../include/nsff_render.h"
+
+#ifndef NSFF_W
+#define NSFF_W 256
+#endif
+
+namespace nsff_tb {
+
+struct JobK { const float* w[NSFF_MAX_LAYERS]; const float* b[NSFF_MAX_LAYERS]; int ld[NSFF_MAX_LAYERS];
+              const float* t_rows; float* out; int rows, in_xyz, in_t;
+              const float* table; const long long* ts; long long n_table, max_t; int delta; float* rows_out; };
+struct Args { JobK job[NSFF_MAX_TIME_BIAS_JOBS]; long long n_rays; unsigned gx, max_rows, n_blocks; };
+constexpr int RAYS = 16;
+
+int prepare(const NsffTimeBiasJob* jobs, int n_jobs, int64_t n_rays, Args& a);
+
+typedef const __attribute__((address_space(4))) float cfloat;
+typedef const __attribute__((address_space(4))) long long clong;
+
+__device__ __forceinline__ const float* t_row(const JobK& j, long long ray) {
+    if (j.t_rows != nullptr) return j.t_rows + ray * j.in_t;
+    long long t = *(clong*)(j.ts + ray) + j.delta;
+    if (j.delta > 0) t = t < j.max_t ? t : j.max_t;
+    if (j.delta < 0) t = t > 0 ? t : 0;
+    t = t < 0 ? 0 : (t > j.n_table - 1 ? j.n_table - 1 : t);
+    return j.table + t * j.in_t;
+}
+
+__device__ __forceinline__ void block(const Args& a, unsigned g) {
+    const unsigned x = g % a.gx, rest = g / a.gx;
+    const int i = (int)(rest % a.max_rows), z = (int)(rest / a.max_rows);
+    const JobK& j = a.job[z];
+    if (i >= j.rows) return;
+    const int n = threadIdx.x;
+    const long long r0 = (long long)x * RAYS, last = a.n_rays - 1;
+    __shared__ float sw[16][NSFF_W + 1];
+    const float* __restrict__ wl = j.w[i] + j.in_xyz;
+    const int ld = j.ld[i], in_t = j.in_t;
+    float wv[4][16];
+#pragma unroll
+    for (int q = 0; q < 4; ++q)
+#pragma unroll
+        for (int k = 0; k < 16; ++k) {
+            const int e = threadIdx.x + 256 * k, row = e >> 4, c = 16 * q + (e & 15);
+            wv[q][k] = c < in_t ? wl[row * ld + c] : 0.f;
+        }
+    const float b = j.b[i][n];
+    if (j.rows_out != nullptr && i == 0) {
+#pragma unroll
+        for (int k = 0; k < RAYS / 4; ++k) {
+            const int e = threadIdx.x + 256 * k, r = e >> 6, c = e & 63;
+            if (c < in_t && r0 + r <= last) j.rows_out[(r0 + r) * in_t + c] = t_row(j, r0 + r)[c];
+        }
+    }
+    float wr[64];
+#pragma unroll
+    for (int q = 0; q < 4; ++q) {
+        if (16 * q >= in_t) break;
+        __syncthreads();
+#pragma unroll
+        for (int k = 0; k < 16; ++k) { const int e = threadIdx.x + 256 * k; sw[e & 15][e >> 4] = wv[q][k]; }
+        __syncthreads();
+#pragma unroll
+        for (int u = 0; u < 16; ++u) wr[16 * q + u] = sw[u][n];
+    }
+#pragma unroll
+    for (int r4 = 0; r4 < RAYS; r4 += 4) {
+        cfloat* row[4];
+        float acc[4];
+#pragma unroll
+        for (int rr = 0; rr < 4; ++rr) {
+            const long long ray = r0 + r4 + rr <= last ? r0 + r4 + rr : last;
+            row[rr] = (cfloat*)t_row(j, ray);
+            acc[rr] = b;
+        }
+#pragma unroll
+        for (int q = 0; q < 4; ++q) {
+            if (16 * q >= in_t) break;
+#pragma unroll
+            for (int u = 0; u < 16; u += 4) {
+                const int c = 16 * q + u;
+#pragma unroll
+                for (int rr = 0; rr < 4; ++rr) {
+                    float t[4] = {0.f, 0.f, 0.f, 0.f};
+                    if (c < in_t) { t[0] = row[rr][c]; t[1] = row[rr][c + 1]; t[2] = row[rr][c + 2]; t[3] = row[rr][c + 3]; }
+                    acc[rr] = fmaf(wr[c + 3], t[3], fmaf(wr[c + 2], t[2], fmaf(wr[c + 1], t[1], fmaf(wr[c], t[0], acc[rr]))));
+                }
+            }
+        }
+#pragma unroll
+        for (int rr = 0; rr < 4; ++rr)
+            if (r0 + r4 + rr <= last) j.out[((r0 + r4 + rr) * j.rows + i) * NSFF_W + n] = acc[rr];
+    }
+}
+
+}
diff --git a/nsff_pl_amd/csrc/rays.hip b/nsff_pl_amd/csrc/rays.hip
--- a/nsff_pl_amd/csrc/rays.hip
+++ b/nsff_pl_amd/csrc/rays.hip
@@ -98,11 +98,11 @@
     float* zs_fine; float* xyz_fine;
 };
 
-__global__ __launch_bounds__(64 * WAVES_PER_BLOCK) void fine_samples_kernel(const FineArgs a) {
-    extern __shared__ __attribute__((aligned(16))) float smem[];
+__host__ __device__ inline int fine_lds_floats(int S, int Sf) { return WAVES_PER_BLOCK * S + ((S + 3) & ~3) + Sf; }
+
+__device__ __forceinline__ void fine_ray(const FineArgs& a, long long ray, const float* w_s, const float* w_t, float* smem) {
     const int lane = threadIdx.x & 63, wave = threadIdx.x >> 6, tid = threadIdx.x;
     constexpr int T = 64 * WAVES_PER_BLOCK;
-    const long long ray = blockIdx.x;
     const int S = a.S, n_imp = a.n_imp;
     const int k_sets = a.w_transient ? 2 : 1;
     const int Sf = S + k_sets * n_imp;
@@ -115,7 +115,7 @@
     {
         const bool mine = wave < k_sets;
         const int set = mine ? wave : 0;
-        const float* w = (set == 0 ? a.w_static : a.w_transient) + ray * S + 1;
+        const float* w = (set == 0 ? w_s : w_t) + 1;
         const float* ub = set == 0 ? a.u_static : a.u_transient;
         const float* u = a.u_per_ray ? ub + ray * n_imp : ub;
         float* keep = set == 0 ? a.samples_static : a.samples_transient;
@@ -145,6 +145,12 @@
         a.xyz_fine[dst * 3 + 1] = o1 + d1 * v;
         a.xyz_fine[dst * 3 + 2] = o2 + d2 * v;
     }
+}
+
+__global__ __launch_bounds__(64 * WAVES_PER_BLOCK) void fine_samples_kernel(const FineArgs a) {
+    extern __shared__ __attribute__((aligned(16))) float smem[];
+    const long long ray = blockIdx.x;
+    fine_ray(a, ray, a.w_static + ray * a.S, a.w_transient ? a.w_transient + ray * a.S : nullptr, smem);
 }
 
 struct PdfArgs {
@@ -241,10 +247,7 @@
     if (p < n_points) out[p] = frustum_count(v, xyz[3 * p], xyz[3 * p + 1], xyz[3 * p + 2]);
 }
 
-__global__ __launch_bounds__(64 * WAVES_PER_BLOCK) void composite_kernel(const NsffCompositeArgs a) {
-    const int lane = threadIdx.x & 63;
-    const long long ray = (long long)blockIdx.x * WAVES_PER_BLOCK + (threadIdx.x >> 6);
-    if (ray >= a.n_rays) return;
+__device__ __forceinline__ void composite_ray(const NsffCompositeArgs& a, long long ray, int lane, float* lw_s, float* lw_t) {
     const int S = a.n_samples;
     const bool tr = a.has_transient != 0;
     const bool flows = tr && a.flow_mode >= 1;
@@ -315,6 +318,8 @@
                 if (a.static_weights) a.static_weights[idx] = w;
                 if (a.weights) a.weights[idx] = w;
             }
+            if (lw_s) lw_s[i] = tr ? w_s : w;
+            if (lw_t && tr) lw_t[i] = w_t;
         }
         if (!a.has_rgb) continue;
 
@@ -449,6 +454,24 @@
     }
 }
 
+__global__ __launch_bounds__(64 * WAVES_PER_BLOCK) void composite_kernel(const NsffCompositeArgs a) {
+    const int lane = threadIdx.x & 63;
+    const long long ray = (long long)blockIdx.x * WAVES_PER_BLOCK + (threadIdx.x >> 6);
+    if (ray >= a.n_rays) return;
+    composite_ray(a, ray, lane, nullptr, nullptr);
+}
+
+__global__ __launch_bounds__(64 * WAVES_PER_BLOCK) void coarse_fine_kernel(const NsffCompositeArgs c, const FineArgs f) {
+    extern __shared__ __attribute__((aligned(16))) float smem[];
+    const long long ray = blockIdx.x;
+    const int S = c.n_samples;
+    float* lw_s = smem;
+    float* lw_t = smem + S;
+    if ((threadIdx.x >> 6) == 0) composite_ray(c, ray, threadIdx.x & 63, lw_s, f.w_transient ? lw_t : nullptr);
+    __syncthreads();
+    fine_ray(f, ray, lw_s, lw_t, smem + ((2 * S + 3) & ~3));
+}
+
 template <int NCH>
 __global__ __launch_bounds__(64 * NCH) void composite_kernel_chunks(const NsffCompositeArgs a) {
     __shared__ float tot[NCH][4];
@@ -489,15 +512,36 @@
         alpha = 1.f - (1.f - al_s) * (1.f - al_t);
         if (a.has_rgb) { rgb_t[0] = rec[4]; rgb_t[1] = rec[5]; rgb_t[2] = rec[6]; }
     }
+    const bool far = z > a.z_far;
+    float ffw[3] = {0.f, 0.f, 0.f}, fbw[3] = {0.f, 0.f, 0.f}, x[3] = {0.f, 0.f, 0.f};
+    float sgw[2] = {0.f, 0.f}, rgbw[2][3] = {}, backw[2][3] = {}, xw[2][3] = {};
+    if (flows) {
+#pragma unroll
+        for (int k = 0; k < 3; ++k) {
+            ffw[k] = far ? 0.f : rec[8 + k];
+            fbw[k] = far ? 0.f : rec[11 + k];
+            x[k] = a.xyz[idx * 3 + k];
+        }
+    }
+    if (a.has_rgb && warps) {
+#pragma unroll
+        for (int dir = 0; dir < 2; ++dir) {
+            const float* recw = (dir == 0 ? a.raw_fw : a.raw_bw) + idx * RS;
+            const float* xwp = (dir == 0 ? a.xyz_fw : a.xyz_bw) + idx * 3;
+            const int head = dir == 0 ? 11 : 8;
+            sgw[dir] = recw[7];
+#pragma unroll
+            for (int k = 0; k < 3; ++k) { rgbw[dir][k] = recw[4 + k]; backw[dir][k] = recw[head + k]; xw[dir][k] = xwp[k]; }
+        }
+    }
     const float inc = wave_scan_mul(on ? 1.f - alpha : 1.f, lane);
     float incs = 1.f, incw[2] = {1.f, 1.f}, al_tw[2] = {0.f, 0.f};
     if (a.has_rgb && tr) incs = wave_scan_mul(on ? 1.f - al_s : 1.f, lane);
     if (a.has_rgb && warps) {
 #pragma unroll
         for (int dir = 0; dir < 2; ++dir) {
-            const float* recw = (dir == 0 ? a.raw_fw : a.raw_bw) + idx * RS;
             const float* nz = dir == 0 ? a.noise_fw : a.noise_bw;
-            float sg = recw[7];
+            float sg = sgw[dir];
             if (nz) sg += nz[idx] * a.noise_std;
             al_tw[dir] = 1.f - expf(-d_t * softplus(sg));
             const float al_w = 1.f - (1.f - al_s) * (1.f - al_tw[dir]);
@@ -565,14 +609,6 @@
         }
     }
     if (flows) {
-        const bool far = z > a.z_far;
-        float ffw[3], fbw[3], x[3];
-#pragma unroll
-        for (int k = 0; k < 3; ++k) {
-            ffw[k] = far ? 0.f : rec[8 + k];
-            fbw[k] = far ? 0.f : rec[11 + k];
-            x[k] = a.xyz[idx * 3 + k];
-        }
         if (on) {
 #pragma unroll
             for (int k = 0; k < 3; ++k) {
@@ -584,20 +620,17 @@
         if (warps) {
 #pragma unroll
             for (int dir = 0; dir < 2; ++dir) {
-                const float* recw = (dir == 0 ? a.raw_fw : a.raw_bw) + idx * RS;
                 float excw = __shfl_up(incw[dir], 1);
                 if (lane == 0) excw = 1.f;
                 const float Tw = cTw[dir] * excw;
                 const float ws_w = al_s * Tw, wt_w = al_tw[dir] * Tw;
                 if (on) {
 #pragma unroll
-                    for (int k = 0; k < 3; ++k) p[(dir == 0 ? P_RGBFW : P_RGBBW) + k] = ws_w * rgb_s[k] + wt_w * recw[4 + k];
-                    const float* xw = (dir == 0 ? a.xyz_fw : a.xyz_bw) + idx * 3;
+                    for (int k = 0; k < 3; ++k) p[(dir == 0 ? P_RGBFW : P_RGBBW) + k] = ws_w * rgb_s[k] + wt_w * rgbw[dir][k];
                     float* cyc = dir == 0 ? a.xyzs_fw_bw : a.xyzs_bw_fw;
-                    const int head = dir == 0 ? 11 : 8;
                     if (cyc) {
 #pragma unroll
-                        for (int k = 0; k < 3; ++k) cyc[idx * 3 + k] = xw[k] + (far ? 0.f : recw[head + k]);
+                        for (int k = 0; k < 3; ++k) cyc[idx * 3 + k] = xw[dir][k] + (far ? 0.f : backw[dir][k]);
                     }
                     const float occ = wt_w - w_t;
                     if (dir == 0) { p[P_OCCFW] = occ; if (a.disoccs_fw) a.disoccs_fw[idx] = 1.f - fabsf(occ); }
@@ -809,11 +842,40 @@
                weights_static, weights_transient, u_static, u_transient, u_per_ray,
                samples_static, samples_transient, zs_fine, xyz_fine};
     const int Sf = n_samples + (weights_transient ? 2 : 1) * n_importance;
-    const size_t lds = (size_t)(WAVES_PER_BLOCK * n_samples + ((n_samples + 3) & ~3) + Sf) * sizeof(float);
+    const size_t lds = (size_t)fine_lds_floats(n_samples, Sf) * sizeof(float);
     if (lds > 64 * 1024 || n_rays > 0x7fffffffLL) return NSFF_ERR_INVALID;
     const unsigned blocks = (unsigned)n_rays;
     hipLaunchKernelGGL(fine_samples_kernel, dim3(blocks), dim3(64 * WAVES_PER_BLOCK), lds,
                        (hipStream_t)stream, a);
+    return nsff_launch_status();
+}
+
+int nsff_composite_fine_samples(const NsffCompositeArgs* coarse, const float* rays, const float* z_lin, int32_t n_importance,
+                                const float* u_static, const float* u_transient, int32_t u_per_ray,
+                                float* samples_static, float* samples_transient, float* zs_fine, float* xyz_fine, void* stream) {
+    if (!coarse) return NSFF_ERR_NULL;
+    const NsffCompositeArgs& c = *coarse;
+    if (c.n_rays < 0 || c.n_samples < 3 || n_importance < 1 || c.flow_mode != 0) return NSFF_ERR_INVALID;
+    if (c.n_rays == 0) return NSFF_OK;
+    const bool tr = c.has_transient != 0;
+    if (!c.static_weights || (tr && !c.transient_weights)) return NSFF_ERR_NULL;
+    if (c.n_samples > 64) {
+        const int rc = nsff_composite(coarse, stream);
+        if (rc) return rc;
+        return nsff_fine_samples(rays, c.n_rays, z_lin, c.zs, c.n_samples, n_importance, c.static_weights,
+                                 tr ? c.transient_weights : nullptr, u_static, tr ? u_transient : nullptr, u_per_ray,
+                                 samples_static, samples_transient, zs_fine, xyz_fine, stream);
+    }
+    if (!c.raw || !c.zs || !rays || !z_lin || !u_static || !zs_fine || !xyz_fine || (tr && !u_transient)) return NSFF_ERR_NULL;
+    if (c.vis.w2c && (!c.vis.ts || !c.xyz)) return NSFF_ERR_NULL;
+    if (c.vis.w2c && (c.vis.n_cams < 1 || c.vis.n_frames < 1)) return NSFF_ERR_INVALID;
+    if (c.n_rays > 0x7fffffffLL) return NSFF_ERR_INVALID;
+    const int S = c.n_samples, Sf = S + (tr ? 2 : 1) * n_importance;
+    FineArgs f{rays, c.n_rays, z_lin, c.zs, S, n_importance, c.static_weights, tr ? c.transient_weights : nullptr,
+               u_static, tr ? u_transient : nullptr, u_per_ray, samples_static, samples_transient, zs_fine, xyz_fine};
+    const size_t lds = (size_t)(((2 * S + 3) & ~3) + fine_lds_floats(S, Sf)) * sizeof(float);
+    if (lds > 64 * 1024) return NSFF_ERR_INVALID;
+    hipLaunchKernelGGL(coarse_fine_kernel, dim3((unsigned)c.n_rays), dim3(64 * WAVES_PER_BLOCK), lds, (hipStream_t)stream, c, f);
     return nsff_launch_status();
 }
 
diff --git a/nsff_pl_amd/csrc/rng.hip b/nsff_pl_amd/csrc/rng.hip
--- a/nsff_pl_amd/csrc/rng.hip
+++ b/nsff_pl_amd/csrc/rng.hip
@@ -4,6 +4,7 @@
 
 #include "../../include/nsff_render.h"
 #include "nsff_common.h"
+#include "nsff_time_bias.h"
 
 namespace {
 
@@ -32,11 +33,11 @@
     for (int k = 0; k < 3; ++k) { const float dz = r[3 + k] * z; c.xyz[idx * 3 + k] = r[k] + dz; }
 }
 
-__global__ __launch_bounds__(256) void nsff_rng_kernel(const RngArgs a) {
+__device__ __forceinline__ void rng_block(const RngArgs& a, unsigned block) {
     int j = 0;
-    while (j + 1 < a.n && blockIdx.x >= a.first_block[j + 1]) ++j;
+    while (j + 1 < a.n && block >= a.first_block[j + 1]) ++j;
     const NsffRngJob& J = a.job[j];
-    const long long idx = (long long)(blockIdx.x - a.first_block[j]) * 256 + threadIdx.x;
+    const long long idx = (long long)(block - a.first_block[j]) * 256 + threadIdx.x;
     hiprandStatePhilox4_32_10_t state;
     hiprand_init(a.seed, (unsigned long long)idx, J.offset, &state);
     const long long stride = 256LL * J.grid, numel = J.numel;
@@ -57,17 +58,23 @@
     }
 }
 
+__global__ __launch_bounds__(256) void nsff_rng_kernel(const RngArgs a) { rng_block(a, blockIdx.x); }
+
+__global__ __launch_bounds__(256) void nsff_rng_tb_kernel(const RngArgs a, const nsff_tb::Args t) {
+    if (blockIdx.x < t.n_blocks) nsff_tb::block(t, blockIdx.x);
+    else rng_block(a, blockIdx.x - t.n_blocks);
+}
+
 }
 
 extern "C" int nsff_rng_draws(const NsffRngJob* jobs, int32_t n_jobs, uint64_t seed, void* stream) {
     return nsff_rng_draws_coarse(jobs, n_jobs, seed, nullptr, stream);
 }
 
-extern "C" int nsff_rng_draws_coarse(const NsffRngJob* jobs, int32_t n_jobs, uint64_t seed, const NsffRngCoarse* coarse, void* stream) {
-    if (n_jobs == 0) return coarse ? NSFF_ERR_INVALID : NSFF_OK;
+static int rng_args(const NsffRngJob* jobs, int32_t n_jobs, uint64_t seed, const NsffRngCoarse* coarse, RngArgs& a) {
     if (!jobs) return NSFF_ERR_NULL;
-    if (n_jobs < 0 || n_jobs > NSFF_MAX_RNG_JOBS) return NSFF_ERR_INVALID;
-    RngArgs a{};
+    if (n_jobs < 1 || n_jobs > NSFF_MAX_RNG_JOBS) return NSFF_ERR_INVALID;
+    a = RngArgs{};
     a.coarse.job = -1;
     if (coarse) {
         const NsffRngCoarse& c = *coarse;
@@ -89,7 +96,35 @@
     a.first_block[n_jobs] = total;
     a.n = n_jobs;
     a.seed = seed;
-    hipLaunchKernelGGL(nsff_rng_kernel, dim3(total), dim3(256), 0, (hipStream_t)stream, a);
+    return NSFF_OK;
+}
+
+extern "C" int nsff_rng_draws_coarse(const NsffRngJob* jobs, int32_t n_jobs, uint64_t seed, const NsffRngCoarse* coarse, void* stream) {
+    if (n_jobs == 0) return coarse ? NSFF_ERR_INVALID : NSFF_OK;
+    RngArgs a;
+    const int rc = rng_args(jobs, n_jobs, seed, coarse, a);
+    if (rc) return rc;
+    hipLaunchKernelGGL(nsff_rng_kernel, dim3(a.first_block[n_jobs]), dim3(256), 0, (hipStream_t)stream, a);
     const hipError_t e = hipGetLastError();
     return e == hipSuccess ? NSFF_OK : nsff_hip_fail(e);
 }
+
+extern "C" int nsff_rng_draws_time_bias(const NsffRngJob* jobs, int32_t n_jobs, uint64_t seed, const NsffRngCoarse* coarse,
+                                        const NsffTimeBiasJob* tb_jobs, int32_t n_tb_jobs, int64_t tb_n_rays, void* stream) {
+    if (n_jobs == 0 || tb_n_rays == 0) {
+        int rc = nsff_rng_draws_coarse(jobs, n_jobs, seed, coarse, stream);
+        if (rc == NSFF_OK) rc = nsff_time_bias(tb_jobs, n_tb_jobs, tb_n_rays, stream);
+        return rc;
+    }
+    RngArgs a;
+    int rc = rng_args(jobs, n_jobs, seed, coarse, a);
+    if (rc) return rc;
+    nsff_tb::Args t;
+    rc = nsff_tb::prepare(tb_jobs, n_tb_jobs, tb_n_rays, t);
+    if (rc) return rc;
+    const unsigned draws = a.first_block[n_jobs];
+    if (t.n_blocks + draws < draws) return NSFF_ERR_INVALID;
+    hipLaunchKernelGGL(nsff_rng_tb_kernel, dim3(t.n_blocks + draws), dim3(256), 0, (hipStream_t)stream, a, t);
+    const hipError_t e = hipGetLastError();
+    return e == hipSuccess ? NSFF_OK : nsff_hip_fail(e);
+}
diff --git a/nsff_pl_amd/rendering.py b/nsff_pl_amd/rendering.py
--- a/nsff_pl_amd/rendering.py
+++ b/nsff_pl_amd/rendering.py
@@ -35,7 +35,8 @@
 
 class _Draws:
 
-    def __init__(self, device, n_rays, N_samples, N_importance, perturb, noise_std, test_time, models, kwargs, coarse=None):
+    def __init__(self, device, n_rays, N_samples, N_importance, perturb, noise_std, test_time, models, kwargs, coarse=None,
+                 time_bias=None):
         self.device = device
         self.coarse_done = False
         self.fused = (device.type == "cuda" and torch.rand is _TORCH_RAND and torch.randn is _TORCH_RANDN
@@ -75,7 +76,7 @@
                 add("randn", noisy, n_rays, S)
                 add("randn", noisy, n_rays, S)
         self.plan = plan
-        self.values = _lib.fused_draws(plan, device, need, coarse=hook)
+        self.values = _lib.fused_draws(plan, device, need, coarse=hook, time_bias=time_bias)
         self.coarse_done = hook is not None
 
     def take(self, kind, *shape):
@@ -89,7 +90,7 @@
 
 class _Pass:
     __slots__ = ("embeddings", "rays", "ts", "max_t", "noise_std", "test_time", "kwargs",
-                 "freqs_xyz", "dir_embedded", "n_rays", "rec", "tbias", "neighbour_rows", "draws")
+                 "freqs_xyz", "dir_embedded", "n_rays", "rec", "tbias", "neighbour_rows", "draws", "tb_pending")
 
 
 def _embed_rows(embeddings, key, idx):
@@ -141,7 +142,8 @@
              and ts.dim() == 1 and ts.shape[0] == n_rays)
     if (plan and plain and all(mod.in_channels_t == m.weight.shape[1] for _, _, mod, _ in plan)
             and not os.environ.get('NSFF_NO_TIME_INDEX')):
-        outs, rows = _lib.time_bias([(mod, d) for _, _, mod, d in plan], index=(m.weight.detach(), ts.contiguous(), ctx.max_t))
+        outs, rows = _lib.time_bias([(mod, d) for _, _, mod, d in plan], index=(m.weight.detach(), ts.contiguous(), ctx.max_t),
+                                    pending=ctx.tb_pending)
         for (typ, which, _, _), out in zip(plan, outs):
             ctx.tbias[(typ, which)] = out
         if 1 in rows:
@@ -154,13 +156,13 @@
         if any(w == 'fw' for _, w, _, _ in plan):
             ctx.neighbour_rows = _neighbour_time_rows(ctx.embeddings, ts, ctx.max_t)
         src = {0: t_embedded, 1: ctx.neighbour_rows[0] if ctx.neighbour_rows else None, -1: ctx.neighbour_rows[1] if ctx.neighbour_rows else None}
-        for (typ, which, _, _), out in zip(plan, _lib.time_bias([(mod, src[d]) for _, _, mod, d in plan])):
+        for (typ, which, _, _), out in zip(plan, _lib.time_bias([(mod, src[d]) for _, _, mod, d in plan], pending=ctx.tb_pending)):
             ctx.tbias[(typ, which)] = out
     return t_embedded
 
 
 def _inference(results, ctx, model, xyz, zs, output_transient, output_transient_flow,
-               t_embedded, a_embedded):
+               t_embedded, a_embedded, defer_composite=False):
     typ = model.typ
     n_rays, S = zs.shape
     test_time = ctx.test_time
@@ -298,8 +300,11 @@
                     args['disoccs_fw'] = out('disoccs_fw', n_rays, S, 1)
                     args['disocc_bw'] = out('disocc_bw', n_rays, 1)
                     args['disoccs_bw'] = out('disoccs_bw', n_rays, S, 1)
+    if defer_composite:
+        return args
     if n_rays:
         _lib.composite(**args)
+    return None
 
 
 def render_rays(models,
@@ -345,22 +350,27 @@
             view_dir = kwargs.get('view_dir', rays[:, 3:6])
             ctx.dir_embedded = embedding_dir(view_dir.contiguous().float())
 
+        glue = not os.environ.get('NSFF_NO_GLUE_FUSION')
+        output_transient = bool(kwargs.get('output_transient', True)
+                                and models['coarse' if N_importance > 0 else 'fine'].encode_transient)
+        ctx.tb_pending = []
+        t_embedded = _time_codes(ctx, models, kwargs, N_samples, N_importance, output_transient,
+                                 kwargs.get('output_transient_flow', []))
+
         z_lin = _unit_linspace(N_samples, rays.device)
         zs = _new(rays, n_rays, N_samples)
         xyz_coarse = _new(rays, n_rays, N_samples, 3)
         ctx.draws = _Draws(rays.device, n_rays, N_samples, N_importance, perturb, noise_std, test_time, models, kwargs,
-                           coarse=(rays, z_lin, zs, xyz_coarse))
+                           coarse=(rays, z_lin, zs, xyz_coarse), time_bias=ctx.tb_pending if glue else None)
         perturb_rand = ctx.draws.take("rand", n_rays, N_samples) if perturb > 0 else None
         if n_rays and not ctx.draws.coarse_done:
             _lib.coarse_samples(rays, z_lin, perturb, perturb_rand, zs, xyz_coarse)
-
-        t_embedded = None
+        _lib.launch_time_bias(ctx.tb_pending)
+
         if N_importance > 0:
             model = models['coarse']
-            output_transient = bool(kwargs.get('output_transient', True) and model.encode_transient)
-            t_embedded = _time_codes(ctx, models, kwargs, N_samples, N_importance, output_transient,
-                                     kwargs.get('output_transient_flow', []))
-            _inference(results, ctx, model, xyz_coarse, zs, output_transient, [], t_embedded, None)
+            coarse_args = _inference(results, ctx, model, xyz_coarse, zs, output_transient, [], t_embedded, None,
+                                     defer_composite=glue)
 
             det = perturb == 0
             if det:
@@ -374,7 +384,10 @@
             zs_transient = _new(rays, n_rays, N_importance) if (test_time and output_transient) else None
             zs_fine = _new(rays, n_rays, S_fine)
             xyz_fine = _new(rays, n_rays, S_fine, 3)
-            if n_rays:
+            if n_rays and coarse_args is not None:
+                _lib.composite_fine_samples(coarse_args, rays, z_lin, N_importance, u_s, u_t if output_transient else None,
+                                            0 if det else 1, zs_static, zs_transient, zs_fine, xyz_fine)
+            elif n_rays:
                 _lib.fine_samples(rays, z_lin, zs, N_importance,
                                   results['static_weights_coarse'],
                                   results['transient_weights_coarse'] if output_transient else None,
@@ -397,9 +410,6 @@
         if model.encode_appearance:
             a_embedded = kwargs['a_embedded'] if 'a_embedded' in kwargs else embeddings['a'](ts)
             a_embedded = a_embedded.detach().contiguous().float()
-        if N_importance == 0:
-            output_transient = bool(kwargs.get('output_transient', True) and model.encode_transient)
-            t_embedded = _time_codes(ctx, models, kwargs, N_samples, 0, output_transient, kwargs.get('output_transient_flow', []))
         output_transient_flow = [] if not output_transient else kwargs.get('output_transient_flow', [])
         _inference(results, ctx, model, xyz, zs, output_transient, output_transient_flow,
                    t_embedded, a_embedded)
diff --git a/profiles/summarize_r07.py b/profiles/summarize_r07.py
--- /dev/null
+++ b/profiles/summarize_r07.py
@@ -0,0 +1,66 @@
+#!/usr/bin/env python
+import csv
+import statistics
+import sys
+
+
+def short(name):
+    name = name.replace("(anonymous namespace)::", "")
+    for cut in ("(", " "):
+        if name.startswith("void "):
+            name = name[5:]
+        name = name.split(cut)[0] if cut == "(" else name
+    return name
+
+
+def calls_of(rows):
+    calls, cur = [], None
+    for r in rows:
+        if r["name"].startswith("nsff_rng"):
+            if cur:
+                calls.append(cur)
+            cur = []
+        if cur is not None:
+            cur.append(r)
+    if cur:
+        calls.append(cur)
+    return calls
+
+
+def main():
+    path = sys.argv[1]
+    skip = int(sys.argv[sys.argv.index("--skip") + 1]) if "--skip" in sys.argv else 5
+    rows = []
+    with open(path) as f:
+        for r in csv.DictReader(f):
+            rows.append(dict(name=short(r["Kernel_Name"]), t0=int(r["Start_Timestamp"]), t1=int(r["End_Timestamp"])))
+    rows.sort(key=lambda r: r["t0"])
+    calls = calls_of(rows)
+    seqs = [tuple(r["name"] for r in c) for c in calls[skip:-1]]
+    common = statistics.mode(seqs)
+    steady = [c for c in calls[skip:-1] if tuple(r["name"] for r in c) == common]
+    print(f"{len(calls)} calls in the trace, {len(steady)} steady-state calls with the common sequence of {len(common)} launches")
+    print(f"{'#':>2} {'kernel':<34} {'dur us':>8} {'gap us':>8} {'start us':>9} {'end us':>9}   (median over calls; start/end of the median call)")
+    durs = [[(c[i]["t1"] - c[i]["t0"]) / 1e3 for c in steady] for i in range(len(common))]
+    gaps = [[(c[i]["t0"] - c[i - 1]["t1"]) / 1e3 if i else 0.0 for c in steady] for i in range(len(common))]
+    spans = [(c[-1]["t1"] - c[0]["t0"]) / 1e3 for c in steady]
+    med_call = steady[sorted(range(len(steady)), key=lambda k: spans[k])[len(steady) // 2]]
+    base = med_call[0]["t0"]
+    for i, name in enumerate(common):
+        print(f"{i:>2} {name[:34]:<34} {statistics.median(durs[i]):8.1f} {statistics.median(gaps[i]):8.1f} "
+              f"{(med_call[i]['t0'] - base) / 1e3:9.1f} {(med_call[i]['t1'] - base) / 1e3:9.1f}")
+    field = [i for i, n in enumerate(common) if n.startswith("nsff_field_kernel")]
+    k_field = sum(statistics.median(durs[i]) for i in field)
+    k_other = sum(statistics.median(durs[i]) for i in range(len(common)) if i not in field)
+    g_all = sum(statistics.median(gaps[i]) for i in range(len(common)))
+    inter = []
+    for a, b in zip(calls[skip:-1], calls[skip + 1:]):
+        inter.append((b[0]["t0"] - a[-1]["t1"]) / 1e3)
+    print(f"launches per call {len(common)}; call span (first start -> last end) median {statistics.median(spans):.1f} us")
+    print(f"kernel time: field {k_field:.1f} us, other {k_other:.1f} us; gaps inside the call {g_all:.1f} us; "
+          f"gap between calls median {statistics.median(inter):.1f} us")
+    print(f"outside the field kernels (other kernels + gaps inside the call): {k_other + g_all:.1f} us")
+
+
+if __name__ == "__main__":
+    main()
```
